# DeMoriarty/TorchPQ

Hardware: AMD Instinct MI355X
Metric: queries/sec + recall@100, SIFT1M IVFPQ d=128 m=64 nprobe=32 (higher is better)
Workload: dtype f32; 1 GPU; SIFT1M-like d=128 n=1000000 IVFPQ n_cells=1024 m=64 nprobe=32 k=100 on 1xMI355X per rank; n_query_per_rank=10000, code_layout=packed, codes=u8 (8-bit PQ), arithmetic=f32 LUT entries, f32 sums, exact ids, use_smart_probing=False, parallelism=query-sharded x1, replicated index, world_size_seen=1, index_broadcast_bytes=0

## Files before the change

__graft_entry__.py:

```python
import os
import subprocess
import sys

ROOT = os.path.dirname(os.path.abspath(__file__))
if ROOT not in sys.path:
    sys.path.insert(0, ROOT)


def build_cabi_demo() -> None:
    src = os.path.join(ROOT, "tests", "cabi", "scan_demo.cpp")
    subprocess.check_call([
        os.environ.get("HIPCC", "/opt/rocm/bin/hipcc"), "--offload-arch=gfx950", "-O2",
        "-I", os.path.join(ROOT, "include"), src, "-L", os.path.join(ROOT, "torchpq_amd"),
        "-ltorchpq_amd", "-Wl,-rpath,$ORIGIN/../../torchpq_amd",
        "-o", os.path.join(ROOT, "tests", "cabi", "scan_demo")])


def check_store_hazard() -> None:
    if os.environ.get("TPQ_SKIP_HAZARD_CHECK", "0") == "1":
        return
    tool = os.path.join(ROOT, "tools", "check_store_hazard.py")
    procs = [(u, subprocess.Popen([sys.executable, tool, "--window", "2", u], stdout=subprocess.PIPE,
                                  stderr=subprocess.STDOUT, text=True))
             for u in ("cascade_core.hip", "assign_cascade.hip", "probe_sims.hip", "lloyd.hip", "select.hip",
                       "coarse_probe.hip", "assign_fast.hip", "flat_topk.hip")]
    bad = []
    for u, p in procs:
        out = p.communicate()[0]
        print(out.strip().splitlines()[-1] if out.strip() else f"{u}: no output")
        if p.returncode != 0:
            bad.append((u, out[-1500:]))
    assert not bad, f"store-data hazard pattern within two instructions: {bad}"


def check_flat_tile_registers() -> None:
    if os.environ.get("TPQ_SKIP_HAZARD_CHECK", "0") == "1":
        return
    out = subprocess.run([sys.executable, os.path.join(ROOT, "tools", "kernel_regs.py"), "flat_topk.hip", "--grep",
                          "flat_tile_kernel"], capture_output=True, text=True, check=True).stdout
    rows = [line for line in out.splitlines() if "flat_tile_kernel" in line]
    assert len(rows) == 5, out
    bad = [line for line in rows if " spill   0 " not in line]
    assert not bad, f"flat_tile_kernel spills registers: {bad}"
    print(f"flat_topk.hip: {len(rows)} flat_tile_kernel instantiations, no register spills")


def check_flat_range_registers() -> None:
    if os.environ.get("TPQ_SKIP_HAZARD_CHECK", "0") == "1":
        return
    out = subprocess.run([sys.executable, os.path.join(ROOT, "tools", "kernel_regs.py"), "flat_range.hip", "--grep",
                          "flat_range_"], capture_output=True, text=True, check=True).stdout
    rows = [line for line in out.splitlines() if "flat_range_" in line]
    assert len(rows) == 2, out
    bad = [line for line in rows if " spill   0 scratch    0 " not in line]
    assert not bad, f"flat_range kernels spill registers or use scratch: {bad}"
    print(f"flat_range.hip: {len(rows)} kernels, no register spills, no scratch")


def check_scan_range_registers() -> None:
    if os.environ.get("TPQ_SKIP_HAZARD_CHECK", "0") == "1":
        return
    out = subprocess.run([sys.executable, os.path.join(ROOT, "tools", "kernel_regs.py"), "scan_range.hip", "--grep",
                          "ivfpq_range_"], capture_output=True, text=True, check=True).stdout
    rows = [line for line in out.splitlines() if "ivfpq_range_" in line]
    assert len(rows) == 4, out
    bad = [line for line in rows if " spill   0 scratch    0 " not in line]
    assert not bad, f"scan_range kernels spill registers or use scratch: {bad}"
    print(f"scan_range.hip: {len(rows)} kernels, no register spills, no scratch")


def check_scan_filtered_registers() -> None:
    if os.environ.get("TPQ_SKIP_HAZARD_CHECK", "0") == "1":
        return
    out = subprocess.run([sys.executable, os.path.join(ROOT, "tools", "kernel_regs.py"), "scan_filtered.hip", "--grep",
                          "filter"], capture_output=True, text=True, check=True).stdout
    rows = [line for line in out.splitlines() if "scan_filtered_" in line or "slot_filter_build" in line]
    assert len(rows) == 11, out
    bad = [line for line in rows if " spill   0 " not in line]
    bad += [line for line in rows if ("<1>" in line or "<2>" in line or "slot_filter" in line)
            and " scratch    0 " not in line]
    assert not bad, f"scan_filtered kernels spill registers or use scratch: {bad}"
    print(f"scan_filtered.hip: {len(rows)} kernels, no register spills, no scratch up to k = 128")


def check_scan_pq4_filtered_registers() -> None:
    if os.environ.get("TPQ_SKIP_HAZARD_CHECK", "0") == "1":
        return
    out = subprocess.run([sys.executable, os.path.join(ROOT, "tools", "kernel_regs.py"), "scan_pq4_filtered.hip",
                          "--grep", "scan_pq4_filtered_"], capture_output=True, text=True, check=True).stdout
    rows = [line for line in out.splitlines() if "scan_pq4_filtered_" in line]
    assert len(rows) == 20, out
    bad = [line for line in rows if " spill   0 " not in line]
    bad += [line for line in rows if ("kernel<1," in line or "kernel<2," in line) and " scratch    0 " not in line]
    assert not bad, f"scan_pq4_filtered kernels spill registers or use scratch: {bad}"
    print(f"scan_pq4_filtered.hip: {len(rows)} kernels, no register spills, no scratch up to k = 128")


def check_scan_pq4_range_registers() -> None:
    if os.environ.get("TPQ_SKIP_HAZARD_CHECK", "0") == "1":
        return
    out = subprocess.run([sys.executable, os.path.join(ROOT, "tools", "kernel_regs.py"), "scan_pq4_range.hip", "--grep",
                          "ivfpq4_range_"], capture_output=True, text=True, check=True).stdout
    rows = [line for line in out.splitlines() if "ivfpq4_range_" in line]
    assert len(rows) == 16, out
    bad = [line for line in rows if " spill   0 scratch    0 " not in line]
    assert not bad, f"scan_pq4_range kernels spill registers or use scratch: {bad}"
    print(f"scan_pq4_range.hip: {len(rows)} kernels, no register spills, no scratch")


def check_scan_flat_registers() -> None:
    if os.environ.get("TPQ_SKIP_HAZARD_CHECK", "0") == "1":
        return
    out = subprocess.run([sys.executable, os.path.join(ROOT, "tools", "kernel_regs.py"), "scan_flat.hip", "--grep",
                          "scan_flat_kernel"], capture_output=True, text=True, check=True).stdout
    rows = [line for line in out.splitlines() if "scan_flat_kernel" in line]
    assert len(rows) == 20, out
    bad = [line for line in rows if " spill   0 " not in line or int(line.split(" vgpr ")[1].split()[0]) > 72]
    assert not bad, f"scan_flat_kernel spills registers or drops below seven waves per SIMD: {bad}"
    print(f"scan_flat.hip: {len(rows)} scan_flat_kernel instantiations, no register spills, at most 72 VGPRs")


def build() -> None:
    subprocess.check_call(["bash", os.path.join(ROOT, "torchpq_amd", "csrc", "build.sh")])
    subprocess.check_call(["make", "-C", os.path.join(ROOT, "oracle"), "libivfpq_oracle.so"])
    build_cabi_demo()
    check_store_hazard()
    check_flat_tile_registers()
    check_flat_range_registers()
    check_scan_range_registers()
    check_scan_filtered_registers()
    check_scan_pq4_filtered_registers()
    check_scan_pq4_range_registers()
    check_scan_flat_registers()
    import torchpq_amd
    from torchpq_amd import _lib
    lib = _lib.load()
    assert lib.tpq_version() >= 100
    for name in _lib.SIGNATURES:
        getattr(lib, name)
    print("build ok:", _lib.LIB_PATH, "version", lib.tpq_version(), "torchpq_amd", torchpq_amd.__version__)


def smoke() -> None:
    import numpy as np
    import torch
    from oracle import c_oracle
    from oracle import ivfpq_oracle as orc
    from torchpq_amd.index import IVFPQIndex

    assert torch.cuda.is_available(), "smoke() needs the MI355X"
    rng = np.random.default_rng(0)
    d, n, nq, k = 64, 8192, 64, 10
    centers = rng.standard_normal((d, 32)) * 4
    base = (centers[:, rng.integers(0, 32, n)] + rng.standard_normal((d, n))).astype(np.float32)
    queries = (base[:, :nq] + 0.1 * rng.standard_normal((d, nq))).astype(np.float32)
    np.random.seed(0)
    idx = IVFPQIndex(d_vector=d, n_subvectors=16, n_cells=32, initial_size=512, device="cuda:0")
    idx.train(torch.from_numpy(base).cuda())
    idx.add(torch.from_numpy(base).cuda())
    idx.n_probe = 8
    xq = torch.from_numpy(queries).cuda()
    vals, ids = idx.search(xq, k=k)
    torch.cuda.synchronize()

    _, cells, npl = idx.probe(xq)
    cells, npl = cells.cpu().numpy(), npl.cpu().numpy()
    lut = c_oracle.adc_lut(queries, idx.pq_codec.codebook.cpu().numpy())
    cs = idx._cell_start.cpu().numpy()[cells]
    sz = idx._cell_size.cpu().numpy()[cells]
    ev, ea = c_oracle.scan_topk(idx._storage.cpu().numpy(), lut, idx._is_empty.cpu().numpy(), cs, sz,
                                npl, k)
    ei = orc.get_id_by_address(idx._address2id.cpu().numpy(), ea)
    assert np.array_equal(vals.cpu().numpy(), ev), "values differ from the oracle"
    assert np.array_equal(ids.cpu().numpy(), ei), "ids differ from the oracle"
    hit = float((ids[:, 0].cpu().numpy() == np.arange(nq)).mean())
    assert hit > 0.8, hit
    print(f"smoke ok: top-1 self hit {hit:.2f}, values/ids bit-exact vs oracle")


if __name__ == "__main__":
    build()
    if len(sys.argv) > 1 and sys.argv[1] == "smoke":
        smoke()
```

include/torchpq_amd.h:

```cpp
#ifndef TORCHPQ_AMD_H_
#define TORCHPQ_AMD_H_

#include <stddef.h>
#include <stdint.h>

#ifdef __cplusplus
extern "C" {
#endif

#define TPQ_VERSION 500

#define TPQ_OK 0
#define TPQ_ERR_INVALID_ARGUMENT (-1)
#define TPQ_ERR_HIP (-2)
#define TPQ_ERR_WORKSPACE (-3)
#define TPQ_ERR_UNSUPPORTED (-4)

#define TPQ_METRIC_NEG_SQ_L2 0
#define TPQ_METRIC_INNER 1

typedef void* tpq_stream_t;

int tpq_version(void);
const char* tpq_last_error(void);

size_t tpq_ivfpq_scan_workspace_bytes(int nq, int k, int n_split, int m);

int tpq_ivfpq_scan_topk(const uint8_t* codes, const float* lut, const uint8_t* is_empty,
                        const int64_t* cell_start, const int64_t* cell_size,
                        const int64_t* n_probe_list, float* out_vals, int64_t* out_addr,
                        const int64_t* address2id, int64_t* out_ids, int64_t n_slots, int nq,
                        int max_nprobe, int m, int k, int n_split, void* workspace,
                        size_t workspace_bytes, tpq_stream_t stream);

int tpq_ivfpq_pack_codes(const uint8_t* codes, uint8_t* packed, int64_t n_slots, int m,
                         int64_t slot_begin, int64_t slot_end, tpq_stream_t stream);

int tpq_ivfpq_scan_topk_packed(const uint8_t* packed, const uint8_t* codes, const float* lut,
                               const uint8_t* is_empty, const int64_t* cell_start,
                               const int64_t* cell_size, const int64_t* n_probe_list,
                               float* out_vals, int64_t* out_addr, const int64_t* address2id,
                               int64_t* out_ids, int64_t n_slots, int nq, int max_nprobe, int m,
                               int k, int n_split, void* workspace, size_t workspace_bytes,
                               tpq_stream_t stream);
size_t tpq_ivfpq_scan_tickets_bytes(int nq);

#define TPQ_SCAN_ROUTE_REF 0
#define TPQ_SCAN_ROUTE_ONE_LAUNCH 1
#define TPQ_SCAN_ROUTE_LISTS 2
#define TPQ_SCAN_ROUTE_POOLS 3
#define TPQ_SCAN_ROUTE_DUMP_F32 8
#define TPQ_SCAN_ROUTE_DUMP_SEL16 16
#define TPQ_SCAN_ROUTE_DUMP_SEL16_W8 17
int tpq_ivfpq_scan_route(int nq, int k, int n_split, int m, int ds, int max_nprobe, int64_t slots_hint, int has_lut,
                         int has_packed, int has_tickets, int residual);
int tpq_ivfpq_scan_order(const int64_t* cell_start, const int64_t* cell_size, const int64_t* n_probe_list, int nq,
                         int max_nprobe, int tile_shift, int32_t* order, int32_t* rank, int32_t* work,
                         tpq_stream_t stream);
int tpq_ivfpq_scan_ordered(int nq, int k, int n_split, int m, int ds, int max_nprobe, int64_t slots_hint, int has_lut,
                           int has_packed, int has_tickets, int residual, int slots, size_t workspace_bytes);
int tpq_ivfpq_scan_topk_packed_tickets(const uint8_t* packed, const uint8_t* codes, const float* lut,
                                       const uint8_t* is_empty, const int64_t* cell_start,
                                       const int64_t* cell_size, const int64_t* n_probe_list,
                                       float* out_vals, int64_t* out_addr, const int64_t* address2id,
                                       int64_t* out_ids, int64_t n_slots, int nq, int max_nprobe,
                                       int m, int k, int n_split, void* workspace,
                                       size_t workspace_bytes, int32_t* tickets, int64_t slots_hint,
                                       tpq_stream_t stream);

int tpq_ivfpq_search_fused(const uint8_t* packed, const uint8_t* codes, const float* query,
                           const float* codebook, int ds, int metric, const uint8_t* is_empty,
                           const int64_t* cell_start, const int64_t* cell_size,
                           const int64_t* n_probe_list, float* out_vals, int64_t* out_addr,
                           const int64_t* address2id, int64_t* out_ids, int64_t n_slots, int nq,
                           int max_nprobe, int m, int k, int n_split, void* workspace,
                           size_t workspace_bytes, tpq_stream_t stream);
int tpq_ivfpq_search_fused_tickets(const uint8_t* packed, const uint8_t* codes, const float* query,
                                   const float* codebook, int ds, int metric, const uint8_t* is_empty,
                                   const int64_t* cell_start, const int64_t* cell_size,
                                   const int64_t* n_probe_list, float* out_vals, int64_t* out_addr,
                                   const int64_t* address2id, int64_t* out_ids, int64_t n_slots,
                                   int nq, int max_nprobe, int m, int k, int n_split, void* workspace,
                                   size_t workspace_bytes, int32_t* tickets, int64_t slots_hint,
                                   tpq_stream_t stream);
int tpq_ivfpq_search_fused_cells(const uint8_t* packed, const uint8_t* codes, const float* query,
                                 const float* codebook, int ds, int metric, const uint8_t* is_empty,
                                 const int64_t* cell_start, const int64_t* cell_size,
                                 const int64_t* n_probe_list, float* out_vals, int64_t* out_addr,
                                 const int64_t* address2id, int64_t* out_ids, int64_t n_slots,
                                 int nq, int max_nprobe, int m, int k, int n_split, void* workspace,
                                 size_t workspace_bytes, int32_t* tickets, int64_t slots_hint,
                                 const int64_t* cells, int n_cells, tpq_stream_t stream);
int tpq_ivfpq_scan_cell_major(int nq, int k, int n_split, int m, int ds, int max_nprobe, int64_t slots_hint, int has_lut,
                              int has_packed, int has_tickets, int residual, int n_cells, int64_t n_slots,
                              size_t workspace_bytes);
int tpq_ivfpq_scan_cell_norms(int nq, int k, int n_split, int m, int ds, int max_nprobe, int64_t slots_hint, int has_lut,
                              int has_packed, int has_tickets, int residual, int n_cells, int64_t n_slots,
                              size_t workspace_bytes);
size_t tpq_ivfpq_cell_candidates_workspace_bytes(int nq, int max_nprobe, int n_cells, int first_probe);
size_t tpq_ivfpq_cell_candidates_norms_workspace_bytes(int nq, int max_nprobe, int n_cells, int first_probe,
                                                       int64_t n_slots);
int tpq_ivfpq_cell_candidates(const uint8_t* codes, const float* query, const float* codebook, int ds, int metric,
                              const uint8_t* is_empty, const int64_t* cell_start, const int64_t* cell_size,
                              const int64_t* n_probe_list, const int64_t* cells, int n_cells, int first_probe,
                              const float* threshold, int64_t n_slots, int nq, int max_nprobe, int m, int capacity,
                              int32_t* out_count, uint32_t* out_keys, uint32_t* out_addr, float* out_delta,
                              int32_t* out_flags, void* workspace, size_t workspace_bytes, tpq_stream_t stream);
float tpq_ivfpq_cell_fold_threshold(float threshold, float q2);
int tpq_ivfpq_scan_cell_threshold(int nq, int k, int n_split, int m, int ds, int max_nprobe, int64_t slots_hint,
                                  int has_lut, int has_packed, int has_tickets, int residual, int n_cells,
                                  int64_t n_slots, size_t workspace_bytes);
int tpq_ivfpq_scan_use_cell_threshold(int on);
int tpq_ivfpq_scan_cell_threshold_probes(void);
#define TPQ_HAS_IVFPQ_CELL_KEPT 1
size_t tpq_ivfpq_cell_kept_bytes(int64_t n_slots, int ds);
long long tpq_ivfpq_scan_cell_inversions(void);
int tpq_ivfpq_search_fused_cells_kept(const uint8_t* packed, const uint8_t* codes, const float* query,
                                      const float* codebook, int ds, int metric, const uint8_t* is_empty,
                                      const int64_t* cell_start, const int64_t* cell_size,
                                      const int64_t* n_probe_list, float* out_vals, int64_t* out_addr,
                                      const int64_t* address2id, int64_t* out_ids, int64_t n_slots,
                                      int nq, int max_nprobe, int m, int k, int n_split, void* workspace,
                                      size_t workspace_bytes, int32_t* tickets, int64_t slots_hint,
                                      const int64_t* cells, int n_cells, void* kept, size_t kept_bytes,
                                      int kept_valid, tpq_stream_t stream);

int tpq_ivfpq_scan_topk_residual(const uint8_t* codes, const float* part1, const float* part2,
                                 const float* full_lut, const int64_t* cells,
                                 const float* base_sims, const uint8_t* is_empty,
                                 const int64_t* cell_start, const int64_t* cell_size,
                                 const int64_t* n_probe_list, float* out_vals, int64_t* out_addr,
                                 const int64_t* address2id, int64_t* out_ids, int64_t n_slots,
                                 int nq, int max_nprobe, int m, int k, tpq_stream_t stream);
int tpq_residual_part1(const float* query, const float* codebook, float* part1, int m, int ds,
                       int nq, tpq_stream_t stream);

int tpq_ivfpq_residual_slot_terms(const uint8_t* codes, const float* part2,
                                  const int64_t* cell_start, const int64_t* cell_size,
                                  float* slot_term, float* cell_bound, int64_t n_slots,
                                  int n_cells, int m, tpq_stream_t stream);
int tpq_ivfpq_scan_topk_residual_packed(
    const uint8_t* packed, const uint8_t* codes, const float* part1, const float* query,
    const float* codebook, int ds, const float* part2, const float* slot_term,
    const float* cell_bound, const int64_t* cells, const float* base_sims, const uint8_t* is_empty,
    const int64_t* cell_start, const int64_t* cell_size, const int64_t* n_probe_list,
    float* out_vals, int64_t* out_addr, const int64_t* address2id, int64_t* out_ids,
    int64_t n_slots, int nq, int max_nprobe, int m, int k, int n_split, void* workspace,
    size_t workspace_bytes, tpq_stream_t stream);

int tpq_adc_lut(const float* query, const float* codebook, float* lut, int m, int ds, int nq,
                int metric, tpq_stream_t stream);

int tpq_topk_select(const float* x, float* vals, int64_t* idx, int rows, int cols, int k,
                    tpq_stream_t stream);

int tpq_coarse_select(const float* dots, const float* a2, const float* b2, float* vals, int64_t* idx,
                      int rows, int cols, int k, tpq_stream_t stream);

size_t tpq_ivfpq_coarse_probe_workspace_bytes(int nq, int n_cells);
int tpq_ivfpq_coarse_probe(const float* query, const float* centroids,
                           const int64_t* cell_start_tbl, const int64_t* cell_size_tbl,
                           float* topk_sims, int64_t* cells, int64_t* cell_start,
                           int64_t* cell_size, int64_t* n_probe_list, int d, int nq, int n_cells,
                           int n_probe, float smart_temperature, void* workspace,
                           size_t workspace_bytes, tpq_stream_t stream);
#define TPQ_PROBE_ROUTE_AUTO 0
#define TPQ_PROBE_ROUTE_FP32 1
#define TPQ_PROBE_ROUTE_FP16 2
size_t tpq_ivfpq_coarse_probe_route_workspace_bytes(int d, int nq, int n_cells, int route);
int tpq_ivfpq_coarse_probe_route(const float* query, const float* centroids,
                                 const int64_t* cell_start_tbl, const int64_t* cell_size_tbl,
                                 float* topk_sims, int64_t* cells, int64_t* cell_start,
                                 int64_t* cell_size, int64_t* n_probe_list, int d, int nq, int n_cells,
                                 int n_probe, float smart_temperature, int route, const void* prepared,
                                 void* workspace, size_t workspace_bytes, tpq_stream_t stream);
size_t tpq_ivfpq_coarse_probe_prepared_bytes(int d, int n_cells);
int tpq_ivfpq_coarse_probe_prepare(const float* centroids, int d, int n_cells, void* prepared,
                                   size_t prepared_bytes, tpq_stream_t stream);

int tpq_smart_probing(const float* topk_sims, int64_t* n_probe_list, int rows, int n_probe,
                      float temperature, tpq_stream_t stream);

int tpq_get_address_by_id(const int64_t* address2id, int64_t capacity, const int64_t* ids,
                          int64_t* address, int64_t n_ids, tpq_stream_t stream);

int tpq_get_id_by_address(const int64_t* address2id, int64_t capacity, const int64_t* address,
                          int64_t* ids, int64_t n, tpq_stream_t stream);

int tpq_max_sim(const float* A, const float* B, float* vals, int64_t* inds, int l, int d, int m,
                int n, int metric, tpq_stream_t stream);

int tpq_max_sim_split_supported(int d, int64_t m, int n);
int tpq_max_sim_split(const float* A, const float* B, float* vals, int64_t* inds, int l, int d, int m,
                      int n, int metric, tpq_stream_t stream);

#define TPQ_ASSIGN_ROUTE_AUTO 0
#define TPQ_ASSIGN_ROUTE_CASCADE 1
int tpq_coarse_assign_supported(int d, int64_t m, int n);
size_t tpq_coarse_assign_workspace_bytes(int d, int64_t m, int n);
size_t tpq_coarse_assign_count_offset(int d, int64_t m, int n);
int tpq_coarse_assign(const float* A, const float* B, float* vals, int64_t* inds, int d, int64_t m, int n,
                      int metric, void* workspace, size_t workspace_bytes, tpq_stream_t stream);
size_t tpq_coarse_assign_route_workspace_bytes(int d, int64_t m, int n, int route);
int tpq_coarse_assign_route(const float* A, const float* B, float* vals, int64_t* inds, int d, int64_t m, int n,
                            int metric, int route, void* workspace, size_t workspace_bytes, tpq_stream_t stream);

int tpq_max_sim_select_supported(int l, int d, int64_t m, int n);
size_t tpq_max_sim_select_workspace_bytes(int l, int d, int64_t m, int n);
int tpq_max_sim_select(const float* A, const float* B, float* vals, int64_t* inds, int l, int d, int64_t m,
                       int n, int metric, void* workspace, size_t workspace_bytes, tpq_stream_t stream);

int tpq_lloyd_supported(int l, int d, int64_t m, int n);
size_t tpq_lloyd_prepared_bytes(int l, int d, int64_t m);
int tpq_lloyd_prepare(const float* data, const float* centroids0, void* prepared, size_t prepared_bytes,
                      int l, int d, int64_t m, int n, tpq_stream_t stream);
size_t tpq_lloyd_step_workspace_bytes(int l, int d, int64_t m, int n);
size_t tpq_lloyd_step_count_offset(int l, int d, int64_t m, int n, int level);
int tpq_lloyd_step(const float* data, const void* prepared, const float* centroids, float* new_centroids,
                   float* vals, int64_t* inds, int l, int d, int64_t m, int n, void* workspace,
                   size_t workspace_bytes, tpq_stream_t stream);

size_t tpq_compute_centroids_workspace_bytes(int l, int d, int k);
int tpq_compute_centroids(const float* data, const int64_t* labels, float* centroids, int l, int d,
                          int64_t n, int k, void* workspace, size_t workspace_bytes,
                          tpq_stream_t stream);

size_t tpq_get_ioa_workspace_bytes(int64_t n);
int tpq_get_ioa(const int64_t* labels, int64_t* ioa, int64_t n, int64_t n_cells, void* workspace,
                size_t workspace_bytes, tpq_stream_t stream);
int tpq_get_write_address(const uint8_t* is_empty, const int64_t* cell_start,
                          const int64_t* cell_capacity, const int64_t* labels, const int64_t* ioa,
                          int64_t* write_address, int64_t n_slots, int64_t n_labels,
                          tpq_stream_t stream);
int tpq_get_cell_by_address(const int64_t* address, const int64_t* cell_start,
                            const int64_t* cell_capacity, int64_t* cells, int64_t n_address,
                            int64_t n_cells, tpq_stream_t stream);

int tpq_grow_cells(const uint8_t* storage, const int64_t* address2id, const uint8_t* is_empty,
                   const int64_t* old_start, const int64_t* old_capacity, const int64_t* new_start,
                   const int64_t* new_capacity, uint8_t* new_storage, int64_t* new_address2id,
                   uint8_t* new_is_empty, int64_t old_slots, int64_t new_slots, int n_cells, int m,
                   tpq_stream_t stream);

int tpq_pq_decode(const float* codebook, const uint8_t* codes, float* out, int m, int ds, int64_t n,
                  tpq_stream_t stream);

int tpq_scatter_codes(const uint8_t* codes, const int64_t* address, uint8_t* storage,
                      uint8_t* packed, int m, int64_t n, int64_t n_slots, tpq_stream_t stream);

int tpq_ivfpqr_rerank(const uint8_t* storage, int64_t capacity, int m, int m_r, const float* codebook,
                      const float* codebook_r, const float* query, int d, int nq, const int64_t* cand_address,
                      int k1, int k, int use_residual, int distance, const int64_t* address2id, float* out_vals,
                      int64_t* out_address, int64_t* out_ids, tpq_stream_t stream);

size_t tpq_ivfflat_scan_workspace_bytes(int nq, int k, int n_split);
int tpq_ivfflat_scan_topk(const float* vectors, const float* query, const uint8_t* is_empty,
                          const int64_t* cell_start, const int64_t* cell_size, const int64_t* n_probe_list,
                          float* out_vals, int64_t* out_addr, int64_t n_slots, int d, int nq, int max_nprobe, int k,
                          int metric, int n_split, void* workspace, size_t workspace_bytes, tpq_stream_t stream);

size_t tpq_ivfpq4_scan_workspace_bytes(int nq, int k, int n_split);
int tpq_ivfpq4_scan_topk(const uint8_t* codes, const float* query, const float* codebook, const uint8_t* is_empty,
                         const int64_t* cell_start, const int64_t* cell_size, const int64_t* n_probe_list,
                         float* out_vals, int64_t* out_addr, int64_t n_slots, int m, int ds, int nq, int max_nprobe,
                         int k, int metric, int n_split, void* workspace, size_t workspace_bytes,
                         tpq_stream_t stream);
// ... 133 lines not shown
```

torchpq_amd/_lib.py:

```python
from __future__ import annotations

import ctypes as C
import os

import torch

_HERE = os.path.dirname(os.path.abspath(__file__))
LIB_PATH = os.environ.get("TPQ_AMD_LIB") or os.path.join(_HERE, "libtorchpq_amd.so")

METRIC_NEG_SQ_L2 = 0
METRIC_INNER = 1
ERR_UNSUPPORTED = -4
ERR_WORKSPACE = -3
ASSIGN_ROUTE_AUTO = 0
ASSIGN_ROUTE_CASCADE = 1
PROBE_ROUTE_AUTO, PROBE_ROUTE_FP32, PROBE_ROUTE_FP16 = 0, 1, 2

_vp, _i, _i64, _sz, _f = C.c_void_p, C.c_int, C.c_int64, C.c_size_t, C.c_float

SIGNATURES = {
    "tpq_version": (_i, []),
    "tpq_last_error": (C.c_char_p, []),
    "tpq_ivfpq_scan_workspace_bytes": (_sz, [_i, _i, _i, _i]),
    "tpq_ivfpq_scan_topk": (_i, [_vp, _vp, _vp, _vp, _vp, _vp, _vp, _vp, _vp, _vp, _i64, _i, _i, _i,
                                 _i, _i, _vp, _sz, _vp]),
    "tpq_ivfpq_pack_codes": (_i, [_vp, _vp, _i64, _i, _i64, _i64, _vp]),
    "tpq_ivfpq_scan_topk_packed": (_i, [_vp, _vp, _vp, _vp, _vp, _vp, _vp, _vp, _vp, _vp, _vp, _i64,
                                        _i, _i, _i, _i, _i, _vp, _sz, _vp]),
    "tpq_ivfpq_search_fused": (_i, [_vp, _vp, _vp, _vp, _i, _i, _vp, _vp, _vp, _vp, _vp, _vp, _vp, _vp,
                                    _i64, _i, _i, _i, _i, _i, _vp, _sz, _vp]),
    "tpq_ivfpq_scan_tickets_bytes": (_sz, [_i]),
    "tpq_ivfpq_scan_route": (_i, [_i, _i, _i, _i, _i, _i, _i64, _i, _i, _i, _i]),
    "tpq_ivfpq_scan_order": (_i, [_vp, _vp, _vp, _i, _i, _i, _vp, _vp, _vp, _vp]),
    "tpq_ivfpq_scan_ordered": (_i, [_i, _i, _i, _i, _i, _i, _i64, _i, _i, _i, _i, _i, _sz]),
    "tpq_ivfpq_scan_topk_packed_tickets": (_i, [_vp, _vp, _vp, _vp, _vp, _vp, _vp, _vp, _vp, _vp, _vp, _i64,
                                                _i, _i, _i, _i, _i, _vp, _sz, _vp, _i64, _vp]),
    "tpq_ivfpq_search_fused_tickets": (_i, [_vp, _vp, _vp, _vp, _i, _i, _vp, _vp, _vp, _vp, _vp, _vp, _vp, _vp,
                                            _i64, _i, _i, _i, _i, _i, _vp, _sz, _vp, _i64, _vp]),
    "tpq_ivfpq_search_fused_cells": (_i, [_vp, _vp, _vp, _vp, _i, _i, _vp, _vp, _vp, _vp, _vp, _vp, _vp, _vp,
                                          _i64, _i, _i, _i, _i, _i, _vp, _sz, _vp, _i64, _vp, _i, _vp]),
    "tpq_ivfpq_search_fused_cells_kept": (_i, [_vp, _vp, _vp, _vp, _i, _i, _vp, _vp, _vp, _vp, _vp, _vp, _vp, _vp,
                                               _i64, _i, _i, _i, _i, _i, _vp, _sz, _vp, _i64, _vp, _i, _vp, _sz, _i,
                                               _vp]),
    "tpq_ivfpq_cell_kept_bytes": (_sz, [_i64, _i]),
    "tpq_ivfpq_scan_cell_inversions": (_i64, []),
    "tpq_ivfpq_scan_cell_major": (_i, [_i, _i, _i, _i, _i, _i, _i64, _i, _i, _i, _i, _i, _i64, _sz]),
    "tpq_ivfpq_scan_cell_norms": (_i, [_i, _i, _i, _i, _i, _i, _i64, _i, _i, _i, _i, _i, _i64, _sz]),
    "tpq_ivfpq_cell_candidates_workspace_bytes": (_sz, [_i, _i, _i, _i]),
    "tpq_ivfpq_cell_candidates_norms_workspace_bytes": (_sz, [_i, _i, _i, _i, _i64]),
    "tpq_ivfpq_cell_candidates": (_i, [_vp, _vp, _vp, _i, _i, _vp, _vp, _vp, _vp, _vp, _i, _i, _vp, _i64, _i, _i, _i,
                                       _i, _vp, _vp, _vp, _vp, _vp, _vp, _sz, _vp]),
    "tpq_ivfpq_cell_fold_threshold": (_f, [_f, _f]),
    "tpq_ivfpq_scan_cell_threshold": (_i, [_i, _i, _i, _i, _i, _i, _i64, _i, _i, _i, _i, _i, _i64, _sz]),
    "tpq_ivfpq_scan_use_cell_threshold": (_i, [_i]),
    "tpq_ivfpq_scan_cell_threshold_probes": (_i, []),
    "tpq_ivfpq_scan_topk_residual": (_i, [_vp, _vp, _vp, _vp, _vp, _vp, _vp, _vp, _vp, _vp, _vp, _vp,
                                          _vp, _vp, _i64, _i, _i, _i, _i, _vp]),
    "tpq_residual_part1": (_i, [_vp, _vp, _vp, _i, _i, _i, _vp]),
    "tpq_ivfpq_residual_slot_terms": (_i, [_vp, _vp, _vp, _vp, _vp, _vp, _i64, _i, _i, _vp]),
    "tpq_ivfpq_scan_topk_residual_packed": (_i, [_vp, _vp, _vp, _vp, _vp, _i, _vp, _vp, _vp, _vp, _vp,
                                                 _vp, _vp, _vp, _vp, _vp, _vp, _vp, _vp, _i64, _i, _i,
                                                 _i, _i, _i, _vp, _sz, _vp]),
    "tpq_adc_lut": (_i, [_vp, _vp, _vp, _i, _i, _i, _i, _vp]),
    "tpq_topk_select": (_i, [_vp, _vp, _vp, _i, _i, _i, _vp]),
    "tpq_coarse_select": (_i, [_vp, _vp, _vp, _vp, _vp, _i, _i, _i, _vp]),
    "tpq_smart_probing": (_i, [_vp, _vp, _i, _i, _f, _vp]),
    "tpq_ivfpq_coarse_probe_workspace_bytes": (_sz, [_i, _i]),
    "tpq_ivfpq_coarse_probe": (_i, [_vp, _vp, _vp, _vp, _vp, _vp, _vp, _vp, _vp, _i, _i, _i, _i, _f,
                                    _vp, _sz, _vp]),
    "tpq_ivfpq_coarse_probe_route_workspace_bytes": (_sz, [_i, _i, _i, _i]),
    "tpq_ivfpq_coarse_probe_route": (_i, [_vp, _vp, _vp, _vp, _vp, _vp, _vp, _vp, _vp, _i, _i, _i, _i, _f, _i,
                                          _vp, _vp, _sz, _vp]),
    "tpq_ivfpq_coarse_probe_prepared_bytes": (_sz, [_i, _i]),
    "tpq_ivfpq_coarse_probe_prepare": (_i, [_vp, _i, _i, _vp, _sz, _vp]),
    "tpq_get_id_by_address": (_i, [_vp, _i64, _vp, _vp, _i64, _vp]),
    "tpq_get_address_by_id": (_i, [_vp, _i64, _vp, _vp, _i64, _vp]),
    "tpq_max_sim": (_i, [_vp, _vp, _vp, _vp, _i, _i, _i, _i, _i, _vp]),
    "tpq_max_sim_split_supported": (_i, [_i, _i64, _i]),
    "tpq_max_sim_split": (_i, [_vp, _vp, _vp, _vp, _i, _i, _i, _i, _i, _vp]),
    "tpq_max_sim_select_supported": (_i, [_i, _i, _i64, _i]),
    "tpq_max_sim_select_workspace_bytes": (_sz, [_i, _i, _i64, _i]),
    "tpq_max_sim_select": (_i, [_vp, _vp, _vp, _vp, _i, _i, _i64, _i, _i, _vp, _sz, _vp]),
    "tpq_lloyd_supported": (_i, [_i, _i, _i64, _i]),
    "tpq_lloyd_prepared_bytes": (_sz, [_i, _i, _i64]),
    "tpq_lloyd_prepare": (_i, [_vp, _vp, _vp, _sz, _i, _i, _i64, _i, _vp]),
    "tpq_lloyd_step_workspace_bytes": (_sz, [_i, _i, _i64, _i]),
    "tpq_lloyd_step_count_offset": (_sz, [_i, _i, _i64, _i, _i]),
    "tpq_lloyd_step": (_i, [_vp, _vp, _vp, _vp, _vp, _vp, _i, _i, _i64, _i, _vp, _sz, _vp]),
    "tpq_coarse_assign_supported": (_i, [_i, _i64, _i]),
    "tpq_coarse_assign_workspace_bytes": (_sz, [_i, _i64, _i]),
    "tpq_coarse_assign_count_offset": (_sz, [_i, _i64, _i]),
    "tpq_coarse_assign": (_i, [_vp, _vp, _vp, _vp, _i, _i64, _i, _i, _vp, _sz, _vp]),
    "tpq_coarse_assign_route_workspace_bytes": (_sz, [_i, _i64, _i, _i]),
    "tpq_coarse_assign_route": (_i, [_vp, _vp, _vp, _vp, _i, _i64, _i, _i, _i, _vp, _sz, _vp]),
    "tpq_compute_centroids_workspace_bytes": (_sz, [_i, _i, _i]),
    "tpq_compute_centroids": (_i, [_vp, _vp, _vp, _i, _i, _i64, _i, _vp, _sz, _vp]),
    "tpq_get_ioa_workspace_bytes": (_sz, [_i64]),
    "tpq_get_ioa": (_i, [_vp, _vp, _i64, _i64, _vp, _sz, _vp]),
    "tpq_get_write_address": (_i, [_vp, _vp, _vp, _vp, _vp, _vp, _i64, _i64, _vp]),
    "tpq_get_cell_by_address": (_i, [_vp, _vp, _vp, _vp, _i64, _i64, _vp]),
    "tpq_grow_cells": (_i, [_vp, _vp, _vp, _vp, _vp, _vp, _vp, _vp, _vp, _vp, _i64, _i64, _i, _i, _vp]),
    "tpq_pq_decode": (_i, [_vp, _vp, _vp, _i, _i, _i64, _vp]),
    "tpq_scatter_codes": (_i, [_vp, _vp, _vp, _vp, _i, _i64, _i64, _vp]),
    "tpq_ivfpqr_rerank": (_i, [_vp, _i64, _i, _i, _vp, _vp, _vp, _i, _i, _vp, _i, _i, _i, _i, _vp, _vp, _vp, _vp,
                               _vp]),
    "tpq_ivfflat_scan_workspace_bytes": (_sz, [_i, _i, _i]),
    "tpq_ivfflat_scan_topk": (_i, [_vp, _vp, _vp, _vp, _vp, _vp, _vp, _vp, _i64, _i, _i, _i, _i, _i, _i, _vp, _sz,
                                   _vp]),
    "tpq_ivfpq4_scan_workspace_bytes": (_sz, [_i, _i, _i]),
    "tpq_ivfpq4_scan_topk": (_i, [_vp] * 9 + [_i64, _i, _i, _i, _i, _i, _i, _i, _vp, _sz, _vp]),
    "tpq_ivfpq4_scan_residual_topk": (_i, [_vp] * 5 + [_i] + [_vp] * 6 + [_i64, _i, _i, _i, _i, _i, _i, _i, _vp, _sz,
                                           _vp]),
    "tpq_ivfpq4_scan_filtered_topk": (_i, [_vp] * 9 + [_i, _i64, _vp, _vp, _i64, _i, _i, _i, _i, _i, _i, _i, _vp, _sz,
                                           _vp]),
    "tpq_ivfpq4_scan_filtered_residual_topk": (_i, [_vp] * 5 + [_i] + [_vp] * 6 + [_i, _i64, _vp, _vp, _i64, _i, _i,
                                                    _i, _i, _i, _i, _i, _vp, _sz, _vp]),
    "tpq_ivfpq4_range_segments": (_sz, [_i, _i]),
    "tpq_ivfpq4_range_count": (_i, [_vp] * 9 + [_i, _i64, _vp, _vp, _i64, _i, _i, _i, _i, _i, _i, _vp]),
    "tpq_ivfpq4_range_fill": (_i, [_vp] * 9 + [_i, _i64] + [_vp] * 4 + [_i64, _i, _i, _i, _i, _i, _i, _vp]),
    "tpq_ivfpq4_range_residual_segments": (_sz, [_i, _i]),
    "tpq_ivfpq4_range_residual_count": (_i, [_vp] * 5 + [_i] + [_vp] * 6 + [_i, _i64, _vp, _vp, _i64, _i, _i, _i, _i,
                                             _i, _vp]),
    "tpq_ivfpq4_range_residual_fill": (_i, [_vp] * 5 + [_i] + [_vp] * 6 + [_i, _i64] + [_vp] * 4 + [_i64, _i, _i, _i,
                                            _i, _i, _vp]),
    "tpq_ivfflat_range_segments": (_sz, [_i, _i]),
    "tpq_ivfflat_range_count": (_i, [_vp, _vp, _vp, _vp, _vp, _vp, _vp, _vp, _i64, _i, _i, _i, _i, _i, _vp]),
    "tpq_ivfflat_range_fill": (_i, [_vp, _vp, _vp, _vp, _vp, _vp, _vp, _vp, _vp, _vp, _i64, _i, _i, _i, _i, _i,
                                    _vp]),
    "tpq_ivfpq_range_segments": (_sz, [_i, _i]),
    "tpq_ivfpq_range_count": (_i, [_vp] * 4 + [_i, _i] + [_vp] * 6 + [_i64, _i, _i, _i, _i, _vp]),
    "tpq_ivfpq_range_fill": (_i, [_vp] * 4 + [_i, _i] + [_vp] * 8 + [_i64, _i, _i, _i, _i, _vp]),
    "tpq_ivfpq_range_residual_segments": (_sz, [_i, _i]),
    "tpq_ivfpq_range_residual_count": (_i, [_vp] * 4 + [_i] + [_vp] * 10 + [_i64, _i, _i, _i, _vp]),
    "tpq_ivfpq_range_residual_fill": (_i, [_vp] * 4 + [_i] + [_vp] * 12 + [_i64, _i, _i, _i, _vp]),
    "tpq_ivfpq_scan_filtered_workspace_bytes": (_sz, [_i, _i, _i]),
    "tpq_ivfpq_scan_filtered_topk": (_i, [_vp] * 4 + [_i, _i] + [_vp] * 6 + [_i, _i64] + [_vp] * 4
                                     + [_i64, _i, _i, _i, _i, _i, _vp, _sz, _vp]),
    "tpq_ivfpq_scan_filtered_residual_topk": (_i, [_vp] * 4 + [_i] + [_vp] * 10 + [_i, _i64] + [_vp] * 4
                                              + [_i64, _i, _i, _i, _i, _vp]),
    "tpq_slot_filter_build": (_i, [_vp, _i64, _vp, _i64, _vp]),
    "tpq_flat_topk_workspace_bytes": (_sz, [_i, _i, _i]),
    "tpq_flat_topk": (_i, [_vp, _vp, _vp, _vp, _vp, _vp, _i64, _i, _i, _i, _i, _i, _vp, _sz, _vp]),
    "tpq_flat_range_segments": (_sz, [_i, _i]),
    "tpq_flat_range_count": (_i, [_vp, _vp, _vp, _vp, _vp, _i64, _i, _i, _i, _i, _vp]),
    "tpq_flat_range_fill": (_i, [_vp, _vp, _vp, _vp, _vp, _vp, _vp, _vp, _i64, _i, _i, _i, _i, _vp]),
    "tpq_ubench_stream_read": (_i, [_vp, _sz, _vp, _i, _vp]),
    "tpq_ubench_stream_read_ex": (_i, [_vp, _sz, _vp, _i, _i, _i, _sz, _i, _vp]),
    "tpq_ubench_rows_read": (_i, [_vp, _i, _i, _i64, _i, _vp, _vp]),
}

_lib = None


class TorchPQAmdError(RuntimeError):
    pass


def load():
    global _lib
    if _lib is None:
        if not os.path.exists(LIB_PATH):
            raise TorchPQAmdError(
                f"{LIB_PATH} not found: build it with `python -c 'import __graft_entry__ as g; "
                "g.build()'` (or torchpq_amd/csrc/build.sh). torchpq_amd has no CPU fallback.")
        lib = C.CDLL(LIB_PATH)
        for name, (res, args) in SIGNATURES.items():
            fn = getattr(lib, name)
            fn.restype = res
            fn.argtypes = args
        _lib = lib
    return _lib


def last_error() -> str:
    msg = load().tpq_last_error()
    return msg.decode("utf-8", "replace") if msg else ""


def check(rc: int, what: str):
    if rc != 0:
        raise TorchPQAmdError(f"{what} failed (code {rc}): {last_error()}")


def ptr(t):
    return None if t is None else C.c_void_p(t.data_ptr())


def stream_ptr(device=None):
    return C.c_void_p(torch.cuda.current_stream(device).cuda_stream)


def require_gpu(*tensors):
    for t in tensors:
        if t is None:
            continue
        if t.device.type != "cuda":
            raise TorchPQAmdError(
                "torchpq_amd runs on an AMD GPU (torch device 'cuda'); got a tensor on "
                f"'{t.device}'. There is no CPU fallback.")
        if not t.is_contiguous():
            raise TorchPQAmdError("torchpq_amd kernels need contiguous tensors")
```

torchpq_amd/csrc/scan.hip:

```cpp
#include <atomic>
#include <chrono>

#include "scan_cells.h"
#include "scan_device.h"
#include "scan_order.h"
#include "scan_ref.h"

namespace tpq {

__global__ __launch_bounds__(256) void residual_part1_kernel(const float* __restrict__ query,
                                                            const float* __restrict__ codebook,
                                                            float* __restrict__ part1, int m,
                                                            int ds, int nq) {
  const int j = blockIdx.y, q = blockIdx.x, c = threadIdx.x;
  float dot = 0.f;
  for (int e = 0; e < ds; ++e)
    dot = fmaf(query[(int64_t)(j * ds + e) * nq + q], codebook[((int64_t)j * ds + e) * 256 + c], dot);
  part1[((int64_t)q * m + j) * 256 + c] = 2.f * dot;
}


static size_t ref_lds_bytes(int m, int R, int max_nprobe, int fused_floats) {
  return list_scan_lds_bytes(list_region0((size_t)m * 1024, R), max_nprobe, (size_t)fused_floats * 4);
}
// ... 110 lines not shown
    if (a.k > kmax || rl4 > 4) return 0;
    if (!a.lut && a.m * a.ds > 128) return 0;
    if (a.lut && a.slots_hint < kDumpLutMinSlots) return 0;
    return kDumpF32;
  }
  if (a.lut || !dump_built(a.m, kDumpSel16) || a.ds > 2) return 0;
  const int rl8 = list_regs_scan(a.k, a.m, a.max_nprobe, a.slots_hint);
  if (rl4 <= 2 || (rl4 <= 4 && rl4 <= rl8)) return kDumpSel16;
  if (e && atoi(e) == 1) return 0;
  if (a.k > 248 && rl8 <= 2) return kDumpSel16W8;
  return 0;
}

template <int N, class Query>
static int device_cached(std::atomic<int> (&cache)[64][N], int i, int fallback, Query query) {
  int dev = 0;
  if (hipGetDevice(&dev) != hipSuccess || dev < 0 || dev >= 64) return fallback;
  int n = cache[dev][i].load(std::memory_order_relaxed);
  if (n <= 0) {
    n = query(dev);
    if (n <= 0) n = fallback;
    cache[dev][i].store(n, std::memory_order_relaxed);
  }
  return n;
}
static int device_cus() {
  static std::atomic<int> cus[64][1] = {};
  return device_cached(cus, 0, 256, [](int dev) {
    int n = 0;
    return hipDeviceGetAttribute(&n, hipDeviceAttributeMultiprocessorCount, dev) == hipSuccess ? n : 0;
  });
}
static int dump_slots(const PackedUnit& u, int mode) {
  static std::atomic<int> per_cu[64][3 * 4] = {};
  const int mi = mode == kDumpSel16 ? 0 : (mode == kDumpF32 ? 1 : 2), ci = u.m == 64 ? 0 : (u.m == 32 ? 1 : (u.m == 16 ? 2 : 3));
  return device_cached(per_cu, mi * 4 + ci, 4, [&](int) { return u.dump_occupancy(mode); }) * device_cus();
}
static void dump_tail(int nq, int nw, int RL, int slots, int* unsplit, int* parts) {
  *unsplit = nq;
  *parts = 1;
  if (slots <= 0) return;
  const int whole = (nq / slots) * slots, rest = nq - whole;
  if (rest == 0) return;
  for (int c = 4; c >= 2; c >>= 1) {
    if ((int64_t)rest * c <= slots && c * nw * RL <= 16) {
      *unsplit = whole;
      *parts = c;
      return;
    }
  }
}

struct ScanPlan {
  int route = -1;
  int R = 0;
  int RL = 0;
  int Rf = 0;
  int mode = 0;
  int waves = 0;
  int n_split = 1;
  bool fuse = false;
  bool small_lists = false;
  int unsplit = 0;
  int parts = 1;
  bool ordered = false;
};

static ScanPlan plan_scan(const ScanArgs& a, bool residual) {
  const int m = a.m, k = a.k;
  ScanPlan p;
  p.n_split = a.n_split;
  if (!packed_unit(m)) {
    if (!residual && !a.lut) p.route = TPQ_SCAN_ROUTE_REF;
    return p;
  }
  p.R = list_regs_packed(k);
  p.waves = packed_waves(m);
  const bool lds_fits =
      scan_lds_bytes_packed(m, p.R > 16 ? 16 : p.R, a.max_nprobe, fused_floats_of(a), residual) <= 160 * 1024;
  if (p.R > 16 || !lds_fits) {
    p.route = TPQ_SCAN_ROUTE_REF;
    if (residual) p.n_split = 1;
    return p;
  }
  const bool pools = !residual && p.R >= pool_min_list_regs(m) && (p.waves < 16 || k > 768) && fuse_enabled();
  const int Rf = dump_finish_regs(k, a.slots_hint), mode = dump_route(a, residual, Rf);
  if (mode && !(is_sel16(mode) && pools)) {
    const int nw = scan_waves(m, mode), RL = list_regs_scan(k, m, a.max_nprobe, a.slots_hint, nw);
    if (dump_pair_built(mode, RL, Rf)) {
      p.route = mode == kDumpF32 ? TPQ_SCAN_ROUTE_DUMP_F32
                                 : (mode == kDumpSel16 ? TPQ_SCAN_ROUTE_DUMP_SEL16 : TPQ_SCAN_ROUTE_DUMP_SEL16_W8);
      p.mode = mode, p.waves = nw, p.RL = RL, p.Rf = Rf, p.n_split = 1;
      return p;
    }
  }
  if (pools) {
    p.route = TPQ_SCAN_ROUTE_POOLS;
    p.RL = pool_list_regs(k, m);
    if (p.n_split > pool_max_split(m, k)) p.n_split = pool_max_split(m, k);
    return p;
  }
  p.RL = list_regs_scan(k, m, a.max_nprobe, a.slots_hint);
  p.small_lists = p.RL < p.R;
  p.fuse = !residual && fuse_enabled() && fuse_fits(m, p.R) && p.waves * p.RL >= p.R && (a.n_split == 1 || a.tickets);
  p.route = p.fuse ? TPQ_SCAN_ROUTE_ONE_LAUNCH : TPQ_SCAN_ROUTE_LISTS;
  return p;
}

static void plan_dump_dispatch(ScanPlan& p, int nq, int slots, size_t workspace_bytes) {
  int unsplit = nq, parts = 1;
  if (p.mode != kDumpSel16W8) dump_tail(nq, p.waves, p.RL, slots, &unsplit, &parts);
  if (parts > 1 && workspace_bytes < ws_bytes_for(nq, p.RL, parts * p.waves)) unsplit = nq, parts = 1;
  p.parts = parts;
  p.unsplit = parts > 1 ? unsplit : 0;
  p.ordered = slots > 0 && nq > slots && nq <= kOrderMaxQueries &&
              workspace_bytes >= ws_bytes_for(nq, p.RL, parts * p.waves) + order_ws_bytes(nq);
}
static bool is_dump_route(int route) {
  return route == TPQ_SCAN_ROUTE_DUMP_F32 || route == TPQ_SCAN_ROUTE_DUMP_SEL16 || route == TPQ_SCAN_ROUTE_DUMP_SEL16_W8;
}

static ScanArgs route_query_args(int nq, int k, int n_split, int m, int ds, int max_nprobe, int64_t slots_hint,
                                 int has_lut, int has_tickets) {
  ScanArgs a{};
  static const float dummy_lut = 0.f;
  static int32_t dummy_tickets = 0;
  a.lut = has_lut ? &dummy_lut : nullptr;
  a.ds = has_lut ? 0 : ds;
  a.nq = nq; a.k = k; a.n_split = n_split; a.m = m; a.max_nprobe = max_nprobe;
  a.slots_hint = slots_hint;
  a.tickets = has_tickets ? &dummy_tickets : nullptr;
  return a;
}

extern "C" int tpq_ivfpq_scan_route(int nq, int k, int n_split, int m, int ds, int max_nprobe, int64_t slots_hint,
                                    int has_lut, int has_packed, int has_tickets, int residual) {
  if (nq <= 0 || k < 1 || k > 1024 || m < 4 || m % 4 != 0 || n_split < 1 || max_nprobe < 1) return -1;
  if (!has_packed) return TPQ_SCAN_ROUTE_REF;
  return plan_scan(route_query_args(nq, k, n_split, m, ds, max_nprobe, slots_hint, has_lut, has_tickets), residual != 0)
      .route;
}

extern "C" int tpq_ivfpq_scan_ordered(int nq, int k, int n_split, int m, int ds, int max_nprobe, int64_t slots_hint,
                                      int has_lut, int has_packed, int has_tickets, int residual, int slots,
                                      size_t workspace_bytes) {
  if (nq <= 0 || k < 1 || k > 1024 || m < 4 || m % 4 != 0 || n_split < 1 || max_nprobe < 1) return -1;
  if (!has_packed) return 0;
  ScanPlan p =
      plan_scan(route_query_args(nq, k, n_split, m, ds, max_nprobe, slots_hint, has_lut, has_tickets), residual != 0);
  if (!is_dump_route(p.route)) return 0;
  plan_dump_dispatch(p, nq, slots > 0 ? slots : dump_slots(*packed_unit(m), p.mode), workspace_bytes);
  return p.ordered ? 1 : 0;
}

struct CellMajor {
  const int64_t* cells;
  int n_cells;
  void* kept = nullptr;
  size_t kept_bytes = 0;
  int kept_valid = 0;
};
static void cell_major_use_kept(CellArgs& c, const CellMajor& cm) {
  if (cm.kept && c.norm && cm.kept_bytes >= cell_kept_bytes(c.n_slots, c.ds)) cell_use_kept(c, cm.kept, cm.kept_valid);
}
static int cell_major_chunks(const ScanArgs& a, const ScanPlan& p, bool residual, int n_cells, size_t workspace_bytes) {
  if (residual || p.route != TPQ_SCAN_ROUTE_DUMP_SEL16 || a.lut || a.m != 64 || a.ds < 1 || a.ds > 2) return 0;
  if (a.k > 128 || a.max_nprobe <= kCellP0 || n_cells < 1 || a.n_slots <= 0 || a.slots_hint <= 0) return 0;
  if ((int64_t)a.nq * a.slots_hint < (int64_t)kCellMinRereads * a.n_slots) return 0;
  if ((int64_t)a.nq * a.max_nprobe >= 0x7fffffffLL) return 0;
  const size_t extra = cell_extra_bytes(a.nq, a.max_nprobe, n_cells, kCellP0);
  for (int chunks = 16; chunks >= 8; chunks >>= 1)
    if ((a.k + 63) / 64 < chunks && workspace_bytes >= ws_bytes_for(a.nq, 1, chunks) + extra) return chunks;
  return 0;
}
static bool cell_major_norms(const ScanArgs& a, int chunks, int n_cells, size_t workspace_bytes) {
  return chunks > 0 && workspace_bytes >= ws_bytes_for(a.nq, 1, chunks) +
                                              cell_extra_bytes(a.nq, a.max_nprobe, n_cells, kCellP0) +
                                              cell_norm_bytes(a.n_slots);
}

static int run_cell_major(ScanArgs& a, ScanPlan p, const PackedUnit& u, const CellMajor& cm, int chunks, void* workspace,
                          size_t workspace_bytes, hipStream_t st) {
  const int nq = a.nq;
  ScanArgs t = a;
  t.probe_cap = kCellP0;
  plan_dump_dispatch(p, nq, dump_slots(u, p.mode), workspace_bytes);
  t.n_split = p.parts;
  t.unsplit = p.unsplit;
  const size_t lists_bytes = ws_bytes_for(nq, p.RL, p.parts * p.waves);
  int rc = need_ws(workspace, workspace_bytes, lists_bytes, "ivfpq_scan_packed");
  if (rc) return rc;
  fill_ws(t, workspace, p.RL, p.parts * p.waves);
  if (p.ordered) {
    int* o = reinterpret_cast<int*>(reinterpret_cast<char*>(workspace) + lists_bytes);
    const size_t stride = order_ws_bytes(nq) / 3 / sizeof(int);
    rc = launch_scan_order(a.cell_start, a.cell_size, a.n_probe_list, nq, a.max_nprobe, packed_tile_shift(a.m), o,
                           o + stride, o + 2 * stride, st, kCellP0);
    if (rc) return rc;
    t.order = o;
    t.rank = o + stride;
  }
  rc = u.dump(t, p.RL, p.Rf, p.mode, st);
  if (rc) return rc;
  a.n_split = 1;
  a.unsplit = 0;
  fill_ws(a, workspace, 1, chunks);
  CellArgs c{};
  c.codes = a.codes; c.query = a.query; c.codebook = a.codebook; c.is_empty = a.is_empty;
  c.cell_start = a.cell_start; c.cell_size = a.cell_size; c.n_probe_list = a.n_probe_list; c.cells = cm.cells;
  c.n_slots = a.n_slots; c.nq = nq; c.max_nprobe = a.max_nprobe; c.n_cells = cm.n_cells; c.ds = a.ds;
  c.euclid = a.euclid; c.p0 = kCellP0; c.p_hi = a.max_nprobe; c.k = a.k; c.chunks = chunks; c.epoch = a.epoch;
  c.rel = cell_delta_rel(a.ds);
  c.seed_vals = a.out_vals; c.seed_addr = a.out_addr;
  c.keys = reinterpret_cast<unsigned*>(a.ws_vals); c.idx = reinterpret_cast<unsigned*>(a.ws_idx);
  c.list_evict = a.list_evict; c.flags = a.flags; c.ws_delta = a.ws_delta;
  const size_t cm_lists = ws_bytes_for(nq, 1, chunks);
  cell_fill_extras(c, reinterpret_cast<char*>(workspace) + cm_lists, workspace_bytes - cm_lists);
  cell_major_use_kept(c, cm);
  rc = launch_cell_candidates(c, st);
  if (rc) return rc;
  return u.finish(a, chunks, p.Rf, (a.k + 63) / 64, c.cnt, st);
}

static bool cell_threshold_form(const ScanArgs& a, int chunks, int n_cells, size_t workspace_bytes) {
  if (!cell_major_norms(a, chunks, n_cells, workspace_bytes) || a.max_nprobe <= kCellThrProbes) return false;
  const size_t need = ws_bytes_for(a.nq, 1, chunks) + cell_extra_bytes(a.nq, a.max_nprobe, n_cells, kCellP0) +
                      cell_norm_bytes(a.n_slots) + cell_thr_bytes(a.nq, a.max_nprobe, n_cells);
  const int64_t mean_cell = a.slots_hint / a.max_nprobe;
  return workspace_bytes >= need && mean_cell >= kCellThrMinCell &&
         (int64_t)kCellThrProbes * mean_cell / kCellThrGroup >= 2 * (int64_t)a.k;
}

static int run_cell_threshold(ScanArgs& a, const ScanPlan& p, const PackedUnit& u, const CellMajor& cm, int chunks,
                              void* workspace, hipStream_t st) {
  const int nq = a.nq;
  a.n_split = 1;
  a.unsplit = 0;
  fill_ws(a, workspace, 1, chunks);
  CellArgs c{};
  c.codes = a.codes; c.query = a.query; c.codebook = a.codebook; c.is_empty = a.is_empty;
  c.cell_start = a.cell_start; c.cell_size = a.cell_size; c.n_probe_list = a.n_probe_list; c.cells = cm.cells;
  c.n_slots = a.n_slots; c.nq = nq; c.max_nprobe = a.max_nprobe; c.n_cells = cm.n_cells; c.ds = a.ds;
  c.euclid = a.euclid; c.p0 = 0; c.p_hi = a.max_nprobe; c.k = 0; c.thr_k = a.k; c.chunks = chunks; c.epoch = a.epoch;
  c.rel = cell_delta_rel(a.ds);
  c.keys = reinterpret_cast<unsigned*>(a.ws_vals); c.idx = reinterpret_cast<unsigned*>(a.ws_idx);
  c.list_evict = a.list_evict; c.flags = a.flags; c.ws_delta = a.ws_delta;
  char* at = reinterpret_cast<char*>(workspace) + ws_bytes_for(nq, 1, chunks);
  const size_t head = cell_extra_bytes(nq, a.max_nprobe, cm.n_cells, kCellP0) + cell_norm_bytes(a.n_slots);
  cell_fill_extras(c, at, head, kCellP0);
  cell_major_use_kept(c, cm);
  CellThrArrays t{};
  cell_fill_thr(t, at + head, nq, a.max_nprobe, cm.n_cells);
  int rc = launch_cell_threshold(c, t, st);
  if (rc) return rc;
  return u.finish(a, chunks, p.Rf, 0, c.cnt, st);
}

extern "C" int tpq_ivfpq_scan_cell_major(int nq, int k, int n_split, int m, int ds, int max_nprobe, int64_t slots_hint,
                                         int has_lut, int has_packed, int has_tickets, int residual, int n_cells,
                                         int64_t n_slots, size_t workspace_bytes) {
  if (nq <= 0 || k < 1 || k > 1024 || m < 4 || m % 4 != 0 || n_split < 1 || max_nprobe < 1) return -1;
  if (!has_packed) return 0;
  ScanArgs a = route_query_args(nq, k, n_split, m, ds, max_nprobe, slots_hint, has_lut, has_tickets);
  a.n_slots = n_slots;
  const ScanPlan p = plan_scan(a, residual != 0);
  return cell_major_chunks(a, p, residual != 0, n_cells, workspace_bytes) ? 1 : 0;
}

extern "C" int tpq_ivfpq_scan_cell_norms(int nq, int k, int n_split, int m, int ds, int max_nprobe, int64_t slots_hint,
                                         int has_lut, int has_packed, int has_tickets, int residual, int n_cells,
                                         int64_t n_slots, size_t workspace_bytes) {
  if (nq <= 0 || k < 1 || k > 1024 || m < 4 || m % 4 != 0 || n_split < 1 || max_nprobe < 1) return -1;
  if (!has_packed) return 0;
  ScanArgs a = route_query_args(nq, k, n_split, m, ds, max_nprobe, slots_hint, has_lut, has_tickets);
  a.n_slots = n_slots;
  const ScanPlan p = plan_scan(a, residual != 0);
  const int chunks = cell_major_chunks(a, p, residual != 0, n_cells, workspace_bytes);
  return cell_major_norms(a, chunks, n_cells, workspace_bytes) ? 1 : 0;
}

extern "C" int tpq_ivfpq_scan_cell_threshold(int nq, int k, int n_split, int m, int ds, int max_nprobe,
                                             int64_t slots_hint, int has_lut, int has_packed, int has_tickets,
                                             int residual, int n_cells, int64_t n_slots, size_t workspace_bytes) {
  if (nq <= 0 || k < 1 || k > 1024 || m < 4 || m % 4 != 0 || n_split < 1 || max_nprobe < 1) return -1;
  if (!has_packed) return 0;
  ScanArgs a = route_query_args(nq, k, n_split, m, ds, max_nprobe, slots_hint, has_lut, has_tickets);
  a.n_slots = n_slots;
  const ScanPlan p = plan_scan(a, residual != 0);
  const int chunks = cell_major_chunks(a, p, residual != 0, n_cells, workspace_bytes);
  return cell_threshold_form(a, chunks, n_cells, workspace_bytes) ? 1 : 0;
}

static std::atomic<int> g_cell_threshold{1};
extern "C" int tpq_ivfpq_scan_use_cell_threshold(int on) { return g_cell_threshold.exchange(on ? 1 : 0); }
extern "C" int tpq_ivfpq_scan_cell_threshold_probes(void) { return kCellThrProbes; }

static int run_packed(ScanArgs a, const ResidualArgs* ra, void* workspace, size_t workspace_bytes,
                      tpq_stream_t stream, const CellMajor* cm = nullptr) {
  int rc = validate(a);
  if (rc) return rc;
  TPQ_REQUIRE(a.packed != nullptr, "ivfpq_scan_packed: null packed pointer");
  if (a.nq == 0) return TPQ_OK;
  hipStream_t st = reinterpret_cast<hipStream_t>(stream);
  ScanPlan p = plan_scan(a, ra != nullptr);
  if (p.route == TPQ_SCAN_ROUTE_REF) {
    a.n_split = p.n_split;
    return ra ? run_residual_ref(a, *ra, st) : run_ref(a, workspace, workspace_bytes, st);
  }
  if (p.route < 0) {
    set_error("ivfpq_scan_packed: no scan-layout kernel instantiated for n_subvectors=%d; use "
              "tpq_ivfpq_scan_topk", a.m);
    return TPQ_ERR_UNSUPPORTED;
  }
  const PackedUnit& u = *packed_unit(a.m);
  const int nq = a.nq;
  a.n_split = p.n_split;
  a.small_lists = p.small_lists;
  a.fuse = p.fuse;
  if (!p.fuse) a.tickets = nullptr;
  a.epoch = fresh_epoch();
#ifdef TPQ_SCAN_PROFILE
  a.prof = g_scan_prof;
#endif
  switch (p.route) {
    case TPQ_SCAN_ROUTE_POOLS: {
      const int n_lists = p.n_split * p.waves;
      rc = need_ws(workspace, workspace_bytes, pool_ws_bytes(nq, a.k, a.m, n_lists), "ivfpq_scan_packed");
      if (rc) return rc;
      fill_ws_pool(a, workspace, n_lists);
      rc = u.pool(a, p.RL, st);
      break;
    }
    case TPQ_SCAN_ROUTE_DUMP_F32:
    case TPQ_SCAN_ROUTE_DUMP_SEL16:
    case TPQ_SCAN_ROUTE_DUMP_SEL16_W8: {
      if (const int chunks = cm ? cell_major_chunks(a, p, ra != nullptr, cm->n_cells, workspace ? workspace_bytes : 0) : 0) {
        rc = g_cell_threshold.load() && cell_threshold_form(a, chunks, cm->n_cells, workspace_bytes)
                 ? run_cell_threshold(a, p, u, *cm, chunks, workspace, st)
                 : run_cell_major(a, p, u, *cm, chunks, workspace, workspace_bytes, st);
        break;
      }
      plan_dump_dispatch(p, nq, dump_slots(u, p.mode), workspace ? workspace_bytes : 0);
      a.n_split = p.parts;
      a.unsplit = p.unsplit;
      const size_t lists_bytes = ws_bytes_for(nq, p.RL, p.parts * p.waves);
      rc = need_ws(workspace, workspace_bytes, lists_bytes, "ivfpq_scan_packed");
      if (rc) return rc;
      fill_ws(a, workspace, p.RL, p.parts * p.waves);
      if (p.ordered) {
        int* o = reinterpret_cast<int*>(reinterpret_cast<char*>(workspace) + lists_bytes);
        const size_t stride = order_ws_bytes(nq) / 3 / sizeof(int);
        rc = launch_scan_order(a.cell_start, a.cell_size, a.n_probe_list, nq, a.max_nprobe, packed_tile_shift(a.m), o,
                               o + stride, o + 2 * stride, st, 0);
        if (rc) return rc;
        a.order = o;
        a.rank = o + stride;
      }
      rc = u.dump(a, p.RL, p.Rf, p.mode, st);
      break;
    }
    default: {
      const int n_lists = p.n_split * p.waves;
      rc = need_ws(workspace, workspace_bytes, ws_bytes_for(nq, p.RL, n_lists), "ivfpq_scan_packed");
      if (rc) return rc;
      fill_ws(a, workspace, p.RL, n_lists);
      rc = u.packed(a, ra, p.RL, p.R, st);
      if (p.fuse) return rc;
    }
  }
  if (rc) return rc;
  return redo_flagged(a, ra, st);
}

extern "C" size_t tpq_ivfpq_scan_tickets_bytes(int nq) { return nq > 0 ? (size_t)nq * sizeof(int32_t) : 0; }

extern "C" size_t tpq_ivfpq_cell_kept_bytes(int64_t n_slots, int ds) {
  return n_slots > 0 && (ds == 1 || ds == 2) ? cell_kept_bytes(n_slots, ds) : 0;
}

extern "C" int tpq_ivfpq_search_fused_cells_kept(const uint8_t* packed, const uint8_t* codes,
                                                 const float* query, const float* codebook, int ds,
                                                 int metric, const uint8_t* is_empty,
                                                 const int64_t* cell_start, const int64_t* cell_size,
                                                 const int64_t* n_probe_list, float* out_vals,
                                                 int64_t* out_addr, const int64_t* address2id,
                                                 int64_t* out_ids, int64_t n_slots, int nq, int max_nprobe,
                                                 int m, int k, int n_split, void* workspace,
                                                 size_t workspace_bytes, int32_t* tickets,
                                                 int64_t slots_hint, const int64_t* cells, int n_cells,
                                                 void* kept, size_t kept_bytes, int kept_valid,
                                                 tpq_stream_t stream) {
  TPQ_REQUIRE(metric == TPQ_METRIC_NEG_SQ_L2 || metric == TPQ_METRIC_INNER,
              "ivfpq_search_fused: bad metric %d", metric);
  TPQ_REQUIRE(ds >= 1 && ds <= 1024, "ivfpq_search_fused: bad sub-vector length %d", ds);
  ScanArgs a = scan_args(codes, packed, nullptr, is_empty, cell_start, cell_size, n_probe_list, out_vals, out_addr,
                         address2id, out_ids, n_slots, nq, max_nprobe, m, k, n_split);
  a.query = query; a.codebook = codebook; a.ds = ds; a.euclid = metric == TPQ_METRIC_NEG_SQ_L2 ? 1 : 0;
  a.tickets = tickets; a.slots_hint = slots_hint;
  TPQ_REQUIRE((reinterpret_cast<uintptr_t>(kept) & 15) == 0, "ivfpq_search_fused: the kept state must be 16-byte aligned");
  const CellMajor cm{cells, n_cells, kept, kept_bytes, kept_valid};
  return packed ? run_packed(a, nullptr, workspace, workspace_bytes, stream, cells ? &cm : nullptr)
                : run_ref(a, workspace, workspace_bytes, reinterpret_cast<hipStream_t>(stream));
}

extern "C" int tpq_ivfpq_search_fused_cells(const uint8_t* packed, const uint8_t* codes,
                                            const float* query, const float* codebook, int ds,
                                            int metric, const uint8_t* is_empty,
                                            const int64_t* cell_start, const int64_t* cell_size,
                                            const int64_t* n_probe_list, float* out_vals,
                                            int64_t* out_addr, const int64_t* address2id,
                                            int64_t* out_ids, int64_t n_slots, int nq, int max_nprobe,
                                            int m, int k, int n_split, void* workspace,
                                            size_t workspace_bytes, int32_t* tickets,
                                            int64_t slots_hint, const int64_t* cells, int n_cells,
                                            tpq_stream_t stream) {
  return tpq_ivfpq_search_fused_cells_kept(packed, codes, query, codebook, ds, metric, is_empty, cell_start, cell_size,
                                           n_probe_list, out_vals, out_addr, address2id, out_ids, n_slots, nq,
                                           max_nprobe, m, k, n_split, workspace, workspace_bytes, tickets, slots_hint,
                                           cells, n_cells, nullptr, 0, 0, stream);
}

extern "C" int tpq_ivfpq_search_fused_tickets(const uint8_t* packed, const uint8_t* codes,
                                              const float* query, const float* codebook, int ds,
                                              int metric, const uint8_t* is_empty,
                                              const int64_t* cell_start, const int64_t* cell_size,
                                              const int64_t* n_probe_list, float* out_vals,
                                              int64_t* out_addr, const int64_t* address2id,
                                              int64_t* out_ids, int64_t n_slots, int nq, int max_nprobe,
                                              int m, int k, int n_split, void* workspace,
                                              size_t workspace_bytes, int32_t* tickets,
                                              int64_t slots_hint, tpq_stream_t stream) {
  return tpq_ivfpq_search_fused_cells(packed, codes, query, codebook, ds, metric, is_empty, cell_start, cell_size,
                                      n_probe_list, out_vals, out_addr, address2id, out_ids, n_slots, nq, max_nprobe, m,
                                      k, n_split, workspace, workspace_bytes, tickets, slots_hint, nullptr, 0, stream);
}

extern "C" int tpq_ivfpq_search_fused(const uint8_t* packed, const uint8_t* codes,
                                      const float* query, const float* codebook, int ds,
                                      int metric, const uint8_t* is_empty,
                                      const int64_t* cell_start, const int64_t* cell_size,
                                      const int64_t* n_probe_list, float* out_vals,
                                      int64_t* out_addr, const int64_t* address2id,
                                      int64_t* out_ids, int64_t n_slots, int nq, int max_nprobe,
                                      int m, int k, int n_split, void* workspace,
                                      size_t workspace_bytes, tpq_stream_t stream) {
  return tpq_ivfpq_search_fused_tickets(packed, codes, query, codebook, ds, metric, is_empty, cell_start,
                                        cell_size, n_probe_list, out_vals, out_addr, address2id, out_ids,
                                        n_slots, nq, max_nprobe, m, k, n_split, workspace, workspace_bytes,
                                        nullptr, 0, stream);
}

extern "C" int tpq_ivfpq_scan_topk(const uint8_t* codes, const float* lut, const uint8_t* is_empty,
                                   const int64_t* cell_start, const int64_t* cell_size,
                                   const int64_t* n_probe_list, float* out_vals, int64_t* out_addr,
// ... 149 lines not shown
```

torchpq_amd/csrc/scan_cells.h:

```cpp
#pragma once
#include "common.h"

namespace tpq {

#ifndef TPQ_CELL_P0
#define TPQ_CELL_P0 4
#endif
constexpr int kCellP0 = TPQ_CELL_P0;
#ifndef TPQ_CELL_THR_PROBES
#define TPQ_CELL_THR_PROBES 6
#endif
#ifndef TPQ_CELL_THR_GROUP
#define TPQ_CELL_THR_GROUP 16
#endif
constexpr int kCellThrProbes = TPQ_CELL_THR_PROBES;
constexpr int kCellThrGroup = TPQ_CELL_THR_GROUP;
static_assert(kCellThrGroup == 8 || kCellThrGroup == 16, "a group is half or all of a lane's 16 rows of a tile");
constexpr int kCellThrMinCell = 512;
constexpr int kCellMinRereads = 96;
constexpr int kCellQSplit = 256;
constexpr int kCellGroup = 32;
#ifndef TPQ_CELL_PIECES_A
#define TPQ_CELL_PIECES_A 2
#endif
#ifndef TPQ_CELL_PIECES_B
#define TPQ_CELL_PIECES_B 1
#endif
constexpr int kCellPiecesA = TPQ_CELL_PIECES_A, kCellPiecesB = TPQ_CELL_PIECES_B;
static_assert(kCellPiecesA >= 1 && kCellPiecesA <= 8 && kCellPiecesB >= 1 && kCellPiecesB <= 8, "pieces per block");
constexpr int cell_pieces(bool maxima) { return maxima ? kCellPiecesA : kCellPiecesB; }
#ifndef TPQ_CELL_SLICE
#define TPQ_CELL_SLICE 128
#endif
constexpr int kCellSlice = TPQ_CELL_SLICE;
constexpr int kCellLdsCells = 16384;

struct CellView {
  int *hist, *cell_off, *blk_off, *cell_st, *cell_sz, *pairs;
};

struct CellArgs {
  const uint8_t* codes;
  const float* query;
  const float* codebook;
  const uint8_t* is_empty;
  const int64_t* cell_start;
  const int64_t* cell_size;
  const int64_t* n_probe_list;
  const int64_t* cells;
  int64_t n_slots;
  int nq, max_nprobe, n_cells, ds, euclid;
  int p0;
  int p_hi;
  int k;
  int thr_k;
  int work;
  int chunks;
  int epoch;
  float rel;
  const float* seed_vals;
  const int64_t* seed_addr;
  const float* thr_in;
  unsigned* keys;
  unsigned* idx;
  int* list_evict;
  int* flags;
  float* ws_delta;
  float* params;
  float* thr;
  float* qscale;
  float* qnorm;
  int* cnt;
  int* hist;
  int* cell_off;
  int* blk_off;
  int* cell_st;
  int* cell_sz;
  int* pairs;
  _Float16* qsplit;
  float* norm;
  int* hist2;
  int* n_max;
  int p_a;
  CellView va;
  float* kparams;
  unsigned* book;
  int kept_build;
};
inline size_t cell_book_bytes(int ds) { return (size_t)64 * 256 * 4 * ds; }
inline size_t cell_kept_bytes(int64_t n_slots, int ds) {
  return 256 + cell_book_bytes(ds) + ((((size_t)(n_slots > 0 ? n_slots : 0) * 4) + 255) & ~(size_t)255);
}
inline void cell_use_kept(CellArgs& a, void* kept, int valid) {
  char* p = reinterpret_cast<char*>(kept);
  a.kparams = reinterpret_cast<float*>(p);
  a.book = reinterpret_cast<unsigned*>(p + 256);
  a.norm = reinterpret_cast<float*>(p + 256 + cell_book_bytes(a.ds));
  a.kept_build = valid ? 0 : 1;
}
struct CellThrArrays {
  int* pairs_b;
  int *hist, *cell_off, *blk_off, *cell_st, *cell_sz, *pairs, *n_max;
};

__host__ __device__ inline CellView cell_view(const CellArgs& a) {
  return CellView{a.hist, a.cell_off, a.blk_off, a.cell_st, a.cell_sz, a.pairs};
}
inline size_t cell_align(size_t x) { return (x + 255) & ~(size_t)255; }
inline size_t cell_extra_bytes(int nq, int max_nprobe, int n_cells, int p0) {
  const int np = max_nprobe > p0 ? max_nprobe - p0 : 0;
  return 256 + 4 * cell_align((size_t)nq * 4) + cell_align((size_t)n_cells * 4) +
         2 * cell_align(((size_t)n_cells + 1) * 4) + 2 * cell_align((size_t)n_cells * 4) +
         cell_align((size_t)nq * np * 4) + cell_align((size_t)nq * kCellQSplit * 2);
}
inline size_t cell_norm_bytes(int64_t n_slots) { return cell_align((size_t)(n_slots > 0 ? n_slots : 0) * 4); }
inline size_t cell_thr_bytes(int nq, int max_nprobe, int n_cells) {
  const int t = max_nprobe < kCellThrProbes ? max_nprobe : kCellThrProbes;
  return cell_align((size_t)nq * max_nprobe * 4) + 3 * cell_align((size_t)n_cells * 4) +
         2 * cell_align(((size_t)n_cells + 1) * 4) + cell_align((size_t)nq * t * 4) + cell_align((size_t)nq * 4);
}
__host__ __device__ inline int cell_float_ord(float f) {
  const unsigned b = __builtin_bit_cast(unsigned, f);
  return (b & 0x80000000u) ? (int)(0x80000000u - b) : (int)b;
}
__host__ __device__ inline float cell_ord_float(int o) {
  return __builtin_bit_cast(float, o >= 0 ? (unsigned)o : 0x80000000u - (unsigned)o);
}
__host__ __device__ inline float cell_fold_threshold(float thr, float q2) {
  constexpr long long kTop = 0x7f800000;
  if (!(thr == thr) || thr == __builtin_inff() || thr == -__builtin_inff()) return thr;
  auto pass = [&](long long o) { return (cell_ord_float((int)o) - q2) >= thr; };
  const float t0 = thr + q2;
  if (!(t0 == t0)) return t0;
  long long lo, hi, step = 1;
  if (pass(cell_float_ord(t0))) {
    hi = cell_float_ord(t0);
    for (;; step *= 2) {
      lo = hi - step > -kTop ? hi - step : -kTop;
      if (lo == -kTop || !pass(lo)) break;
      hi = lo;
    }
  } else {
    lo = cell_float_ord(t0);
    for (;; step *= 2) {
      hi = lo + step < kTop ? lo + step : kTop;
      if (hi == kTop || pass(hi)) break;
      lo = hi;
    }
  }
  while (hi - lo > 1) {
    const long long mid = lo + (hi - lo) / 2;
    if (pass(mid)) hi = mid; else lo = mid;
  }
  return cell_ord_float((int)hi);
}

void cell_fill_extras(CellArgs& a, void* at, size_t room, int layout_p0 = -1);
float cell_delta_rel(int ds);
int launch_cell_candidates(const CellArgs& a, hipStream_t st);
void cell_fill_thr(CellThrArrays& t, void* at, int nq, int max_nprobe, int n_cells);
int launch_cell_threshold(const CellArgs& a, const CellThrArrays& t, hipStream_t st);

}
```

torchpq_amd/csrc/scan_cells.hip:

```cpp
#include <atomic>
#include <cmath>

#include "mfma_util.h"
#include "scan_cells.h"
#include "scan_fk.h"
#include "wave_topk.h"

namespace tpq {

float cell_delta_rel(int ds) {
  const double D = 64.0 * ds, N = 3.0 * D, u = 1.0 / 16777216.0;
  const double sum = 0.5 * (3.03 * 4 * u + 1.003 * N * 2 * u) + 1.01 * std::sqrt(D) * u / 4 + (D + 1) * u + 14 * u + 4 * u +
                     1.001 * (64 + ds + 2) * u;
  return (float)(1.25 * sum * (1.0 + 1.0 / 1024));
}

void cell_fill_extras(CellArgs& a, void* at, size_t room, int layout_p0) {
  char* p = reinterpret_cast<char*>(at);
  const int p0 = layout_p0 >= 0 ? layout_p0 : a.p0;
  const size_t extras = cell_extra_bytes(a.nq, a.max_nprobe, a.n_cells, p0);
  a.norm = room >= extras && room - extras >= cell_norm_bytes(a.n_slots) ? reinterpret_cast<float*>(p + extras) : nullptr;
  auto take = [&](size_t bytes) {
    char* r = p;
    p += cell_align(bytes);
    return r;
  };
  const int np = a.max_nprobe > p0 ? a.max_nprobe - p0 : 0;
  a.params = reinterpret_cast<float*>(take(256));
  a.thr = reinterpret_cast<float*>(take((size_t)a.nq * 4));
  a.qscale = reinterpret_cast<float*>(take((size_t)a.nq * 4));
  a.qnorm = reinterpret_cast<float*>(take((size_t)a.nq * 4));
  a.cnt = reinterpret_cast<int*>(take((size_t)a.nq * 4));
  a.hist = reinterpret_cast<int*>(take((size_t)a.n_cells * 4));
  a.cell_off = reinterpret_cast<int*>(take(((size_t)a.n_cells + 1) * 4));
  a.blk_off = reinterpret_cast<int*>(take(((size_t)a.n_cells + 1) * 4));
  a.cell_st = reinterpret_cast<int*>(take((size_t)a.n_cells * 4));
  a.cell_sz = reinterpret_cast<int*>(take((size_t)a.n_cells * 4));
  a.pairs = reinterpret_cast<int*>(take((size_t)a.nq * np * 4));
  a.qsplit = reinterpret_cast<_Float16*>(take((size_t)a.nq * kCellQSplit * 2));
  a.kparams = a.params;
  a.book = nullptr;
  a.kept_build = 0;
}

constexpr int kCellScaleExp = 12;
constexpr int kCellMaxExp = 40;
constexpr unsigned kMaxFiniteBits = 0x7f7fffffu;

__device__ __forceinline__ float pow2i(int e) { return __uint_as_float((unsigned)(e + 127) << 23); }
__device__ __forceinline__ int exp_of_bits(unsigned bits) { return (int)((bits >> 23) & 255u) - 127; }

template <int DS>
__device__ __forceinline__ unsigned prep_maxima(const float* __restrict__ codebook, int lane, int wave, float* c2max_s) {
  float y[4][4][DS];
#pragma unroll
  for (int jj = 0; jj < 4; ++jj)
#pragma unroll
    for (int cc = 0; cc < 4; ++cc)
#pragma unroll
      for (int e = 0; e < DS; ++e) y[jj][cc][e] = codebook[((wave + 16 * jj) * DS + e) * 256 + lane + 64 * cc];
  unsigned mb = 0u;
#pragma unroll
  for (int jj = 0; jj < 4; ++jj) {
    float c2m = 0.f;
#pragma unroll
    for (int cc = 0; cc < 4; ++cc) {
      float c2 = 0.f;
#pragma unroll
      for (int e = 0; e < DS; ++e) {
        const unsigned b = __float_as_uint(y[jj][cc][e]) & 0x7fffffffu;
        mb = b > mb ? b : mb;
        c2 = fmaf(y[jj][cc][e], y[jj][cc][e], c2);
      }
      c2m = fmaxf(c2m, c2);
    }
#pragma unroll
    for (int d = 32; d > 0; d >>= 1) c2m = fmaxf(c2m, __shfl_xor(c2m, d, 64));
    if (lane == 0) c2max_s[wave + 16 * jj] = c2m;
  }
  return mb;
}

__global__ __launch_bounds__(1024) void cell_prep_kernel(CellArgs a) {
  __shared__ unsigned maxbits_s;
  __shared__ float c2max_s[64];
  const int tid = (int)threadIdx.x, lane = tid & 63, wave = tid >> 6;
  if (tid == 0) maxbits_s = 0u;
  __syncthreads();
  const unsigned mb = a.ds == 1 ? prep_maxima<1>(a.codebook, lane, wave, c2max_s)
                                : prep_maxima<2>(a.codebook, lane, wave, c2max_s);
  atomicMax(&maxbits_s, mb);
  __syncthreads();
  if (tid == 0) {
    float x2 = 0.f;
    for (int j = 0; j < 64; ++j) x2 += c2max_s[j];
    x2 *= 1.0001f;
    const unsigned bits = maxbits_s;
    const int e = exp_of_bits(bits);
    const bool ok = bits != 0u && bits <= kMaxFiniteBits && e >= -kCellMaxExp && e <= kCellMaxExp && x2 <= 3e38f;
    a.kparams[0] = __uint_as_float(bits);
    a.kparams[1] = x2;
    a.kparams[2] = ok ? 1.f : 0.f;
    a.kparams[3] = ok ? pow2i(kCellScaleExp - e) : 0.f;
  }
}

struct ListedProbe {
  bool listed;
  int cell;
};
__device__ __forceinline__ int cell_n_probe(const CellArgs& a, int q) {
  const int n = (int)a.n_probe_list[q];
  return n < 0 ? 0 : (n > a.p_hi ? a.p_hi : n);
}
__device__ __forceinline__ ListedProbe listed_probe(const CellArgs& a, int q, int p) {
  const int64_t o = (int64_t)q * a.max_nprobe + p;
  const int64_t st = a.cell_start[o], sz = a.cell_size[o];
  const bool again = p > 0 && a.cell_start[o - 1] == st;
  return ListedProbe{sz > 0 && !again, (int)a.cells[o]};
}

__global__ __launch_bounds__(256) void cell_seed_kernel(CellArgs a) {
  const int lane = (int)(threadIdx.x & 63);
  const int q = (int)blockIdx.x * 4 + (int)(threadIdx.x >> 6);
  for (int i = (int)(blockIdx.x * 256 + threadIdx.x); i < a.n_cells; i += (int)gridDim.x * 256) {
    a.hist[i] = 0;
    if (a.hist2) a.hist2[i] = 0;
  }
  if (blockIdx.x == 0 && threadIdx.x < 2) reinterpret_cast<int*>(a.params)[8 + threadIdx.x] = 0;
  if (q >= a.nq) return;
  const int D = 64 * a.ds;
  const float x0 = lane < D ? a.query[(int64_t)lane * a.nq + q] : 0.f;
  const float x1 = 64 + lane < D ? a.query[(int64_t)(64 + lane) * a.nq + q] : 0.f;
  unsigned mb = __float_as_uint(x0) & 0x7fffffffu;
  const unsigned mb1 = __float_as_uint(x1) & 0x7fffffffu;
  mb = mb1 > mb ? mb1 : mb;
  float q2 = fmaf(x1, x1, x0 * x0);
#pragma unroll
  for (int d = 32; d > 0; d >>= 1) {
    const unsigned o = (unsigned)__shfl_xor((int)mb, d, 64);
    mb = o > mb ? o : mb;
    q2 += __shfl_xor(q2, d, 64);
  }
  const int n_probe = cell_n_probe(a, q);
  bool bad_cell = false;
  for (int p = a.p0 + lane; p < n_probe; p += 64) {
    const int64_t c = a.cells[(int64_t)q * a.max_nprobe + p];
    bad_cell = bad_cell || c < 0 || c >= (int64_t)a.n_cells;
  }
  bad_cell = __ballot(bad_cell) != 0ull;
  const float tau = a.k > 0 ? a.seed_vals[(int64_t)q * a.k + a.k - 1] : (a.thr_k > 0 ? 0.f : a.thr_in[q]);
  const int eq = exp_of_bits(mb);
  const bool flagged = a.k > 0 && a.flags[q] == a.epoch;
  const bool scalable = a.kparams[2] != 0.f && mb != 0u && mb <= kMaxFiniteBits && eq >= -kCellMaxExp &&
                        eq <= kCellMaxExp && q2 <= 3e38f;
  const bool tau_ok = tau == tau && tau != INFINITY;
  const bool active = !flagged && scalable && tau_ok && !bad_cell;
  if (!active) {
    if (lane == 0) {
      a.flags[q] = a.epoch;
      a.cnt[q] = 0;
      a.thr[q] = INFINITY;
    }
    return;
  }
  const float B = sqrtf(q2) * 1.000001f + sqrtf(a.kparams[1]) * 1.000001f;
  const float delta = a.rel * (B * B);
  if (lane == 0) {
    if (a.thr_k == 0) a.thr[q] = a.euclid ? cell_fold_threshold(tau - delta, q2) : tau - delta;
    a.ws_delta[q] = 2.f * delta;
    a.qscale[q] = pow2i(kCellScaleExp - eq);
    a.qnorm[q] = q2;
    a.cnt[q] = 0;
    if (a.k == 0) a.flags[q] = 0;
  }
  if (a.list_evict && lane < a.chunks) a.list_evict[(int64_t)q * a.chunks + lane] = 0;
  {
    const float sq = pow2i(kCellScaleExp - eq);
    _Float16* qs = a.qsplit + (int64_t)q * kCellQSplit;
    const float y0 = x0 * sq, y1 = x1 * sq;
    const _Float16 h0 = (_Float16)y0, h1 = (_Float16)y1;
    if (lane < D) {
      qs[lane] = h0;
      qs[128 + lane] = (_Float16)(y0 - (float)h0);
    }
    if (64 + lane < D) {
      qs[64 + lane] = h1;
      qs[192 + lane] = (_Float16)(y1 - (float)h1);
    }
  }
  const int64_t base = (int64_t)q * a.chunks * 64;
  const int seed_chunks = (a.k + 63) / 64;
  for (int t = 0; t < a.chunks; ++t) {
    const int e = t * 64 + lane;
    Key key = pad_key();
    if (e < a.k) {
      const int64_t ad = a.seed_addr[(int64_t)q * a.k + e];
      if (ad >= 0) key = make_key(a.seed_vals[(int64_t)q * a.k + e], (int)ad);
    }
    if (t < seed_chunks) a.keys[base + e] = key.hi;
    a.idx[base + e] = key.lo;
  }
}

constexpr int kCellSliceThreads = 1024;
template <class F>
__device__ __forceinline__ void for_slice_pairs(const CellArgs& a, int q0, F&& f) {
  const int np = a.p_hi - a.p0;
  const int nqs = a.nq - q0 < kCellSlice ? a.nq - q0 : kCellSlice;
  for (int i = (int)threadIdx.x; i < nqs * np; i += kCellSliceThreads) {
    const int dq = i / np;
    const int q = q0 + dq, p = a.p0 + (i - dq * np);
    if (p >= cell_n_probe(a, q) || a.flags[q] == a.epoch) continue;
    const ListedProbe lp = listed_probe(a, q, p);
    if (lp.listed) f(q, p, lp.cell);
  }
}
template <bool TWO>
__device__ __forceinline__ void count_slice(const CellArgs& a, int q0, int* cell_h) {
  for (int c = (int)threadIdx.x; c < (TWO ? 2 : 1) * a.n_cells; c += kCellSliceThreads) cell_h[c] = 0;
  __syncthreads();
  for_slice_pairs(a, q0, [&](int, int p, int c) {
    atomicAdd(&cell_h[c], 1);
    if (TWO && p < a.p_a) atomicAdd(&cell_h[a.n_cells + c], 1);
  });
  __syncthreads();
}

template <bool TWO>
__global__ __launch_bounds__(kCellSliceThreads) void cell_count_kernel(CellArgs a) {
  extern __shared__ int cell_h[];
  count_slice<TWO>(a, (int)blockIdx.x * kCellSlice, cell_h);
  for (int c = (int)threadIdx.x; c < a.n_cells; c += kCellSliceThreads) {
    const int h = cell_h[c];
    if (h) atomicAdd(&a.hist[c], h);
    if constexpr (TWO) {
      const int ha = cell_h[a.n_cells + c];
      if (ha) atomicAdd(&a.hist2[c], ha);
    }
  }
}

__global__ __launch_bounds__(256) void cell_count_wide_kernel(CellArgs a) {
  const int lane = (int)(threadIdx.x & 63);
  const int q = (int)blockIdx.x * 4 + (int)(threadIdx.x >> 6);
  if (q >= a.nq) return;
  if (a.flags[q] == a.epoch) return;
  const int n_probe = cell_n_probe(a, q);
  for (int p = a.p0 + lane; p < n_probe; p += 64) {
    const ListedProbe lp = listed_probe(a, q, p);
    if (lp.listed) atomicAdd(&a.hist[lp.cell], 1);
  }
}

__global__ __launch_bounds__(1024) void cell_scan_kernel(CellArgs a) {
  __shared__ int sp[2][1024], sb[2][1024];
  const int tid = (int)threadIdx.x;
  if (blockIdx.x == 1) {
    a.hist = a.va.hist;
    a.cell_off = a.va.cell_off;
    a.blk_off = a.va.blk_off;
  }
  const int per = (a.n_cells + 1023) / 1024;
  const int lo = tid * per < a.n_cells ? tid * per : a.n_cells;
  const int hi = lo + per < a.n_cells ? lo + per : a.n_cells;
  int np = 0, nb = 0;
  for (int c = lo; c < hi; ++c) {
    const int h = a.hist[c];
    np += h;
    nb += (h + kCellGroup - 1) / kCellGroup;
  }
  sp[0][tid] = np;
  sb[0][tid] = nb;
  __syncthreads();
  int cur = 0;
  for (int d = 1; d < 1024; d <<= 1) {
    const int vp = sp[cur][tid] + (tid >= d ? sp[cur][tid - d] : 0);
    const int vb = sb[cur][tid] + (tid >= d ? sb[cur][tid - d] : 0);
    sp[cur ^ 1][tid] = vp;
    sb[cur ^ 1][tid] = vb;
    cur ^= 1;
    __syncthreads();
  }
  int op = sp[cur][tid] - np, ob = sb[cur][tid] - nb;
  for (int c = lo; c < hi; ++c) {
    const int h = a.hist[c];
    a.cell_off[c] = op;
    a.blk_off[c] = ob;
    a.hist[c] = op;
    op += h;
    ob += (h + kCellGroup - 1) / kCellGroup;
  }
  if (tid == 1023) {
    a.cell_off[a.n_cells] = sp[cur][1023];
    a.blk_off[a.n_cells] = sb[cur][1023];
  }
}

__device__ __forceinline__ void place_pair(const CellArgs& a, const CellView& v, int q, int p, int c, int pos) {
  v.pairs[pos] = q;
  if (pos == v.cell_off[c]) {
    const int64_t o = (int64_t)q * a.max_nprobe + p;
    v.cell_st[c] = (int)a.cell_start[o];
    v.cell_sz[c] = (int)a.cell_size[o];
  }
}

template <bool TWO>
__global__ __launch_bounds__(kCellSliceThreads) void cell_scatter_kernel(CellArgs a) {
  extern __shared__ int cell_h[];
  const int q0 = (int)blockIdx.x * kCellSlice;
  count_slice<TWO>(a, q0, cell_h);
  for (int c = (int)threadIdx.x; c < a.n_cells; c += kCellSliceThreads) {
    const int h = cell_h[c];
    if (h) cell_h[c] = atomicAdd(&a.hist[c], h);
    if constexpr (TWO) {
      const int ha = cell_h[a.n_cells + c];
      if (ha) cell_h[a.n_cells + c] = atomicAdd(&a.hist2[c], ha);
    }
  }
  __syncthreads();
  for_slice_pairs(a, q0, [&](int q, int p, int c) {
    place_pair(a, cell_view(a), q, p, c, atomicAdd(&cell_h[c], 1));
    if (TWO && p < a.p_a) place_pair(a, a.va, q, p, c, atomicAdd(&cell_h[a.n_cells + c], 1));
  });
}

__global__ __launch_bounds__(256) void cell_scatter_wide_kernel(CellArgs a) {
  const int lane = (int)(threadIdx.x & 63);
  const int q = (int)blockIdx.x * 4 + (int)(threadIdx.x >> 6);
  if (q >= a.nq) return;
  if (a.flags[q] == a.epoch) return;
  const int n_probe = cell_n_probe(a, q);
  for (int p = a.p0 + lane; p < n_probe; p += 64) {
    const ListedProbe lp = listed_probe(a, q, p);
    if (lp.listed) place_pair(a, cell_view(a), q, p, lp.cell, atomicAdd(&a.hist[lp.cell], 1));
  }
}

#ifndef TPQ_CELL_WAVES
#define TPQ_CELL_WAVES 8
#endif
constexpr int kCellWaves = TPQ_CELL_WAVES;
constexpr size_t kCellLdsBytes = 160 * 1024;
template <int DS>
struct CellBook {
  static constexpr int KS = 4 * DS;
  static constexpr size_t kBook = (size_t)64 * 256 * 4 * DS;
  static constexpr int kWaves = kCellWaves;
  static constexpr int kThreads = 64 * kWaves;
  static constexpr size_t kNorms = (size_t)kWaves * 32 * 4;
  static constexpr int kDepth = (int)((kCellLdsBytes - (size_t)64 * 256 * 8 - kNorms) / ((size_t)kWaves * 64 * 8));
  static constexpr size_t kBytes = kBook + kNorms + (size_t)kWaves * 64 * kDepth * 8;
  static_assert(kDepth >= 1 && kBytes <= kCellLdsBytes, "the staging area does not fit the CU's LDS");
};

__device__ __forceinline__ unsigned pack_f16x2(_Float16 lo, _Float16 hi) {
  return (unsigned)__builtin_bit_cast(unsigned short, lo) | ((unsigned)__builtin_bit_cast(unsigned short, hi) << 16);
}
__device__ __forceinline__ float f16_lo(unsigned w) { return (float)__builtin_bit_cast(_Float16, (unsigned short)(w & 0xffffu)); }
__device__ __forceinline__ float f16_hi(unsigned w) { return (float)__builtin_bit_cast(_Float16, (unsigned short)(w >> 16)); }

template <int DS>
__device__ __forceinline__ void book_entry(const float* __restrict__ codebook, float sx, int i, unsigned* book) {
  const int j = i >> 8, c = i & 255;
  _Float16 h[DS], l[DS];
#pragma unroll
  for (int e = 0; e < DS; ++e) {
    const float ys = codebook[(j * DS + e) * 256 + c] * sx;
    h[e] = (_Float16)ys;
    l[e] = (_Float16)(ys - (float)h[e]);
  }
  if constexpr (DS == 2) {
    book[2 * i] = pack_f16x2(h[0], h[1]);
    book[2 * i + 1] = pack_f16x2(l[0], l[1]);
  } else {
    book[i] = pack_f16x2(h[0], l[0]);
  }
}
template <int DS>
__global__ __launch_bounds__(256) void cell_book_kernel(CellArgs a) {
  const int i = (int)(blockIdx.x * 256 + threadIdx.x);
  book_entry<DS>(a.codebook, a.kparams[3], i, a.book);
}

template <int DS, bool ALL = false>
__global__ __launch_bounds__(512) void cell_norm_kernel(CellArgs a) {
  constexpr int KS = 4 * DS;
  extern __shared__ __attribute__((aligned(16))) char smem[];
  float* sums = reinterpret_cast<float*>(smem);
  const int tid = (int)threadIdx.x;
  const float sx = a.kparams[3];
  const float inv_sx = 1.f / sx;
  const float inv_sx2 = inv_sx * inv_sx;
  for (int i = tid; i < 64 * 256; i += 512) {
    const int j = i >> 8, c = i & 255;
#pragma unroll
    for (int e = 0; e < DS; ++e) {
      const float ys = a.codebook[(j * DS + e) * 256 + c] * sx;
      const _Float16 h = (_Float16)ys;
      const _Float16 l = (_Float16)(ys - (float)h);
      sums[i * DS + e] = (float)h + (float)l;
    }
  }
  __syncthreads();
  const int n_units = ALL ? (int)((a.n_slots + 511) / 512) : a.n_cells;
  for (int c = (int)blockIdx.x; c < n_units; c += (int)gridDim.x) {
    int64_t st;
    int sz;
    if constexpr (ALL) {
      st = (int64_t)c * 512;
      sz = a.n_slots - st < 512 ? (int)(a.n_slots - st) : 512;
    } else {
      if (a.cell_off[c + 1] == a.cell_off[c]) continue;
      st = a.cell_st[c];
      sz = a.cell_sz[c];
      if (st < 0 || sz < 0 || st + sz > a.n_slots) sz = 0;
    }
    for (int r = tid; r < sz; r += 512) {
      const int64_t slot = st + r;
      const uint32_t* __restrict__ cw = reinterpret_cast<const uint32_t*>(a.codes) + slot;
      uint32_t w[16];
#pragma unroll
      for (int g = 0; g < 16; ++g) w[g] = cw[(int64_t)g * a.n_slots];
      const bool empty = a.is_empty && a.is_empty[slot];
      float x2h[2];
#pragma unroll
      for (int half = 0; half < 2; ++half) {
        float x2 = 0.f;
#pragma unroll
        for (int s = 0; s < KS; ++s) {
#pragma unroll
          for (int bb = 0; bb < 8 / DS; ++bb) {
            const int j = (16 * s + 8 * half) / DS + bb;
            const int code = (int)((w[j >> 2] >> (8 * (j & 3))) & 255u);
            if constexpr (DS == 2) {
              const float2 v = reinterpret_cast<const float2*>(sums)[j * 256 + code];
              x2 = fmaf(v.x, v.x, x2);
              x2 = fmaf(v.y, v.y, x2);
            } else {
              const float v = sums[j * 256 + code];
              x2 = fmaf(v, v, x2);
            }
          }
        }
        x2h[half] = x2;
      }
      a.norm[slot] = empty ? __builtin_nanf("") : (x2h[0] + x2h[1]) * inv_sx2;
    }
  }
}

template <int DS, bool NORMS, bool EUCLID, bool MAXIMA = false>
__global__ __launch_bounds__(CellBook<DS>::kThreads) void cell_cand_kernel(CellArgs a) {
  static_assert(!MAXIMA || NORMS, "pass A reads the slot norms");
  using T = CellBook<DS>;
  constexpr int S = cell_pieces(MAXIMA);
  constexpr int KS = T::KS;
  constexpr int kDepth = T::kDepth;
  extern __shared__ __attribute__((aligned(16))) char smem[];
  unsigned* book = reinterpret_cast<unsigned*>(smem);
  const int tid = (int)threadIdx.x, lane = tid & 63, wave = tid >> 6;
  float* x2w = reinterpret_cast<float*>(smem + T::kBook) + wave * 32;
  uint2* stage = reinterpret_cast<uint2*>(smem + T::kBook + T::kNorms) + wave * (64 * kDepth) + lane;
  int* work = reinterpret_cast<int*>(a.params) + 8 + a.work;
  const int n_blocks = a.blk_off[a.n_cells];
  const int col = lane & 31, half = lane >> 5;
  const float sx = a.kparams[3];
  const float inv_sx = 1.f / sx;
  const float inv_sx2 = inv_sx * inv_sx;
  const uint8_t* __restrict__ emp = a.is_empty ? a.is_empty : a.codes;
  if (a.book) {
    const u32x4* __restrict__ img = reinterpret_cast<const u32x4*>(a.book);
    for (int i = tid; i < (int)(T::kBook / 16); i += T::kThreads) reinterpret_cast<u32x4*>(book)[i] = img[i];
  } else {
    for (int i = tid; i < 64 * 256; i += T::kThreads) book_entry<DS>(a.codebook, sx, i, book);
  }
  __syncthreads();
  const int64_t cap = (int64_t)a.chunks * 64;
  const int seed_entries = ((a.k + 63) / 64) * 64;
  for (;;) {
    int b = 0;
    if (lane == 0) b = atomicAdd(work, 1);
    b = __builtin_amdgcn_readfirstlane(b);
    const int piece = S > 1 ? b % S : 0;
    if constexpr (S > 1) b /= S;
    if (b >= n_blocks) break;
    int lo = 0, hi = a.n_cells;
    while (hi - lo > 1) {
      const int mid = (lo + hi) >> 1;
      if (a.blk_off[mid] <= b) lo = mid; else hi = mid;
    }
    const int c = lo, g = b - a.blk_off[c];
    const int first = a.cell_off[c] + g * kCellGroup;
    const int n_listed = a.cell_off[c + 1] - first;
    const int nqs = n_listed < kCellGroup ? n_listed : kCellGroup;
    const int64_t st = a.cell_st[c];
    int sz = a.cell_sz[c];
    if (st < 0 || sz < 0 || st + sz > a.n_slots) sz = 0;
    if (sz == 0) continue;
    int r_lo = 0, r_hi = sz;
    if constexpr (S > 1) {
      const int nt = (sz + 31) >> 5;
      r_lo = (piece * nt / S) << 5;
      r_hi = ((piece + 1) * nt / S) << 5;
      if (r_lo == r_hi) continue;
      if (r_hi > sz) r_hi = sz;
    }
    const bool qvalid = col < nqs;
    const int q = qvalid ? a.pairs[first + col] : 0;
    const float sq = qvalid ? a.qscale[q] : 0.f;
    const float thr2 = qvalid ? a.thr[q] : INFINITY;
    const float q2 = qvalid ? a.qnorm[q] : 0.f;
    const float unscale = qvalid ? (1.f / sq) * inv_sx : 0.f;
    const float um = EUCLID ? 2.f * unscale : unscale;
    f16x8 qh[KS], ql[KS];
    const _Float16* __restrict__ qs = a.qsplit + (int64_t)q * kCellQSplit + 8 * half;
#pragma unroll
    for (int s = 0; s < KS; ++s) {
      const u32x4 z = {0u, 0u, 0u, 0u};
      qh[s] = __builtin_bit_cast(f16x8, qvalid ? *reinterpret_cast<const u32x4*>(qs + 16 * s) : z);
      ql[s] = __builtin_bit_cast(f16x8, qvalid ? *reinterpret_cast<const u32x4*>(qs + 128 + 16 * s) : z);
    }
    auto load_tile = [&](int r0, uint32_t (&w)[8], unsigned& aux) {
      const int row = r0 + col < sz ? r0 + col : sz - 1;
      const int64_t slot = st + row;
      const uint32_t* __restrict__ cw = reinterpret_cast<const uint32_t*>(a.codes) + slot;
#pragma unroll
      for (int i = 0; i < 8; ++i) {
        const int gq = DS == 2 ? 2 * i + half : 4 * (i >> 1) + 2 * half + (i & 1);
        w[i] = cw[(int64_t)gq * a.n_slots];
      }
      if constexpr (NORMS)
        aux = __float_as_uint(a.norm[slot]);
      else
        aux = emp[slot];
    };
    int fill = 0;
    auto flush = [&]() {
      if (fill > 0) {
        const int64_t e0 = (int64_t)seed_entries + atomicAdd(&a.cnt[q], fill);
        if (e0 + fill > cap) a.flags[q] = a.epoch;
        unsigned* __restrict__ qkeys = a.keys + (int64_t)q * cap + e0;
        unsigned* __restrict__ qidx = a.idx + (int64_t)q * cap + e0;
        const int fits = e0 + fill <= cap ? fill : (e0 < cap ? (int)(cap - e0) : 0);
#pragma unroll 1
        for (int i = 0; i < fits; ++i) {
          const uint2 v = stage[i * 64];
          qkeys[i] = v.x;
          qidx[i] = v.y;
        }
      }
      fill = 0;
    };
    int me = (int)cap;
    unsigned* __restrict__ mkeys = a.keys + (int64_t)q * cap;
    if constexpr (MAXIMA) {
      if (qvalid) me = atomicAdd(&a.cnt[q], ((r_hi - r_lo + 31) >> 5) * (16 / kCellThrGroup));
    }
    uint32_t w[8], wn[8];
    unsigned aux = 0u, aux_n = 0u;
    load_tile(r_lo, w, aux);
    for (int r0 = r_lo; r0 < r_hi; r0 += 32) {
      load_tile(r0 + 32, wn, aux_n);
      const bool rv = r0 + col < sz;
      asm volatile("" : "+v"(aux));
      float nrm = 0.f;
      bool live = false;
      if constexpr (NORMS)
        nrm = rv ? __uint_as_float(aux) : __builtin_nanf("");
      else
        live = rv & ((a.is_empty == nullptr) | (aux == 0u));
      f32x16 acc = zero_f32x16();
      float x2 = 0.f;
#pragma unroll
      for (int s = 0; s < KS; ++s) {
        u32x4 vh, vl;
        if constexpr (DS == 2) {
          const int j0 = 8 * s + 4 * half;
          uint2 en[4];
#pragma unroll
          for (int bb = 0; bb < 4; ++bb)
            en[bb] = reinterpret_cast<const uint2*>(book)[(j0 + bb) * 256 + (int)((w[s] >> (8 * bb)) & 255u)];
#pragma unroll
          for (int bb = 0; bb < 4 && !NORMS; ++bb) {
            const float v0 = f16_lo(en[bb].x) + f16_lo(en[bb].y), v1 = f16_hi(en[bb].x) + f16_hi(en[bb].y);
            x2 = fmaf(v0, v0, x2);
            x2 = fmaf(v1, v1, x2);
          }
          vh = u32x4{en[0].x, en[1].x, en[2].x, en[3].x};
          vl = u32x4{en[0].y, en[1].y, en[2].y, en[3].y};
        } else {
          const int j0 = 16 * s + 8 * half;
          unsigned en[8];
#pragma unroll
          for (int bb = 0; bb < 8; ++bb)
            en[bb] = book[(j0 + bb) * 256 + (int)((w[2 * s + (bb >> 2)] >> (8 * (bb & 3))) & 255u)];
#pragma unroll
          for (int bb = 0; bb < 8 && !NORMS; ++bb) {
            const float v0 = f16_lo(en[bb]) + f16_hi(en[bb]);
            x2 = fmaf(v0, v0, x2);
          }
          vh = u32x4{(en[0] & 0xffffu) | (en[1] << 16), (en[2] & 0xffffu) | (en[3] << 16),
                        (en[4] & 0xffffu) | (en[5] << 16), (en[6] & 0xffffu) | (en[7] << 16)};
          vl = u32x4{(en[0] >> 16) | (en[1] & 0xffff0000u), (en[2] >> 16) | (en[3] & 0xffff0000u),
                     (en[4] >> 16) | (en[5] & 0xffff0000u), (en[6] >> 16) | (en[7] & 0xffff0000u)};
        }
        acc = __builtin_amdgcn_mfma_f32_32x32x16_f16(__builtin_bit_cast(f16x8, vl), qh[s], acc, 0, 0, 0);
        acc = __builtin_amdgcn_mfma_f32_32x32x16_f16(__builtin_bit_cast(f16x8, vh), ql[s], acc, 0, 0, 0);
        acc = __builtin_amdgcn_mfma_f32_32x32x16_f16(__builtin_bit_cast(f16x8, vh), qh[s], acc, 0, 0, 0);
      }
      if constexpr (NORMS) {
        if (half == 0) x2w[col] = EUCLID ? nrm : nrm * 0.f;
      } else {
        x2 += __shfl_xor(x2, 32, 64);
        const float v = live ? x2 * inv_sx2 : __builtin_nanf("");
        if (half == 0) x2w[col] = EUCLID ? v : v * 0.f;
      }
      __builtin_amdgcn_fence(__ATOMIC_ACQ_REL, "wavefront");
      if constexpr (MAXIMA) {
        float gm[16 / kCellThrGroup];
#pragma unroll
        for (int g = 0; g < 16 / kCellThrGroup; ++g) gm[g] = -INFINITY;
#pragma unroll
        for (int gq = 0; gq < 4; ++gq) {
          const f32x4 x4 = *reinterpret_cast<const f32x4*>(x2w + 8 * gq + 4 * half);
#pragma unroll
          for (int i = 0; i < 4; ++i) {
            const int r = 4 * gq + i;
            gm[r / kCellThrGroup] = fmaxf(gm[r / kCellThrGroup], fmaf(acc[r], um, -x4[i]));
          }
        }
#pragma unroll
        for (int g = 0; g < 16 / kCellThrGroup; ++g) {
          const unsigned key = gm[g] == -INFINITY ? 0u : f2key(EUCLID ? gm[g] - q2 : gm[g]);
          if (me < (int)cap) mkeys[(int)cap - 1 - me] = key;
          ++me;
        }
        __builtin_amdgcn_fence(__ATOMIC_ACQ_REL, "wavefront");
#pragma unroll
        for (int i = 0; i < 8; ++i) w[i] = wn[i];
        aux = aux_n;
        continue;
      }
      float xr[16];
      bool adm[16];
      unsigned long long any[16];
#pragma unroll
      for (int gq = 0; gq < 4; ++gq) {
        const f32x4 x4 = *reinterpret_cast<const f32x4*>(x2w + 8 * gq + 4 * half);
#pragma unroll
        for (int i = 0; i < 4; ++i) {
          const int r = 4 * gq + i;
          xr[r] = x4[i];
          adm[r] = fmaf(acc[r], um, -xr[r]) >= thr2;
          any[r] = __ballot(adm[r]);
        }
      }
#pragma unroll
      for (int r = 0; r < 16; ++r) asm volatile("" ::"s"(any[r]));
#pragma unroll
      for (int r = 0; r < 16; ++r) {
        if (__builtin_expect(any[r] != 0ull, 0)) {
          if ((any[r] & __ballot(fill >= kDepth)) != 0ull) flush();
          if (adm[r]) {
            const int row = (r & 3) + 8 * (r >> 2) + 4 * half;
            float s = acc[r];
            asm volatile("" : "+v"(s));
            const float dot = s * unscale;
            const float fast = EUCLID ? (2.f * dot - xr[r]) - q2 : dot;
            stage[fill * 64] = make_uint2(f2key(fast), ~(unsigned)(st + r0 + row));
            ++fill;
          }
        }
      }
      __builtin_amdgcn_fence(__ATOMIC_ACQ_REL, "wavefront");
#pragma unroll
      for (int i = 0; i < 8; ++i) w[i] = wn[i];
      aux = aux_n;
    }
    flush();
  }
}

template <int NCH>
__global__ __launch_bounds__(256) void cell_kth_kernel(CellArgs a) {
  const int lane = (int)(threadIdx.x & 63);
  const int q = (int)blockIdx.x * 4 + (int)(threadIdx.x >> 6);
  if (q >= a.nq) return;
  const int n_all = __builtin_amdgcn_readfirstlane(a.cnt[q]);
  if (lane == 0) {
    a.cnt[q] = 0;
    if (a.n_max) a.n_max[q] = n_all;
  }
  if (a.flags[q] == a.epoch) return;
  const int cap = a.chunks * 64;
  const int n = n_all < cap ? n_all : cap;
  const unsigned* __restrict__ keys = a.keys + (int64_t)q * cap;
  unsigned hi[NCH];
#pragma unroll
  for (int t = 0; t < NCH; ++t) hi[t] = t * 64 + lane < n ? keys[cap - 1 - (t * 64 + lane)] : 0u;
  const unsigned fk = finish_fk_upto<2, NCH>(hi, (n + 63) / 64, a.thr_k);
  if (lane == 0) {
    const float t = (fk ? key2f(fk) : -INFINITY) - a.ws_delta[q];
    a.thr[q] = a.euclid ? cell_fold_threshold(t, a.qnorm[q]) : t;
  }
}

template <int DS, bool NORMS, bool MAXIMA = false>
static int launch_cand(const CellArgs& a, dim3 grid, dim3 wg, hipStream_t st) {
  return a.euclid ? launch_with_lds(cell_cand_kernel<DS, NORMS, true, MAXIMA>, "cell_cand_kernel", grid, wg, CellBook<DS>::kBytes, st, a)
                  : launch_with_lds(cell_cand_kernel<DS, NORMS, false, MAXIMA>, "cell_cand_kernel", grid, wg, CellBook<DS>::kBytes, st, a);
}

static int cell_cus() {
  int dev = 0, n_cus = 0;
  if (hipGetDevice(&dev) != hipSuccess ||
      hipDeviceGetAttribute(&n_cus, hipDeviceAttributeMultiprocessorCount, dev) != hipSuccess || n_cus <= 0)
    n_cus = 256;
  return n_cus;
}

static int launch_cell_kept_build(const CellArgs& a, hipStream_t st) {
  hipLaunchKernelGGL(cell_prep_kernel, dim3(1), dim3(1024), 0, st, a);
  TPQ_LAUNCH_CHECK("cell_prep_kernel");
  if (a.ds == 1)
    hipLaunchKernelGGL(cell_book_kernel<1>, dim3(64), dim3(256), 0, st, a);
  else
    hipLaunchKernelGGL(cell_book_kernel<2>, dim3(64), dim3(256), 0, st, a);
  TPQ_LAUNCH_CHECK("cell_book_kernel");
  const int64_t units = (a.n_slots + 511) / 512;
  if (units < 1) return TPQ_OK;
  const int n_cus = cell_cus();
  const dim3 grid((unsigned)(units < n_cus ? units : n_cus)), wg(512);
  return a.ds == 1 ? launch_with_lds(cell_norm_kernel<1, true>, "cell_norm_kernel", grid, wg, 64 * 256 * 4, st, a)
                   : launch_with_lds(cell_norm_kernel<2, true>, "cell_norm_kernel", grid, wg, 64 * 256 * 8, st, a);
}

static int launch_cell_head(const CellArgs& a, hipStream_t st) {
  if (!a.book) {
    hipLaunchKernelGGL(cell_prep_kernel, dim3(1), dim3(1024), 0, st, a);
    TPQ_LAUNCH_CHECK("cell_prep_kernel");
  } else if (a.kept_build) {
    if (int rc = launch_cell_kept_build(a, st)) return rc;
  }
  hipLaunchKernelGGL(cell_seed_kernel, dim3((unsigned)((a.nq + 3) / 4)), dim3(256), 0, st, a);
  TPQ_LAUNCH_CHECK("cell_seed_kernel");
  return TPQ_OK;
}

static std::atomic<long long> g_cell_inversions{0};
static int launch_cell_inversion(const CellArgs& a, hipStream_t st) {
  g_cell_inversions.fetch_add(1);
  const dim3 per_query((unsigned)((a.nq + 3) / 4));
  const bool lds_hist = a.n_cells <= kCellLdsCells;
  const dim3 per_slice((unsigned)((a.nq + kCellSlice - 1) / kCellSlice)), slice_wg(kCellSliceThreads);
  const size_t hist_lds = (size_t)a.n_cells * sizeof(int);
  if (a.p_a > 0) {
    hipLaunchKernelGGL(cell_count_kernel<true>, per_slice, slice_wg, 2 * hist_lds, st, a);
    TPQ_LAUNCH_CHECK("cell_count_kernel");
    hipLaunchKernelGGL(cell_scan_kernel, dim3(2), dim3(1024), 0, st, a);
    TPQ_LAUNCH_CHECK("cell_scan_kernel");
    hipLaunchKernelGGL(cell_scatter_kernel<true>, per_slice, slice_wg, 2 * hist_lds, st, a);
    TPQ_LAUNCH_CHECK("cell_scatter_kernel");
    return TPQ_OK;
  }
  if (lds_hist) {
    hipLaunchKernelGGL(cell_count_kernel<false>, per_slice, slice_wg, hist_lds, st, a);
    TPQ_LAUNCH_CHECK("cell_count_kernel");
  } else {
    hipLaunchKernelGGL(cell_count_wide_kernel, per_query, dim3(256), 0, st, a);
    TPQ_LAUNCH_CHECK("cell_count_wide_kernel");
  }
  hipLaunchKernelGGL(cell_scan_kernel, dim3(1), dim3(1024), 0, st, a);
  TPQ_LAUNCH_CHECK("cell_scan_kernel");
  if (lds_hist) {
    hipLaunchKernelGGL(cell_scatter_kernel<false>, per_slice, slice_wg, hist_lds, st, a);
    TPQ_LAUNCH_CHECK("cell_scatter_kernel");
  } else {
    hipLaunchKernelGGL(cell_scatter_wide_kernel, per_query, dim3(256), 0, st, a);
    TPQ_LAUNCH_CHECK("cell_scatter_wide_kernel");
  }
  return TPQ_OK;
}

static int launch_cell_norms(const CellArgs& a, int n_cus, hipStream_t st) {
  const dim3 norm_grid((unsigned)(a.n_cells < n_cus ? a.n_cells : n_cus)), wg(512);
  return a.ds == 1 ? launch_with_lds(cell_norm_kernel<1>, "cell_norm_kernel", norm_grid, wg, 64 * 256 * 4, st, a)
                   : launch_with_lds(cell_norm_kernel<2>, "cell_norm_kernel", norm_grid, wg, 64 * 256 * 8, st, a);
}

static unsigned cell_cand_grid(const CellArgs& a, int n_cus, bool maxima = false) {
  const int64_t np = (int64_t)a.nq * (a.p_hi > a.p0 ? a.p_hi - a.p0 : 0);
  int64_t blocks = (int64_t)a.n_cells + np / kCellGroup;
  if (blocks > np) blocks = np;
  if (blocks < 1) return 0;
  blocks = (blocks * cell_pieces(maxima) + kCellWaves - 1) / kCellWaves;
  return (unsigned)(blocks > n_cus ? n_cus : blocks);
}

static bool cell_draws_fit(const CellArgs& a) {
  const int64_t blocks = (int64_t)a.n_cells + (int64_t)a.nq * a.max_nprobe / kCellGroup;
  const int s = kCellPiecesA > kCellPiecesB ? kCellPiecesA : kCellPiecesB;
  return blocks * s + 65536 < 0x7fffffffLL;
}

int launch_cell_candidates(const CellArgs& a, hipStream_t st) {
  if (a.nq <= 0) return TPQ_OK;
  TPQ_REQUIRE(cell_draws_fit(a), "ivfpq_scan (cell-major): more pieces of blocks than the draw counter holds");
  if (int rc = launch_cell_head(a, st)) return rc;
  if (a.p_hi <= a.p0) return TPQ_OK;
  if (int rc = launch_cell_inversion(a, st)) return rc;
  const int n_cus = cell_cus();
  const dim3 grid(cell_cand_grid(a, n_cus)), cand_wg(64 * kCellWaves);
  if (a.norm) {
    if (!a.book)
      if (int rc = launch_cell_norms(a, n_cus, st)) return rc;
    return a.ds == 1 ? launch_cand<1, true>(a, grid, cand_wg, st) : launch_cand<2, true>(a, grid, cand_wg, st);
  }
  return a.ds == 1 ? launch_cand<1, false>(a, grid, cand_wg, st) : launch_cand<2, false>(a, grid, cand_wg, st);
}

void cell_fill_thr(CellThrArrays& t, void* at, int nq, int max_nprobe, int n_cells) {
  char* p = reinterpret_cast<char*>(at);
  auto take = [&](size_t bytes) {
    int* r = reinterpret_cast<int*>(p);
    p += cell_align(bytes);
    return r;
  };
  const int tp = max_nprobe < kCellThrProbes ? max_nprobe : kCellThrProbes;
  t.pairs_b = take((size_t)nq * max_nprobe * 4);
  t.hist = take((size_t)n_cells * 4);
  t.cell_off = take(((size_t)n_cells + 1) * 4);
  t.blk_off = take(((size_t)n_cells + 1) * 4);
  t.cell_st = take((size_t)n_cells * 4);
  t.cell_sz = take((size_t)n_cells * 4);
  t.pairs = take((size_t)nq * tp * 4);
  t.n_max = take((size_t)nq * 4);
}

int launch_cell_threshold(const CellArgs& a, const CellThrArrays& t, hipStream_t st) {
  if (a.nq <= 0) return TPQ_OK;
  TPQ_REQUIRE(a.norm && a.k == 0 && a.thr_k >= 1 && a.p0 == 0 && a.p_hi == a.max_nprobe && a.chunks <= 16,
              "ivfpq_scan (cell threshold): arguments outside the form");
  TPQ_REQUIRE(cell_draws_fit(a), "ivfpq_scan (cell threshold): more pieces of blocks than the draw counter holds");
  CellArgs b = a;
  b.n_max = t.n_max;
  b.pairs = t.pairs_b;
  b.hist2 = t.hist;
  b.work = 0;
  CellArgs pa = b;
  pa.p_hi = a.max_nprobe < kCellThrProbes ? a.max_nprobe : kCellThrProbes;
  pa.hist = t.hist; pa.cell_off = t.cell_off; pa.blk_off = t.blk_off; pa.cell_st = t.cell_st; pa.cell_sz = t.cell_sz;
  pa.pairs = t.pairs;
  pa.hist2 = nullptr;
  pa.work = 1;
  if (int rc = launch_cell_head(b, st)) return rc;
  const bool one_walk = a.n_cells <= kCellLdsCells / 2;
  if (one_walk) {
    b.p_a = pa.p_hi;
    b.va = CellView{t.hist, t.cell_off, t.blk_off, t.cell_st, t.cell_sz, t.pairs};
  }
  if (int rc = launch_cell_inversion(b, st)) return rc;
  b.p_a = 0;
  const int n_cus = cell_cus();
  if (!b.book)
    if (int rc = launch_cell_norms(b, n_cus, st)) return rc;
  if (!one_walk)
    if (int rc = launch_cell_inversion(pa, st)) return rc;
  const dim3 cand_wg(64 * kCellWaves);
  if (int rc = a.ds == 1 ? launch_cand<1, true, true>(pa, dim3(cell_cand_grid(pa, n_cus, true)), cand_wg, st)
                         : launch_cand<2, true, true>(pa, dim3(cell_cand_grid(pa, n_cus, true)), cand_wg, st))
    return rc;
  const dim3 per_query((unsigned)((a.nq + 3) / 4));
  if (a.chunks <= 8)
    hipLaunchKernelGGL(cell_kth_kernel<8>, per_query, dim3(256), 0, st, b);
  else
    hipLaunchKernelGGL(cell_kth_kernel<16>, per_query, dim3(256), 0, st, b);
  TPQ_LAUNCH_CHECK("cell_kth_kernel");
  const dim3 grid(cell_cand_grid(b, n_cus));
  return a.ds == 1 ? launch_cand<1, true>(b, grid, cand_wg, st) : launch_cand<2, true>(b, grid, cand_wg, st);
}

}

using namespace tpq;

extern "C" int tpq_ivfpq_cell_candidates(const uint8_t* codes, const float* query, const float* codebook, int ds,
                                         int metric, const uint8_t* is_empty, const int64_t* cell_start,
                                         const int64_t* cell_size, const int64_t* n_probe_list, const int64_t* cells,
                                         int n_cells, int first_probe, const float* threshold, int64_t n_slots, int nq,
                                         int max_nprobe, int m, int capacity, int32_t* out_count, uint32_t* out_keys,
                                         uint32_t* out_addr, float* out_delta, int32_t* out_flags, void* workspace,
                                         size_t workspace_bytes, tpq_stream_t stream) {
  TPQ_REQUIRE(codes && query && codebook && cell_start && cell_size && n_probe_list && cells && threshold &&
                  out_count && out_keys && out_addr && out_delta && out_flags,
              "ivfpq_cell_candidates: null pointer argument");
  TPQ_REQUIRE(m == 64 && (ds == 1 || ds == 2), "ivfpq_cell_candidates: m = 64 and ds <= 2 only (m=%d, ds=%d)", m, ds);
  TPQ_REQUIRE(metric == TPQ_METRIC_NEG_SQ_L2 || metric == TPQ_METRIC_INNER, "ivfpq_cell_candidates: bad metric %d",
              metric);
  TPQ_REQUIRE(nq >= 0 && max_nprobe >= 1 && n_cells >= 1 && first_probe >= 0 && n_slots >= 0 &&
                  n_slots < 0x7fffffffLL && (int64_t)nq * max_nprobe < 0x7fffffffLL,
              "ivfpq_cell_candidates: bad shape (nq=%d, max_nprobe=%d, n_cells=%d, first_probe=%d)", nq, max_nprobe,
              n_cells, first_probe);
  TPQ_REQUIRE(capacity >= 64 && capacity % 64 == 0 && capacity <= 65536,
              "ivfpq_cell_candidates: capacity=%d must be a multiple of 64 in [64, 65536]", capacity);
  const size_t need = cell_extra_bytes(nq, max_nprobe, n_cells, first_probe);
  if (!workspace || workspace_bytes < need) {
    set_error("ivfpq_cell_candidates: workspace too small (%zu < %zu)", workspace_bytes, need);
    return TPQ_ERR_WORKSPACE;
  }
  CellArgs a{};
  a.codes = codes; a.query = query; a.codebook = codebook; a.is_empty = is_empty;
  a.cell_start = cell_start; a.cell_size = cell_size; a.n_probe_list = n_probe_list; a.cells = cells;
  a.n_slots = n_slots; a.nq = nq; a.max_nprobe = max_nprobe; a.n_cells = n_cells; a.ds = ds;
  a.euclid = metric == TPQ_METRIC_NEG_SQ_L2 ? 1 : 0;
  a.p0 = first_probe; a.p_hi = max_nprobe; a.k = 0; a.chunks = capacity / 64; a.epoch = 1; a.rel = cell_delta_rel(ds);
  a.thr_in = threshold;
  a.keys = out_keys; a.idx = out_addr; a.flags = out_flags; a.ws_delta = out_delta;
  cell_fill_extras(a, workspace, workspace_bytes);
  a.cnt = out_count;
  return launch_cell_candidates(a, reinterpret_cast<hipStream_t>(stream));
}

extern "C" long long tpq_ivfpq_scan_cell_inversions(void) { return g_cell_inversions.load(); }

extern "C" float tpq_ivfpq_cell_fold_threshold(float threshold, float q2) { return cell_fold_threshold(threshold, q2); }

extern "C" size_t tpq_ivfpq_cell_candidates_workspace_bytes(int nq, int max_nprobe, int n_cells, int first_probe) {
  if (nq <= 0 || max_nprobe < 1 || n_cells < 1 || first_probe < 0) return 0;
  return cell_extra_bytes(nq, max_nprobe, n_cells, first_probe);
}

extern "C" size_t tpq_ivfpq_cell_candidates_norms_workspace_bytes(int nq, int max_nprobe, int n_cells, int first_probe,
                                                                  int64_t n_slots) {
  if (nq <= 0 || max_nprobe < 1 || n_cells < 1 || first_probe < 0 || n_slots < 0) return 0;
  return cell_extra_bytes(nq, max_nprobe, n_cells, first_probe) + cell_norm_bytes(n_slots);
}
```

torchpq_amd/csrc/scan_host.h:

```cpp
#pragma once
#include "scan_args.h"
#include "scan_packed_kernel.h"
#include "scan_finish.h"

namespace tpq {

static int pool_max_split(int m, int k) {
  const int nw = packed_waves(m), len = 64 * (nw == 4 ? 8 : 4);
  const int kcap = (k + 63) / 64 * 64;
  int s = (int)((65536 - (size_t)kcap * 8) / ((size_t)nw * len * 8));
  return s < 1 ? 1 : s;
}

constexpr int kBandSlack = 8;
static int list_regs_packed(int k) { return pow2_ceil((k + kBandSlack + 63) / 64); }
static int dump_finish_regs(int k, int64_t slots_hint) {
  const int slack = (slots_hint > 0 && slots_hint <= 16384) ? kBandSlack : 16 + k / 8;
  return pow2_ceil((k + slack + 63) / 64);
}
#ifndef TPQ_SCAN_MIN_RL_K
#define TPQ_SCAN_MIN_RL_K 1
#endif
static int list_regs_scan(int k, int m, int max_nprobe, int64_t slots_hint, int waves = 0) {
  const int nw = waves ? waves : packed_waves(m);
  const int rp = list_regs_packed(k);
  if (k < TPQ_SCAN_MIN_RL_K) return rp;
  const int64_t round_slots = (int64_t)nw * 64 * packed_slots(m);
  const bool spread = slots_hint > 0 && 4 * slots_hint >= 3 * round_slots * (max_nprobe > 0 ? max_nprobe : 1);
  const int budget = (spread ? 2 : 4) * k;
  int rl = 1;
  while (rl < rp && nw * 64 * rl < budget) rl <<= 1;
  return rl;
}

static int pool_list_regs(int k, int m) {
  const int nw = packed_waves(m);
  return pow2_ceil(((k + nw - 1) / nw + 63) / 64);
}
static int pool_capacity(int k, int m) {
  return (k <= 512 && m > 32) ? 1024 : 2048;
}

static size_t scan_lds_bytes_packed(int m, int R, int max_nprobe, int fused_floats, bool res) {
  const int nw = packed_waves(m);
  size_t b = (size_t)m * 1024 + packed_aux_bytes(R, m) + nw * 512 +
             (size_t)(3 * max_nprobe + 1) * 4 + 8 + 3 * nw * 4 + (res ? 8 * (size_t)max_nprobe : 0) +
             (size_t)fused_floats * 4;
  return (b + 15) & ~(size_t)15;
}
static size_t scan_lds_bytes_dump(int m, bool sel16, int nw, int max_nprobe, int fused_floats) {
  size_t b = (size_t)m * (sel16 ? 512 : 1024) + nw * 512 + (size_t)(3 * max_nprobe + 1) * 4 + 8 + 3 * nw * 4 +
             (size_t)fused_floats * 4;
  return (b + 15) & ~(size_t)15;
}
static int fused_floats_of(const ScanArgs& a) { return a.lut ? 0 : a.m * a.ds + a.m; }
constexpr int kFuseMaxR = 4;
static bool fuse_fits(int m, int RM) {
  const int nw = packed_waves(m);
  return RM <= kFuseMaxR &&
         (size_t)(nw + 1) * RM * 64 * 8 <= (size_t)m * 1024 + packed_aux_bytes(RM, m) + (size_t)nw * 512;
}

#ifndef TPQ_PACKED_M_LIST
#error "scan_host.h is included through scan_device.h, which defines TPQ_PACKED_M_LIST"
#endif
#define TPQ_DECLARE_PACKED(M) \
  int dispatch_packed_##M(const ScanArgs& a, const ResidualArgs* ra, int RL, int R, hipStream_t st); \
  int dispatch_pool_##M(const ScanArgs& a, int RL, hipStream_t st);                                  \
  int dispatch_dump_##M(const ScanArgs& a, int RL, int R, int mode, hipStream_t st);                 \
  int dump_occupancy_##M(int mode);                                                                  \
  int dispatch_finish_##M(const ScanArgs& a, int chunks, int R, int seed_chunks, const int* cnt, hipStream_t st);
TPQ_PACKED_M_LIST(TPQ_DECLARE_PACKED)
#undef TPQ_DECLARE_PACKED

template <class K>
static int set_lds(K kernel, size_t bytes, const char* name) {
  if (int rc = check_lds(name, bytes)) return rc;
  return check_hip(hipFuncSetAttribute(reinterpret_cast<const void*>(kernel),
                                       hipFuncAttributeMaxDynamicSharedMemorySize, (int)bytes),
                   name);
}

static size_t align256(size_t x) { return (x + 255) & ~(size_t)255; }

static size_t ws_bytes_for(int nq, int R, int n_lists) {
  return 2 * align256((size_t)nq * 4) + (size_t)nq * n_lists * R * 64 * 8 + align256((size_t)nq * n_lists * 4);
}

static size_t pool_ws_bytes(int nq, int k, int m, int n_lists) {
  return 2 * align256((size_t)nq * 4) + (size_t)nq * n_lists * pool_capacity(k, m) * 8 +
         align256((size_t)nq * n_lists * 4);
}
static void fill_ws_pool(ScanArgs& a, void* workspace, int n_lists) {
  char* p = reinterpret_cast<char*>(workspace);
  a.flags = reinterpret_cast<int*>(p);
  a.ws_delta = reinterpret_cast<float*>(p + align256((size_t)a.nq * 4));
  char* pools = p + 2 * align256((size_t)a.nq * 4);
  a.pool_cap = pool_capacity(a.k, a.m);
  const size_t n = (size_t)a.nq * n_lists * a.pool_cap;
  a.pool_hi = reinterpret_cast<unsigned*>(pools);
  a.pool_lo = reinterpret_cast<unsigned*>(pools + n * 4);
  a.pool_cnt = reinterpret_cast<int*>(pools + n * 8);
}

static void fill_ws(ScanArgs& a, void* workspace, int R, int n_lists) {
  char* p = reinterpret_cast<char*>(workspace);
  a.flags = reinterpret_cast<int*>(p);
  a.ws_delta = reinterpret_cast<float*>(p + align256((size_t)a.nq * 4));
  char* lists = p + 2 * align256((size_t)a.nq * 4);
  a.ws_vals = reinterpret_cast<float*>(lists);
  a.ws_idx = reinterpret_cast<int*>(lists + (size_t)a.nq * n_lists * R * 64 * 4);
  a.list_evict = reinterpret_cast<int*>(lists + (size_t)a.nq * n_lists * R * 64 * 8);
}

static int validate(const ScanArgs& a) {
  TPQ_REQUIRE(a.codes && (a.lut || (a.query && a.codebook)) && a.cell_start && a.cell_size &&
                  a.n_probe_list && a.out_vals && a.out_addr,
              "ivfpq_scan: null pointer argument");
  TPQ_REQUIRE(a.lut || a.ds >= 1, "ivfpq_scan: bad sub-vector length %d", a.ds);
  TPQ_REQUIRE(a.nq >= 0 && a.max_nprobe >= 1, "ivfpq_scan: bad nq/max_nprobe (%d, %d)", a.nq,
              a.max_nprobe);
  TPQ_REQUIRE(a.m >= 4 && a.m % 4 == 0, "ivfpq_scan: n_subvectors=%d must be a positive multiple of 4", a.m);
  TPQ_REQUIRE(a.k >= 1 && a.k <= 1024, "ivfpq_scan: k=%d out of range (0, 1024]", a.k);
  TPQ_REQUIRE(a.n_slots >= 0 && a.n_slots < 0x7fffffffLL, "ivfpq_scan: n_slots=%lld out of range",
              (long long)a.n_slots);
  TPQ_REQUIRE(a.n_split >= 1 && a.n_split <= 1024, "ivfpq_scan: n_split=%d out of range", a.n_split);
  TPQ_REQUIRE((a.out_ids == nullptr) || (a.address2id != nullptr),
              "ivfpq_scan: out_ids given without address2id");
  return TPQ_OK;
}

}
```

torchpq_amd/fn/IVFPQTopk.py:

```python
from ..kernels import IVFPQTopkHip


class IVFPQTopk:
    def __init__(self, n_subvectors, contiguous_size=4, sm_size=None):
        self.n_subvectors = n_subvectors
        self.contiguous_size = contiguous_size
        self._scan = IVFPQTopkHip(m=n_subvectors, n_cs=contiguous_size)

    def topk(self, data, precomputed, cell_start, cell_size, is_empty, n_probe_list, k=256,
             packed=None, address2id=None, slots_hint=None):
        assert 0 < k <= 1024
        return self._scan.topk(data=data, precomputed=precomputed, is_empty=is_empty,
                               cell_start=cell_start, cell_size=cell_size,
                               n_probe_list=n_probe_list, n_candidates=k, packed=packed,
                               address2id=address2id, slots_hint=slots_hint)

    def topk_fused(self, data, query, codebook, cell_start, cell_size, is_empty, n_probe_list, k=256,
                   distance="euclidean", packed=None, address2id=None, slots_hint=None, cells=None, n_cells=0,
                   cell_threshold=True, kept=None):
        assert 0 < k <= 1024
        return self._scan.topk_fused(data=data, query=query, codebook=codebook, is_empty=is_empty,
                                     cell_start=cell_start, cell_size=cell_size,
                                     n_probe_list=n_probe_list, n_candidates=k, distance=distance,
                                     packed=packed, address2id=address2id, slots_hint=slots_hint,
                                     cells=cells, n_cells=n_cells, cell_threshold=cell_threshold, kept=kept)

    def topk_residual(self, data, precomputed, cell_start, cell_size, base_sims, is_empty,
                      n_probe_list, k=256, address2id=None):
        assert 0 < k <= 1024
        return self._scan.topk_residual(data=data, precomputed=precomputed, base_sims=base_sims,
                                        is_empty=is_empty, cell_start=cell_start,
                                        cell_size=cell_size, n_probe_list=n_probe_list,
                                        n_candidates=k, address2id=address2id)

    def topk_residual_precomputed(self, data, part1, part2, cell_start, cell_size, cells, base_sims,
                                  is_empty, n_probe_list=None, k=256, address2id=None):
        assert 0 < k <= 1024
        return self._scan.topk_residual_precomputed(
            data=data, part1=part1, part2=part2, cells=cells, base_sims=base_sims,
            is_empty=is_empty, cell_start=cell_start, cell_size=cell_size,
            n_probe_list=n_probe_list, n_candidates=k, address2id=address2id)
```

torchpq_amd/index/IVFPQIndex.py:

```python
import torch

from .. import util
from ..codec import PQCodec
from ..container import CellContainer
from ..fn import IVFPQTopk
from ..kernels import PACKED_M, CellKeptState, IVFPQFilteredTopkHip, IVFPQRangeHip, ResidualPart1Hip, ResidualSlotTermsHip
from ._coarse import CoarseProbeMixin
from ._filter import IdFilter, filtered_search_batches
from ._range import range_search_batches


class IVFPQIndex(CoarseProbeMixin, CellContainer):
    packed_min_subvectors = 0
    packed_max_short_subvectors = 24
    fused_lut_max_subvector = 4
    use_cell_major = True
    use_cell_threshold = True
    use_cell_kept = True

    def __init__(self, d_vector, n_subvectors=8, n_cells=128, initial_size=None,
                 expand_step_size=128, expand_mode="double", distance="euclidean",
                 device="cuda:0", pq_use_residual=False, verbose=0):
        if torch.device(device).type == "cuda":
            assert torch.cuda.is_available(), "cuda is not available"
            assert n_subvectors <= util.max_subvectors()
        assert d_vector % n_subvectors == 0
        assert n_subvectors % 4 == 0, "codes are stored 4 sub-quantizers per word (contiguous_size=4)"
        assert distance in ("euclidean", "cosine"), \
            "euclidean and cosine work end to end (MultiKMeans.py:82-113)"
        super().__init__(code_size=n_subvectors, n_cells=n_cells, dtype="uint8", device=device,
                         initial_size=initial_size, expand_step_size=expand_step_size,
                         expand_mode=expand_mode, use_inverse_id_mapping=True, contiguous_size=4,
                         verbose=verbose)
        self.d_vector = d_vector
        self.n_subvectors = n_subvectors
        self.d_subvector = d_vector // n_subvectors
        self.distance = distance
        self.verbose = verbose
        self.pq_use_residual = pq_use_residual
        self._use_precomputed = bool(pq_use_residual and
                                     (n_cells * 256 * n_subvectors * 4) <= 4 * 1024 ** 3)
        self._precomputed_part2 = None
        self._part2_by_cell = None
        self._slot_terms = None
        self._use_cublas = True
        self._use_tensor_core = False
        self._fp16_scale_mode = "a"
        self.use_packed_layout = True
        self.use_fused_lut = True
        self.use_cell_major = True
        self.use_cell_threshold = True
        self.use_cell_kept = True
        self._cell_kept = None
        self._cell_kept_built = 0

        self._init_coarse(n_cells, verbose)
        self.pq_codec = PQCodec(d_vector=d_vector, n_subvectors=n_subvectors, n_clusters=256,
                                distance=distance, verbose=verbose)
        self._ivfpq_topk = IVFPQTopk(n_subvectors=n_subvectors, contiguous_size=self.contiguous_size)
        self._ivfpq_range = IVFPQRangeHip(m=n_subvectors)
        self._ivfpq_filtered = IVFPQFilteredTopkHip(m=n_subvectors)
        self.to(device)

    @property
    def use_cublas(self):
        return self._use_cublas

    @use_cublas.setter
    def use_cublas(self, value):
        assert type(value) is bool
        self._use_cublas = value

    @property
    def use_tensor_core(self):
        return self._use_tensor_core

    @use_tensor_core.setter
    def use_tensor_core(self, value):
        assert type(value) is bool
        assert self.use_cublas
        self._use_tensor_core = value
        self._coarse_probe.route = "fp16" if value else "auto"

    @property
    def fp16_scale_mode(self):
        return self._fp16_scale_mode

    @fp16_scale_mode.setter
    def fp16_scale_mode(self, value):
        assert value in ["a", "b", "both", "none"]
        self._fp16_scale_mode = value

    @property
    def use_precomputed(self):
        return self._use_precomputed

    @use_precomputed.setter
    def use_precomputed(self, value):
        assert type(value) is bool
        if value:
            assert self.pq_use_residual, " `use_precomputed=True` is only valid when `pq_use_residual` is True"
            assert (self.pq_codec.is_trained and self.vq_codec.is_trained), "index is not trained"
            self.precompute_part2()
        else:
            self._drop_part2()
        self._use_precomputed = value

    def _drop_part2(self):
        self._precomputed_part2 = None
        self._part2_by_cell = None
        self._slot_terms = None

    def precompute_part2(self):
        pq_codebook = self.pq_codec.codebook
        vq_codebook = self.vq_codec.codebook.reshape(self.n_subvectors, self.d_subvector, self.n_cells)
        part2 = (torch.bmm(vq_codebook.transpose(-1, -2), pq_codebook) * -2
                 - pq_codebook.norm(dim=1).pow(2)[:, None])
        self._part2_by_cell = part2.transpose(0, 1).contiguous()
        del part2
        self._precomputed_part2 = self._part2_by_cell.transpose(0, 1)
        self._slot_terms = None

    def _residual_slot_terms(self):
        if self._slot_terms is None or self._slot_terms[0] != self._codes_version:
            st, cb = ResidualSlotTermsHip()(self._storage, self._part2_by_cell, self._cell_start,
                                            self._cell_size)
            self._slot_terms = (self._codes_version, st, cb)
        return self._slot_terms[1], self._slot_terms[2]

    def _codec_knob(codec, attr, typed):
        def getter(self):
            return getattr(getattr(self, codec).kmeans, attr)

        def setter(self, value):
            if typed:
                assert type(value) is int
                assert value > 0
            assert not getattr(self, codec).is_trained, f"{codec} is already trained"
            setattr(getattr(self, codec).kmeans, attr, value)
        return property(getter, setter)

    vq_codec_max_iter = _codec_knob("vq_codec", "max_iter", True)
    vq_codec_n_redo = _codec_knob("vq_codec", "n_redo", True)
    vq_codec_tolerance = _codec_knob("vq_codec", "tol", False)
    pq_codec_max_iter = _codec_knob("pq_codec", "max_iter", True)
    pq_codec_n_redo = _codec_knob("pq_codec", "n_redo", True)
    pq_codec_tolerance = _codec_knob("pq_codec", "tol", False)
    del _codec_knob

    def _cell_kept_state(self, n_bytes, device):
        def ident(t):
            return None if t is None else (t.data_ptr(), tuple(t.shape), util.tensor_version(t), str(t.device))
        key = (self._codes_version, bool(self._has_holes), ident(self.pq_codec.codebook), ident(self._storage),
               ident(self._is_empty))
        st = self._cell_kept
        if st is not None and st.key == key and st.buf.numel() >= n_bytes and st.buf.device == torch.device(device):
            return st
        if torch.cuda.is_current_stream_capturing():
            return None
        self._drop_cell_kept()
        self._cell_kept = CellKeptState(n_bytes, device, key)
        return self._cell_kept

    def _drop_cell_kept(self):
        if self._cell_kept is not None:
            self._cell_kept_built += self._cell_kept.builds
        self._cell_kept = None

    @property
    def cell_kept_builds(self):
        return self._cell_kept_built + (0 if self._cell_kept is None else self._cell_kept.builds)

    def to(self, *args, **kwargs):
        if getattr(self, "_cell_kept", None) is not None:
            self._drop_cell_kept()
        return super().to(*args, **kwargs)

    def _after_load_state_dict(self):
        self.to(self.device)
        self._drop_part2()
        self._drop_cell_kept()
        super()._after_load_state_dict()

    def train(self, x, force_retrain=False):
        if self.vq_codec.is_trained and self.pq_codec.is_trained and not force_retrain:
            self.print_message("index is already trained", 1)
            return
        x = self._prepare(x)
        self.print_message("start training VQ codec...", 1)
        code = self.vq_codec.train(x)
        self.print_message("start training PQ codec...", 1)
        if self.pq_use_residual:
            self.pq_codec.train((x - self.vq_codec.decode(code)).contiguous())
            self._drop_part2()
        else:
            self.pq_codec.train(x)
        self.print_message("index is trained successfully!", 1)

    def encode(self, x):
        x = self._prepare(x)
        if self.pq_use_residual:
            return self._encode_raw(x)
        return self.pq_codec.encode(x)

    def decode(self, x):
        if self.pq_use_residual:
            assert len(x) == 2
            pq_code, vq_code = x
            assert pq_code.shape[0] == self.n_subvectors
            assert pq_code.shape[1] == vq_code.shape[0]
            return self.vq_codec.decode(vq_code.to(self.device)) + self.pq_codec.decode(pq_code.to(self.device))
        assert len(x.shape) == 2
        assert x.shape[0] == self.n_subvectors
        return self.pq_codec.decode(x.to(self.device))

    def add(self, x, ids=None, return_address=False):
        x = self._prepare(x)
        if self.pq_use_residual:
            codes, assigned_cells = self._encode_raw(x)
        else:
            assigned_cells = self.vq_codec.encode(x)
            codes = self.pq_codec.encode(x)
        return super().add(codes, cells=assigned_cells, ids=ids, return_address=return_address)

    def _encode_raw(self, x):
        vq_code = self.vq_codec.encode(x)
        return self.pq_codec.encode((x - self.vq_codec.decode(vq_code)).contiguous()), vq_code

    def precomputed_adc_residual_precomputed(self, x):
        part1 = ResidualPart1Hip()(x, self.pq_codec.codebook)
        if self._precomputed_part2 is None:
            self.precompute_part2()
        return part1, self._part2_by_cell

    def precomputed_adc_residual(self, x, cells):
        n_query, n_probe = cells.shape
        pq_codebook = self.pq_codec.codebook
        xs = x.reshape(self.n_subvectors, self.d_subvector, n_query).transpose(-1, -2)
        part1 = 2 * (xs @ pq_codebook).permute(1, 0, 2) - pq_codebook.norm(dim=1).pow(2)[None]
        vq = self.vq_codec.codebook.reshape(self.n_subvectors, self.d_subvector, self.n_cells)
        vq = vq[:, :, cells].permute(0, 2, 3, 1)
        part2 = -2 * (vq @ pq_codebook[:, None].expand(-1, n_query, -1, -1))
        return (part1[:, None] + part2.permute(1, 2, 0, 3)).contiguous()

    def _scan_layout(self):
        m = self.n_subvectors
        if self.use_packed_layout and m in PACKED_M and (
                m >= self.packed_min_subvectors or m <= self.packed_max_short_subvectors):
            return self.packed_storage()
        return None

    def search_cells(self, x, cells, base_sims=None, n_probe_list=None, k=1, return_address=False,
                     _extents=None):
        n_probe_list, cell_start, cell_size, slots_hint, is_empty = self._scan_preamble(x, cells, n_probe_list,
                                                                                        _extents)
        lists = dict(data=self._scan_codes(), cell_start=cell_start, cell_size=cell_size, is_empty=is_empty,
                     n_probe_list=n_probe_list, address2id=self._address2id)
        fused = self.use_fused_lut and self.d_subvector <= self.fused_lut_max_subvector
        if self.pq_use_residual:
            assert base_sims is not None, "base_sims is required when pq_use_residual is True"
            if self.use_precomputed and self.use_packed_layout and self.n_subvectors in PACKED_M:
                if self._precomputed_part2 is None:
                    self.precompute_part2()
                slot_term, cell_bound = self._residual_slot_terms()
                part1 = None if fused else self.precomputed_adc_residual_precomputed(x)[0]
                found = self._ivfpq_topk._scan.topk_residual_packed(
                    packed=self.packed_storage(), part2=self._part2_by_cell, slot_term=slot_term,
                    cell_bound=cell_bound, cells=cells, base_sims=base_sims, n_candidates=k, part1=part1,
                    query=x if fused else None, codebook=self.pq_codec.codebook if fused else None,
                    slots_hint=slots_hint, **lists)
            elif self.use_precomputed:
                part1, part2 = self.precomputed_adc_residual_precomputed(x)
                found = self._ivfpq_topk.topk_residual_precomputed(
                    part1=part1, part2=part2, cells=cells, base_sims=base_sims, k=k, **lists)
            else:
                found = self._ivfpq_topk.topk_residual(
                    base_sims=base_sims, precomputed=self.precomputed_adc_residual(x, cells), k=k, **lists)
        elif fused:
            found = self._ivfpq_topk.topk_fused(
                packed=self._scan_layout(), query=x, codebook=self.pq_codec.codebook, k=k, distance=self.distance,
                slots_hint=slots_hint, cells=cells if self.use_cell_major else None, n_cells=self.n_cells,
                cell_threshold=self.use_cell_threshold,
                kept=self._cell_kept_state if self.use_cell_kept and self.use_cell_major else None, **lists)
        else:
            found = self._ivfpq_topk.topk(
                packed=self._scan_layout(), precomputed=self.pq_codec.precompute_adc(x), k=k,
                slots_hint=slots_hint, **lists)
        topk_val, topk_address, topk_ids = found
        return (topk_val, topk_ids, topk_address) if return_address else (topk_val, topk_ids)

    def graphed_search(self, n_query, k=1):
        from .graphed import GraphedSearch
        return GraphedSearch(self, n_query, k)

    def search(self, x, k=1, return_address=False):
        x = self._prepare(x)
        assert 0 < k <= 1024
        assert self.vq_codec.is_trained and self.pq_codec.is_trained, "index is not trained"
        assert 1 <= self.n_probe <= self.n_cells
        return self._search_batches(x, lambda xb, sims, cells, n_probe_list, extents: self.search_cells(
            x=xb, cells=cells, base_sims=sims, n_probe_list=n_probe_list, k=k, return_address=False,
            _extents=extents))

    def range_search_cells(self, x, cells, threshold, base_sims=None, n_probe_list=None, return_address=False,
                           _extents=None):
        n_probe_list, cell_start, cell_size, slots_hint, is_empty = self._scan_preamble(x, cells, n_probe_list,
                                                                                        _extents)
        lists = dict(data=self._scan_codes(), cell_start=cell_start.contiguous(), cell_size=cell_size.contiguous(),
                     n_probe_list=n_probe_list, threshold=threshold, is_empty=is_empty)
        fused = self.use_fused_lut and self.d_subvector <= self.fused_lut_max_subvector
        if self.pq_use_residual:
            assert base_sims is not None, "base_sims is required when pq_use_residual is True"
            if self.use_precomputed:
                if self._precomputed_part2 is None:
                    self.precompute_part2()
                tables = dict(part2=self._part2_by_cell, cells=cells)
                if fused:
                    tables.update(query=x, codebook=self.pq_codec.codebook)
                else:
                    tables.update(part1=ResidualPart1Hip()(x, self.pq_codec.codebook))
            else:
                tables = dict(full=self.precomputed_adc_residual(x, cells))
            lims, vals, address = self._ivfpq_range.residual(base_sims=base_sims, **tables, **lists)
        elif fused:
            lims, vals, address = self._ivfpq_range(query=x, codebook=self.pq_codec.codebook, distance=self.distance,
                                                    slots_hint=slots_hint, **lists)
        else:
            lims, vals, address = self._ivfpq_range(precomputed=self.pq_codec.precompute_adc(x),
                                                    slots_hint=slots_hint, **lists)
        ids = self.get_id_by_address(address) if address.numel() else torch.empty_like(address)
        return (lims, vals, ids, address) if return_address else (lims, vals, ids)

    def range_search(self, x, threshold, return_address=False, sort=False):
        x = self._prepare(x)
        assert self.vq_codec.is_trained and self.pq_codec.is_trained, "index is not trained"
        assert 1 <= self.n_probe <= self.n_cells
        return range_search_batches(
            self, x, threshold, lambda xb, thr, sims, cells, n_probe_list, extents: self.range_search_cells(
                xb, cells, thr, base_sims=sims, n_probe_list=n_probe_list, return_address=True, _extents=extents),
            return_address, sort)

    def id_filter(self, ids):
        return IdFilter(self, ids)

    def search_cells_filtered(self, x, cells, flt, filter_of_query=None, base_sims=None, n_probe_list=None, k=1,
                              return_address=False, _extents=None):
        n_probe_list, cell_start, cell_size, slots_hint, is_empty = self._scan_preamble(x, cells, n_probe_list,
                                                                                        _extents)
        lists = dict(data=self._scan_codes(), cell_start=cell_start, cell_size=cell_size, n_probe_list=n_probe_list,
                     k=k, filter_bits=flt.bits(self), filter_of_query=filter_of_query, is_empty=is_empty,
                     address2id=self._address2id)
        fused = self.use_fused_lut and self.d_subvector <= self.fused_lut_max_subvector
        if self.pq_use_residual:
            assert base_sims is not None, "base_sims is required when pq_use_residual is True"
            if self.use_precomputed:
                if self._precomputed_part2 is None:
                    self.precompute_part2()
                tables = dict(part2=self._part2_by_cell, cells=cells)
                if fused:
                    tables.update(query=x, codebook=self.pq_codec.codebook)
                else:
                    tables.update(part1=ResidualPart1Hip()(x, self.pq_codec.codebook))
            else:
                tables = dict(full=self.precomputed_adc_residual(x, cells))
            vals, address, ids = self._ivfpq_filtered.residual(base_sims=base_sims, **tables, **lists)
        elif fused:
            vals, address, ids = self._ivfpq_filtered(query=x, codebook=self.pq_codec.codebook,
                                                      distance=self.distance, slots_hint=slots_hint, **lists)
        else:
            vals, address, ids = self._ivfpq_filtered(precomputed=self.pq_codec.precompute_adc(x),
                                                      slots_hint=slots_hint, **lists)
        return (vals, ids, address) if return_address else (vals, ids)

    def search_filtered(self, x, k, flt, filter_of_query=None):
        x = self._prepare(x)
        assert 0 < k <= 1024
        assert self.vq_codec.is_trained and self.pq_codec.is_trained, "index is not trained"
        assert 1 <= self.n_probe <= self.n_cells
        return filtered_search_batches(
            self, x, flt, filter_of_query, lambda xb, rows, sims, cells, n_probe_list, extents:
            self.search_cells_filtered(xb, cells, flt, filter_of_query=rows, base_sims=sims,
                                       n_probe_list=n_probe_list, k=k, _extents=extents))
```

torchpq_amd/index/graphed.py:

```python
import torch

from ..util import tensor_version


class GraphedSearch:

    KNOBS = ("n_probe", "use_smart_probing", "_smart_probing_temperature", "use_packed_layout",
             "use_fused_lut", "use_cell_major", "use_cell_threshold", "use_cell_kept", "use_fused_probe", "use_cublas", "_use_precomputed", "pq_use_residual",
             "distance", "max_query_batch", "_has_holes", "_codes_version")

    @staticmethod
    def _buffers(index):
        slot = index._slot_terms
        kept = getattr(index, "_cell_kept", None)
        return {
            "vq_codebook": index.vq_codec.codebook, "pq_codebook": index.pq_codec.codebook,
            "_storage": index._storage, "_packed": index._packed if index._packed_valid else None,
            "_is_empty": index._is_empty, "_address2id": index._address2id,
            "_cell_start": index._cell_start, "_cell_size": index._cell_size,
            "_part2_by_cell": index._part2_by_cell,
            "slot_term": None if slot is None else slot[1],
            "cell_bound": None if slot is None else slot[2],
            "cell_kept": None if kept is None or not kept.valid else kept.buf,
        }

    @classmethod
    def _snapshot(cls, index):
        knobs = tuple(getattr(index, name) for name in cls.KNOBS)
        bufs = cls._buffers(index)
        ident = tuple((name, None if t is None else (t.data_ptr(), tuple(t.shape), tensor_version(t)))
                      for name, t in bufs.items())
        return knobs, ident, bufs

    def __init__(self, index, n_query, k, warmup=2):
        assert n_query >= 1
        self.index = index
        self.n_query = n_query
        self.k = k
        device = torch.device(index.device)
        self.x = torch.zeros(index.d_vector, n_query, device=device, dtype=torch.float32)
        self._tickets = torch.zeros(max(n_query, 1), device=device, dtype=torch.int32)
        scan = index._ivfpq_topk._scan
        side = torch.cuda.Stream(device=device)
        side.wait_stream(torch.cuda.current_stream(device))
        prev = scan.ticket_buffer
        scan.ticket_buffer = self._tickets
        try:
            with torch.cuda.stream(side):
                for _ in range(warmup):
                    index.search(self.x, k=k)
            torch.cuda.current_stream(device).wait_stream(side)
            self.graph = torch.cuda.CUDAGraph()
            with torch.cuda.graph(self.graph):
                self.values, self.ids = index.search(self.x, k=k)
        finally:
            scan.ticket_buffer = prev
        self._knobs, self._ident, self._held = self._snapshot(index)

    def stale_reason(self):
        knobs, ident, _ = self._snapshot(self.index)
        for name, old, new in zip(self.KNOBS, self._knobs, knobs):
            if old != new:
                return f"{name} changed ({old!r} -> {new!r})"
        for (name, old), (_, new) in zip(self._ident, ident):
            if old != new:
                return f"buffer {name} was replaced or written"
        return None

    def __call__(self, x):
        assert x.shape == self.x.shape, f"graph was captured for queries of shape {tuple(self.x.shape)}"
        why = self.stale_reason()
        if why is not None:
            raise RuntimeError(f"the index changed since the graph was captured ({why}): "
                               "call index.graphed_search() again")
        self.x.copy_(x, non_blocking=True)
        self.graph.replay()
        return self.values, self.ids
```

torchpq_amd/kernels/scan.py:

```python
import torch

from .._lib import check, load, ptr, require_gpu, stream_ptr
from ._common import alloc_pair, alloc_topk, call, metric_code, topk_result, workgroups_per_query

PACKED_M = (4, 8, 12, 16, 20, 24, 28, 32, 40, 48, 56, 64, 96, 120, 128)


def packed_chunk_width(m):
    return 16 if m % 16 == 0 else (8 if m % 8 == 0 else 4)


class CellKeptState:

    def __init__(self, n_bytes, device, key=None):
        self.buf = torch.empty(n_bytes, device=device, dtype=torch.uint8)
        self.key = key
        self.valid = False
        self.builds = 0
        self.ready = None

    def before_use(self, device):
        if self.valid and not torch.cuda.is_current_stream_capturing():
            torch.cuda.current_stream(device).wait_event(self.ready)

    def after_build(self, device):
        stream = torch.cuda.current_stream(device)
        self.ready = torch.cuda.Event()
        self.ready.record(stream)
        self.valid = True
        self.builds += 1


class IVFPQTopkHip:

    def __init__(self, m=8, k=256, tpb=256, n_cs=4, stack_capacity=2, sm_size=None):
        assert k == 256
        assert n_cs == 4
        assert m % n_cs == 0
        self.m = m
        self.k = k
        self.tpb = tpb
        self.n_cs = n_cs
        self.n_cus = None
        self.record_events = None
        self.last_n_split = None
        self.ticket_buffer = None
        self._ticket_cache = {}
        self.keep_workspace = False
        self.last_workspace = None
        self.last_call = None
        self.workspace_bytes = None
        self.last_workspace_bytes = None
        self._last_device = None
        self._last_cells = None
        self._last_withheld = False
        self.last_cell_kept = None

    def _tickets(self, n_query, n_split, device):
        if n_split <= 1:
            return None
        if self.ticket_buffer is not None:
            t = self.ticket_buffer
            assert t.dtype == torch.int32 and t.numel() >= n_query and t.device == torch.device(device)
            return t
        if torch.cuda.is_current_stream_capturing():
            return None
        dev = torch.device(device)
        key = (dev.index, torch.cuda.current_stream(dev).cuda_stream)
        t = self._ticket_cache.get(key)
        if t is None or t.numel() < n_query:
            if len(self._ticket_cache) >= 64:
                self._ticket_cache.clear()
            t = torch.zeros(max(n_query, 1024), device=dev, dtype=torch.int32)
            self._ticket_cache[key] = t
        return t

    def _drop_tickets(self, device):
        dev = torch.device(device)
        self._ticket_cache.pop((dev.index, torch.cuda.current_stream(dev).cuda_stream), None)

    def last_redone(self, n_query):
        ws = self.last_workspace
        route = self.last_route()
        if ws is None or route in (None, "reference_layout", "rejected"):
            return None
        off = (n_query * 4 + 255) // 256 * 256
        d = ws[off:off + 4 * n_query].view(torch.float32)
        return int((d == (1.0 if route == "one_launch_finish" else -1.0)).sum().item())

    ROUTES = {0: "reference_layout", 1: "one_launch_finish", 2: "sorted_lists", 3: "pools", 8: "dump_f32",
              16: "dump_sel16", 17: "dump_sel16_w8", -1: "rejected"}

    def route(self, n_query, k, n_split=1, ds=0, n_probe=1, slots_hint=None, has_lut=True, packed=True,
              tickets=None, residual=False):
        if tickets is None:
            tickets = n_split > 1
        code = load().tpq_ivfpq_scan_route(int(n_query), int(k), int(n_split), self.m, int(ds), int(n_probe),
                                            int(slots_hint or 0), int(bool(has_lut)),
                                            int(bool(packed) and self.m in PACKED_M), int(bool(tickets)),
                                            int(bool(residual)))
        return self.ROUTES.get(code, str(code))

    def last_route(self):
        return None if self.last_call is None else self.route(**self.last_call)

    def ordered(self, workspace_bytes, slots=0):
        if self.last_call is None:
            return None
        c = self.last_call
        with torch.cuda.device(self._last_device):
            code = load().tpq_ivfpq_scan_ordered(int(c["n_query"]), int(c["k"]), int(c["n_split"]), self.m, int(c["ds"]),
                                                  int(c["n_probe"]), int(c["slots_hint"] or 0), int(bool(c["has_lut"])),
                                                  int(bool(c["packed"]) and self.m in PACKED_M), int(c["n_split"] > 1),
                                                  int(bool(c.get("residual", False))), int(slots), int(workspace_bytes))
        return code == 1

    def last_ordered(self):
        return None if self.last_call is None else self.ordered(self.last_workspace_bytes)

    def _cell_query(self, name, workspace_bytes, n_cells, n_slots):
        if self.last_call is None:
            return None
        c = self.last_call
        code = getattr(load(), name)(int(c["n_query"]), int(c["k"]), int(c["n_split"]), self.m, int(c["ds"]),
                                     int(c["n_probe"]), int(c["slots_hint"] or 0), int(bool(c["has_lut"])),
                                     int(bool(c["packed"]) and self.m in PACKED_M), int(c["n_split"] > 1),
                                     int(bool(c.get("residual", False))), int(n_cells), int(n_slots),
                                     int(workspace_bytes))
        return code == 1

    def cell_major(self, workspace_bytes, n_cells, n_slots):
        return self._cell_query("tpq_ivfpq_scan_cell_major", workspace_bytes, n_cells, n_slots)

    def cell_norms(self, workspace_bytes, n_cells, n_slots):
        return self._cell_query("tpq_ivfpq_scan_cell_norms", workspace_bytes, n_cells, n_slots)

    def last_cell_major(self):
        if self.last_call is None:
            return None
        if self._last_cells is None:
            return False
        return self.cell_major(self.last_workspace_bytes, *self._last_cells)

    def last_cell_norms(self):
        if self.last_call is None:
            return None
        if self._last_cells is None:
            return False
        return self.cell_norms(self.last_workspace_bytes, *self._last_cells)

    def cell_threshold(self, workspace_bytes, n_cells, n_slots):
        return self._cell_query("tpq_ivfpq_scan_cell_threshold", workspace_bytes, n_cells, n_slots)

    def last_cell_threshold(self):
        if self.last_call is None:
            return None
        if self._last_cells is None or self._last_withheld:
            return False
        return self.cell_threshold(self.last_workspace_bytes, *self._last_cells)

    def last_cell_threshold_state(self):
        assert self.last_workspace is not None and self.last_cell_threshold() is True
        ws, c = self.last_workspace, self.last_call
        nq, k, n_probe = c["n_query"], c["k"], c["n_probe"]
        n_cells, n_slots = self._last_cells
        align = lambda n: (n + 255) // 256 * 256
        lists = lambda ch: 2 * align(nq * 4) + nq * ch * 512 + align(nq * ch * 4)
        extras = load().tpq_ivfpq_cell_candidates_workspace_bytes(nq, n_probe, n_cells, 4)
        chunks = next(ch for ch in (16, 8) if (k + 63) // 64 < ch and self.last_workspace_bytes >= lists(ch) + extras)
        cap = chunks * 64

        def arr(off, n, dtype):
            return ws[off:off + 4 * n].view(dtype)
        band = arr(align(nq * 4), nq, torch.float32).clone()
        keys = arr(2 * align(nq * 4), nq * cap, torch.int32).view(nq, cap)
        ex = lists(chunks) + 256
        thr, qnorm, cand = (arr(ex + i * align(nq * 4), nq, t).clone()
                            for i, t in ((0, torch.float32), (2, torch.float32), (3, torch.int32)))
        t_probes = load().tpq_ivfpq_scan_cell_threshold_probes()
        off = (lists(chunks) + extras + align(n_slots * 4) + align(nq * n_probe * 4) + 3 * align(n_cells * 4)
               + 2 * align((n_cells + 1) * 4) + align(nq * min(t_probes, n_probe) * 4))
        count = arr(off, nq, torch.int32).clone()
        e = torch.arange(cap, device=ws.device)[None, :]
        stored = e < count.clamp(max=cap)[:, None]
        rev = keys.flip(1)
        bits = torch.where(rev < 0, rev & 0x7fffffff, ~rev).view(torch.float32)
        maxima = torch.where(stored, bits, torch.full_like(bits, -float("inf")))
        maxima = torch.where(stored & (rev == 0), torch.full_like(bits, float("nan")), maxima)
        survived = stored & (cap - 1 - e >= cand.clamp(max=cap)[:, None])
        return dict(count=count, maxima=maxima, survived=survived, threshold=thr, band=band, qnorm=qnorm,
                    candidates=cand)

    def _n_split(self, n_query, device, slots_hint=None):
        if self.n_cus is None:
            self.n_cus = torch.cuda.get_device_properties(device).multi_processor_count
        per_cu, waves = (4, 4) if self.m <= 32 else (2, 8) if self.m <= 64 else (1, 16)
        return workgroups_per_query(n_query, self.n_cus, per_cu, waves, slots_hint)

    def _scan(self, name, inputs, data, cell_start, address2id, k, n_split, slots_hint, packed, ticketed,
              cells=None, n_cells=0, cell_threshold=True, kept=None, **route):
        n_data, device = data.shape[1], data.device
        n_query, n_probe = cell_start.shape
        values, address, ids = alloc_topk(n_query, k, device, address2id)
        if n_query == 0:
            return topk_result(values, address, ids)
        lib = load()
        if n_split is None:
            n_split = self._n_split(n_query, device, slots_hint)
        self.last_n_split = n_split
        self.last_call = dict(n_query=n_query, k=k, n_split=n_split, n_probe=n_probe, slots_hint=slots_hint,
                              packed=packed is not None, **route)
        self._last_cells = (int(n_cells), int(n_data)) if cells is not None else None
        self._last_withheld = not cell_threshold
        ws_bytes = lib.tpq_ivfpq_scan_workspace_bytes(n_query, k, n_split, self.m)
        if self.workspace_bytes is not None:
            ws_bytes = int(self.workspace_bytes)
        self.last_workspace_bytes, self._last_device = ws_bytes, device
        ws = torch.empty(max(ws_bytes, 1), device=device, dtype=torch.uint8)
        self.last_cell_kept = None
        if kept is not None and cells is not None and self.cell_norms(ws_bytes, n_cells, n_data):
            kept = kept(lib.tpq_ivfpq_cell_kept_bytes(int(n_data), int(route["ds"])), device)
            if kept is not None and not kept.valid and torch.cuda.is_current_stream_capturing():
                kept = None
        else:
            kept = None
        ev = None
        if self.record_events is not None:
            ev = (torch.cuda.Event(enable_timing=True), torch.cuda.Event(enable_timing=True))
            ev[0].record(torch.cuda.current_stream(device))
        with torch.cuda.device(device):
            tail = ()
            if ticketed:
                tickets = self._tickets(n_query, n_split, device) if packed is not None else None
                tail = (ptr(tickets), int(slots_hint or 0))
                if cells is not None:
                    tail += (ptr(cells), int(n_cells))
                if kept is not None:
                    name = "tpq_ivfpq_search_fused_cells_kept"
                    kept.before_use(device)
                    tail += (ptr(kept.buf), kept.buf.numel(), int(kept.valid))
            before = lib.tpq_ivfpq_scan_use_cell_threshold(1 if cell_threshold else 0)
            try:
                rc = getattr(lib, name)(*inputs, ptr(values), ptr(address), ptr(address2id), ptr(ids), n_data, n_query,
                                        n_probe, self.m, k, n_split, ptr(ws), ws_bytes, *tail, stream_ptr(device))
            finally:
                lib.tpq_ivfpq_scan_use_cell_threshold(before)
            if rc != 0 and ticketed:
                self._drop_tickets(device)
            check(rc, name)
            if kept is not None:
                self.last_cell_kept = "reused" if kept.valid else "built"
                if not kept.valid:
                    kept.after_build(device)
        if self.keep_workspace:
            self.last_workspace = ws
        if ev is not None:
            ev[1].record(torch.cuda.current_stream(device))
            self.record_events.append(ev)
        return topk_result(values, address, ids)

    def topk(self, data, precomputed, is_empty, cell_start, cell_size, n_probe_list,
             n_candidates=None, packed=None, address2id=None, n_split=None, slots_hint=None):
        n_data = data.shape[1]
        n_query, n_probe = cell_start.shape
        assert precomputed.shape == (self.m, n_query, self.k)
        assert data.shape[0] == self.m // self.n_cs
        assert data.shape[2] == self.n_cs
        assert cell_size.shape[1] == n_probe
        assert data.dtype == torch.uint8
        assert precomputed.dtype == torch.float32
        assert cell_start.dtype == cell_size.dtype == torch.int64
        assert n_probe_list.shape == (n_query,)
        assert n_probe_list.dtype == torch.int64
        if is_empty is not None:
            assert is_empty.shape[0] == n_data
            assert is_empty.dtype == torch.uint8
        if n_candidates is None:
            n_candidates = self.tpb
        assert 0 < n_candidates <= 1024
        require_gpu(data, precomputed, is_empty, cell_start, cell_size, n_probe_list, packed,
                    address2id)
        inputs = (ptr(data), ptr(precomputed), ptr(is_empty), ptr(cell_start), ptr(cell_size), ptr(n_probe_list))
        if packed is not None and self.m in PACKED_M:
            return self._scan("tpq_ivfpq_scan_topk_packed_tickets", (ptr(packed), *inputs), data, cell_start,
                              address2id, n_candidates, n_split, slots_hint, packed, True, ds=0, has_lut=True)
        return self._scan("tpq_ivfpq_scan_topk", inputs, data, cell_start, address2id, n_candidates, n_split,
                          slots_hint, packed, False, ds=0, has_lut=True)

    def topk_fused(self, data, query, codebook, is_empty, cell_start, cell_size, n_probe_list,
                   n_candidates, distance="euclidean", packed=None, address2id=None, n_split=None,
                   slots_hint=None, cells=None, n_cells=0, cell_threshold=True, kept=None):
        n_data = data.shape[1]
        n_query, n_probe = cell_start.shape
        m, ds, kk = codebook.shape
        assert m == self.m and kk == self.k
        assert query.shape == (m * ds, n_query)
        assert query.dtype == codebook.dtype == torch.float32
        assert data.shape == (self.m // self.n_cs, n_data, self.n_cs) and data.dtype == torch.uint8
        assert cell_size.shape == (n_query, n_probe)
        assert cell_start.dtype == cell_size.dtype == torch.int64
        assert n_probe_list.shape == (n_query,) and n_probe_list.dtype == torch.int64
        assert 0 < n_candidates <= 1024
        query = query.contiguous()
        codebook = codebook.contiguous()
        require_gpu(data, query, codebook, is_empty, cell_start, cell_size, n_probe_list, packed,
                    address2id)
        inputs = (ptr(packed), ptr(data), ptr(query), ptr(codebook), ds, metric_code(distance), ptr(is_empty),
                  ptr(cell_start), ptr(cell_size), ptr(n_probe_list))
        if cells is not None:
            assert cells.shape == (n_query, n_probe) and cells.dtype == torch.int64 and n_cells >= 1
            cells = cells.contiguous()
            require_gpu(cells)
            return self._scan("tpq_ivfpq_search_fused_cells", inputs, data, cell_start, address2id, n_candidates,
                              n_split, slots_hint, packed, True, cells=cells, n_cells=n_cells, cell_threshold=cell_threshold,
                              kept=kept, ds=ds, has_lut=False)
        return self._scan("tpq_ivfpq_search_fused_tickets", inputs, data, cell_start, address2id, n_candidates,
                          n_split, slots_hint, packed, True, ds=ds, has_lut=False)

    def _residual(self, data, part1, part2, full, cells, base_sims, is_empty, cell_start, cell_size,
                  n_probe_list, n_candidates, address2id):
        n_data = data.shape[1]
        n_query, n_probe = cell_start.shape
        assert data.shape == (self.m // self.n_cs, n_data, self.n_cs)
        assert cell_size.shape == (n_query, n_probe)
        assert base_sims.shape == (n_query, n_probe)
        assert data.dtype == torch.uint8
        assert cell_start.dtype == cell_size.dtype == torch.int64
        assert base_sims.dtype == torch.float32
        assert n_probe_list.shape == (n_query,)
        assert n_probe_list.dtype == torch.int64
        if is_empty is not None:
            assert is_empty.shape == (n_data,) and is_empty.dtype == torch.uint8
        if n_candidates is None:
            n_candidates = self.tpb
        assert 0 < n_candidates <= 1024
        part1 = None if part1 is None else part1.contiguous()
        part2 = None if part2 is None else part2.contiguous()
        full = None if full is None else full.contiguous()
        cells = None if cells is None else cells.contiguous()
        base_sims = base_sims.contiguous()
        require_gpu(data, part1, part2, full, cells, base_sims, is_empty, cell_start, cell_size,
                    n_probe_list, address2id)
        k = n_candidates
        values, address, ids = alloc_topk(n_query, k, data.device, address2id)
        if n_query:
            call("tpq_ivfpq_scan_topk_residual", data.device,
                 ptr(data), ptr(part1), ptr(part2), ptr(full), ptr(cells), ptr(base_sims),
                 ptr(is_empty), ptr(cell_start), ptr(cell_size), ptr(n_probe_list), ptr(values),
                 ptr(address), ptr(address2id), ptr(ids), n_data, n_query, n_probe, self.m, k)
        return topk_result(values, address, ids)

    def topk_residual_packed(self, data, packed, part2, slot_term, cell_bound, cells, base_sims,
                             is_empty, cell_start, cell_size, n_probe_list, n_candidates,
                             part1=None, query=None, codebook=None, address2id=None, n_split=None,
                             slots_hint=None):
        n_data = data.shape[1]
        n_query, n_probe = cell_start.shape
        assert self.m in PACKED_M and packed is not None
        assert data.shape == (self.m // self.n_cs, n_data, self.n_cs) and data.dtype == torch.uint8
        assert part2.shape[1:] == (self.m, self.k) and part2.dtype == torch.float32
        assert part2.is_contiguous()
        assert slot_term.shape == (n_data,) and slot_term.dtype == torch.float32
        assert cell_bound.shape == (part2.shape[0],) and cell_bound.dtype == torch.float32
        assert cells.shape == cell_start.shape == cell_size.shape == base_sims.shape
        assert cells.dtype == cell_start.dtype == cell_size.dtype == torch.int64
        assert base_sims.dtype == torch.float32
        assert n_probe_list.shape == (n_query,) and n_probe_list.dtype == torch.int64
        assert 0 < n_candidates <= 1024
        ds = 0
        if part1 is not None:
            assert part1.shape == (n_query, self.m, self.k) and part1.dtype == torch.float32
            part1 = part1.contiguous()
        else:
            assert query is not None and codebook is not None
            ds = codebook.shape[1]
            assert codebook.shape == (self.m, ds, self.k) and query.shape == (self.m * ds, n_query)
            assert query.dtype == codebook.dtype == torch.float32
            query = query.contiguous()
            codebook = codebook.contiguous()
        cells = cells.contiguous()
        base_sims = base_sims.contiguous()
        require_gpu(data, packed, part1, query, codebook, part2, slot_term, cell_bound, cells,
                    base_sims, is_empty, cell_start, cell_size, n_probe_list, address2id)
        inputs = (ptr(packed), ptr(data), ptr(part1), ptr(query), ptr(codebook), ds, ptr(part2), ptr(slot_term),
                  ptr(cell_bound), ptr(cells), ptr(base_sims), ptr(is_empty), ptr(cell_start), ptr(cell_size),
                  ptr(n_probe_list))
        return self._scan("tpq_ivfpq_scan_topk_residual_packed", inputs, data, cell_start, address2id,
                          n_candidates, n_split, slots_hint, packed, False, ds=ds, has_lut=part1 is not None,
                          residual=True)

    def topk_residual(self, data, precomputed, base_sims, is_empty, cell_start, cell_size,
                      n_probe_list, n_candidates=None, address2id=None):
        n_query, n_probe = cell_start.shape
        assert precomputed.shape == (n_query, n_probe, self.m, self.k)
        assert precomputed.dtype == torch.float32
        return self._residual(data, None, None, precomputed, None, base_sims, is_empty, cell_start,
                              cell_size, n_probe_list, n_candidates, address2id)

    def topk_residual_precomputed(self, data, part1, part2, cells, base_sims, is_empty, cell_start,
                                  cell_size, n_probe_list, n_candidates=None, address2id=None):
        n_query = cell_start.shape[0]
        assert part1.shape == (n_query, self.m, self.k) and part2.shape[1:] == (self.m, self.k)
        assert part1.dtype == part2.dtype == torch.float32
        assert cells.shape == cell_start.shape and cells.dtype == torch.int64
        return self._residual(data, part1, part2, None, cells, base_sims, is_empty, cell_start,
                              cell_size, n_probe_list, n_candidates, address2id)


class CellCandidatesHip:

    def __call__(self, data, query, codebook, cells, n_cells, cell_start, cell_size, n_probe_list, threshold,
                 first_probe=0, capacity=1024, is_empty=None, distance="euclidean", slot_norms=True):
        m, ds, kk = codebook.shape
        n_data = data.shape[1]
        n_query, n_probe = cell_start.shape
        assert m == 64 and kk == 256 and ds in (1, 2) and query.shape == (m * ds, n_query)
        assert data.shape == (16, n_data, 4) and data.dtype == torch.uint8
        assert cells.shape == cell_size.shape == (n_query, n_probe)
        assert cells.dtype == cell_start.dtype == cell_size.dtype == n_probe_list.dtype == torch.int64
        assert threshold.shape == (n_query,) and threshold.dtype == torch.float32
        query, codebook, cells = query.contiguous(), codebook.contiguous(), cells.contiguous()
        require_gpu(data, query, codebook, cells, is_empty, cell_start, cell_size, n_probe_list, threshold)
        dev = data.device
        count = torch.zeros(n_query, device=dev, dtype=torch.int32)
        keys = torch.zeros(n_query, capacity, device=dev, dtype=torch.int32)
        addr = torch.zeros(n_query, capacity, device=dev, dtype=torch.int32)
        band = torch.zeros(n_query, device=dev, dtype=torch.float32)
        flags = torch.zeros(n_query, device=dev, dtype=torch.int32)
        if slot_norms:
            ws_bytes = load().tpq_ivfpq_cell_candidates_norms_workspace_bytes(n_query, n_probe, int(n_cells),
                                                                              int(first_probe), n_data)
        else:
            ws_bytes = load().tpq_ivfpq_cell_candidates_workspace_bytes(n_query, n_probe, int(n_cells), int(first_probe))
        ws = torch.empty(max(ws_bytes, 1), device=dev, dtype=torch.uint8)
        call("tpq_ivfpq_cell_candidates", dev, ptr(data), ptr(query), ptr(codebook), ds, metric_code(distance),
             ptr(is_empty), ptr(cell_start), ptr(cell_size), ptr(n_probe_list), ptr(cells), int(n_cells),
             int(first_probe), ptr(threshold), n_data, n_query, n_probe, m, int(capacity), ptr(count), ptr(keys),
             ptr(addr), ptr(band), ptr(flags), ptr(ws), ws_bytes)
        address = (~addr).to(torch.int64)
        stored = torch.arange(capacity, device=dev)[None, :] < count.clamp(max=capacity)[:, None]
        address = torch.where(stored, address, torch.full_like(address, -1))
        neg = keys < 0
        bits = torch.where(neg, keys & 0x7fffffff, ~keys)
        values = torch.where(stored, bits.view(torch.float32), torch.full_like(band[:, None].expand_as(bits), -float("inf")))
        return count, values, address, band, flags


class ScanOrderHip:

    def __call__(self, cell_start, cell_size, n_probe_list, tile_shift=6):
        n_query, n_probe = cell_start.shape
        assert cell_size.shape == (n_query, n_probe) and n_probe >= 1
        assert cell_start.dtype == cell_size.dtype == torch.int64
        assert n_probe_list.shape == (n_query,) and n_probe_list.dtype == torch.int64
        require_gpu(cell_start, cell_size, n_probe_list)
        order, rank, work = (torch.empty(n_query, device=cell_start.device, dtype=torch.int32) for _ in range(3))
        if n_query:
            call("tpq_ivfpq_scan_order", cell_start.device, ptr(cell_start), ptr(cell_size), ptr(n_probe_list),
                 n_query, n_probe, int(tile_shift), ptr(order), ptr(rank), ptr(work))
        return order, rank, work


class ResidualSlotTermsHip:

    def __call__(self, data, part2, cell_start, cell_size):
        n_cells, m, kk = part2.shape
        n_data = data.shape[1]
        assert kk == 256 and data.shape == (m // 4, n_data, 4) and data.dtype == torch.uint8
# ... 621 lines not shown
```

Baseline: 12.83 million queries/s.

## Use single-product f16 candidate keys in cell-threshold scan for ds=2

Adds a single-product mode to the cell-major candidate kernel for ds=2. It multiplies only the f16 high part of the query against an f16 codebook, instead of three split-precision products, which halves the LDS codebook footprint and allows 12 waves instead of 8. To keep candidate filtering safe, the prep kernel computes per-piece codebook norm maxima and the per-query error bound delta is widened accordingly. The finish stage gets a larger register budget to absorb the extra candidates that pass the looser bound. The risk is more false candidates to re-rank and extra prep work.

```diff
diff --git a/__graft_entry__.py b/__graft_entry__.py
--- a/__graft_entry__.py
+++ b/__graft_entry__.py
@@ -120,6 +120,18 @@
     print(f"scan_flat.hip: {len(rows)} scan_flat_kernel instantiations, no register spills, at most 72 VGPRs")
 
 
+def check_scan_cells_registers() -> None:
+    if os.environ.get("TPQ_SKIP_HAZARD_CHECK", "0") == "1":
+        return
+    out = subprocess.run([sys.executable, os.path.join(ROOT, "tools", "kernel_regs.py"), "scan_cells.hip", "--grep",
+                          "cell_cand_kernel"], capture_output=True, text=True, check=True).stdout
+    rows = [line for line in out.splitlines() if "cell_cand_kernel<2, true, " in line and ", 1>" in line]
+    assert len(rows) == 4, out
+    bad = [line for line in rows if " spill   0 scratch    0 " not in line or int(line.split(" vgpr ")[1].split()[0]) > 128]
+    assert not bad, f"single-product cell_cand_kernel spills registers, uses scratch or exceeds 128 VGPRs: {bad}"
+    print(f"scan_cells.hip: {len(rows)} single-product cell_cand_kernel instantiations, no register spills, no scratch")
+
+
 def build() -> None:
     subprocess.check_call(["bash", os.path.join(ROOT, "torchpq_amd", "csrc", "build.sh")])
     subprocess.check_call(["make", "-C", os.path.join(ROOT, "oracle"), "libivfpq_oracle.so"])
@@ -132,6 +144,7 @@
     check_scan_pq4_filtered_registers()
     check_scan_pq4_range_registers()
     check_scan_flat_registers()
+    check_scan_cells_registers()
     import torchpq_amd
     from torchpq_amd import _lib
     lib = _lib.load()
diff --git a/include/torchpq_amd.h b/include/torchpq_amd.h
--- a/include/torchpq_amd.h
+++ b/include/torchpq_amd.h
@@ -112,6 +112,9 @@
                                   int64_t n_slots, size_t workspace_bytes);
 int tpq_ivfpq_scan_use_cell_threshold(int on);
 int tpq_ivfpq_scan_cell_threshold_probes(void);
+#define TPQ_HAS_IVFPQ_CELL_SINGLE_PRODUCT 1
+int tpq_ivfpq_scan_use_cell_single_product(int on);
+int tpq_ivfpq_scan_last_cell_products(void);
 #define TPQ_HAS_IVFPQ_CELL_KEPT 1
 size_t tpq_ivfpq_cell_kept_bytes(int64_t n_slots, int ds);
 long long tpq_ivfpq_scan_cell_inversions(void);
diff --git a/torchpq_amd/_lib.py b/torchpq_amd/_lib.py
--- a/torchpq_amd/_lib.py
+++ b/torchpq_amd/_lib.py
@@ -54,6 +54,8 @@
     "tpq_ivfpq_scan_cell_threshold": (_i, [_i, _i, _i, _i, _i, _i, _i64, _i, _i, _i, _i, _i, _i64, _sz]),
     "tpq_ivfpq_scan_use_cell_threshold": (_i, [_i]),
     "tpq_ivfpq_scan_cell_threshold_probes": (_i, []),
+    "tpq_ivfpq_scan_use_cell_single_product": (_i, [_i]),
+    "tpq_ivfpq_scan_last_cell_products": (_i, []),
     "tpq_ivfpq_scan_topk_residual": (_i, [_vp, _vp, _vp, _vp, _vp, _vp, _vp, _vp, _vp, _vp, _vp, _vp,
                                           _vp, _vp, _i64, _i, _i, _i, _i, _vp]),
     "tpq_residual_part1": (_i, [_vp, _vp, _vp, _i, _i, _i, _vp]),
diff --git a/torchpq_amd/csrc/scan.hip b/torchpq_amd/csrc/scan.hip
--- a/torchpq_amd/csrc/scan.hip
+++ b/torchpq_amd/csrc/scan.hip
@@ -286,6 +286,11 @@
   plan_dump_dispatch(p, nq, slots > 0 ? slots : dump_slots(*packed_unit(m), p.mode), workspace_bytes);
   return p.ordered ? 1 : 0;
 }
+
+static std::atomic<int> g_cell_single_product{1};
+static std::atomic<int> g_cell_products{0};
+extern "C" int tpq_ivfpq_scan_use_cell_single_product(int on) { return g_cell_single_product.exchange(on ? 1 : 0); }
+extern "C" int tpq_ivfpq_scan_last_cell_products(void) { return g_cell_products.load(); }
 
 struct CellMajor {
   const int64_t* cells;
@@ -345,6 +350,8 @@
   c.n_slots = a.n_slots; c.nq = nq; c.max_nprobe = a.max_nprobe; c.n_cells = cm.n_cells; c.ds = a.ds;
   c.euclid = a.euclid; c.p0 = kCellP0; c.p_hi = a.max_nprobe; c.k = a.k; c.chunks = chunks; c.epoch = a.epoch;
   c.rel = cell_delta_rel(a.ds);
+  c.products = 3;
+  g_cell_products.store(3);
   c.seed_vals = a.out_vals; c.seed_addr = a.out_addr;
   c.keys = reinterpret_cast<unsigned*>(a.ws_vals); c.idx = reinterpret_cast<unsigned*>(a.ws_idx);
   c.list_evict = a.list_evict; c.flags = a.flags; c.ws_delta = a.ws_delta;
@@ -376,7 +383,9 @@
   c.cell_start = a.cell_start; c.cell_size = a.cell_size; c.n_probe_list = a.n_probe_list; c.cells = cm.cells;
   c.n_slots = a.n_slots; c.nq = nq; c.max_nprobe = a.max_nprobe; c.n_cells = cm.n_cells; c.ds = a.ds;
   c.euclid = a.euclid; c.p0 = 0; c.p_hi = a.max_nprobe; c.k = 0; c.thr_k = a.k; c.chunks = chunks; c.epoch = a.epoch;
-  c.rel = cell_delta_rel(a.ds);
+  c.products = g_cell_single_product.load() && cell_single_product_built(a.ds) ? 1 : 3;
+  c.rel = c.products == 1 ? cell_delta1_rel(a.ds) : cell_delta_rel(a.ds);
+  g_cell_products.store(c.products);
   c.keys = reinterpret_cast<unsigned*>(a.ws_vals); c.idx = reinterpret_cast<unsigned*>(a.ws_idx);
   c.list_evict = a.list_evict; c.flags = a.flags; c.ws_delta = a.ws_delta;
   char* at = reinterpret_cast<char*>(workspace) + ws_bytes_for(nq, 1, chunks);
@@ -387,7 +396,8 @@
   cell_fill_thr(t, at + head, nq, a.max_nprobe, cm.n_cells);
   int rc = launch_cell_threshold(c, t, st);
   if (rc) return rc;
-  return u.finish(a, chunks, p.Rf, 0, c.cnt, st);
+  const int Rf1 = c.products == 1 ? cell_single_finish_regs(a.k) : 0;
+  return u.finish(a, chunks, Rf1 > p.Rf ? Rf1 : p.Rf, 0, c.cnt, st);
 }
 
 extern "C" int tpq_ivfpq_scan_cell_major(int nq, int k, int n_split, int m, int ds, int max_nprobe, int64_t slots_hint,
@@ -434,6 +444,7 @@
   int rc = validate(a);
   if (rc) return rc;
   TPQ_REQUIRE(a.packed != nullptr, "ivfpq_scan_packed: null packed pointer");
+  g_cell_products.store(0);
   if (a.nq == 0) return TPQ_OK;
   hipStream_t st = reinterpret_cast<hipStream_t>(stream);
   ScanPlan p = plan_scan(a, ra != nullptr);
diff --git a/torchpq_amd/csrc/scan_cells.h b/torchpq_amd/csrc/scan_cells.h
--- a/torchpq_amd/csrc/scan_cells.h
+++ b/torchpq_amd/csrc/scan_cells.h
@@ -86,7 +86,9 @@
   float* kparams;
   unsigned* book;
   int kept_build;
+  int products;
 };
+constexpr int kCellPieceMaxAt = 64;
 inline size_t cell_book_bytes(int ds) { return (size_t)64 * 256 * 4 * ds; }
 inline size_t cell_kept_bytes(int64_t n_slots, int ds) {
   return 256 + cell_book_bytes(ds) + ((((size_t)(n_slots > 0 ? n_slots : 0) * 4) + 255) & ~(size_t)255);
@@ -157,6 +159,8 @@
 
 void cell_fill_extras(CellArgs& a, void* at, size_t room, int layout_p0 = -1);
 float cell_delta_rel(int ds);
+float cell_delta1_rel(int ds);
+inline bool cell_single_product_built(int ds) { return ds == 2; }
 int launch_cell_candidates(const CellArgs& a, hipStream_t st);
 void cell_fill_thr(CellThrArrays& t, void* at, int nq, int max_nprobe, int n_cells);
 int launch_cell_threshold(const CellArgs& a, const CellThrArrays& t, hipStream_t st);
diff --git a/torchpq_amd/csrc/scan_cells.hip b/torchpq_amd/csrc/scan_cells.hip
--- a/torchpq_amd/csrc/scan_cells.hip
+++ b/torchpq_amd/csrc/scan_cells.hip
@@ -11,6 +11,13 @@
 float cell_delta_rel(int ds) {
   const double D = 64.0 * ds, N = 3.0 * D, u = 1.0 / 16777216.0;
   const double sum = 0.5 * (3.03 * 4 * u + 1.003 * N * 2 * u) + 1.01 * std::sqrt(D) * u / 4 + (D + 1) * u + 14 * u + 4 * u +
+                     1.001 * (64 + ds + 2) * u;
+  return (float)(1.25 * sum * (1.0 + 1.0 / 1024));
+}
+
+float cell_delta1_rel(int ds) {
+  const double D = 64.0 * ds, N = D, u = 1.0 / 16777216.0;
+  const double sum = 0.5 * (2.03 * 4 * u + 1.003 * N * 2 * u) + 1.01 * std::sqrt(D) * u / 4 + (D + 1) * u + 14 * u + 4 * u +
                      1.001 * (64 + ds + 2) * u;
   return (float)(1.25 * sum * (1.0 + 1.0 / 1024));
 }
@@ -81,9 +88,45 @@
   return mb;
 }
 
+template <int DS>
+__device__ __forceinline__ void prep_piece_maxima(const float* __restrict__ codebook, float sx, int lane, int wave,
+                                                  float* xh2_s, float* xl2_s) {
+#pragma unroll
+  for (int jj = 0; jj < 4; ++jj) {
+    float hm = 0.f, lm = 0.f;
+#pragma unroll
+    for (int cc = 0; cc < 4; ++cc) {
+      float h2 = 0.f, l2 = 0.f;
+#pragma unroll
+      for (int e = 0; e < DS; ++e) {
+        const float ys = codebook[((wave + 16 * jj) * DS + e) * 256 + lane + 64 * cc] * sx;
+        const _Float16 h = (_Float16)ys;
+        const float hf = (float)h, lf = (float)(_Float16)(ys - hf);
+        h2 = fmaf(hf, hf, h2);
+        l2 = fmaf(lf, lf, l2);
+      }
+      hm = fmaxf(hm, h2);
+      lm = fmaxf(lm, l2);
+    }
+#pragma unroll
+    for (int d = 32; d > 0; d >>= 1) {
+      hm = fmaxf(hm, __shfl_xor(hm, d, 64));
+      lm = fmaxf(lm, __shfl_xor(lm, d, 64));
+    }
+    if (lane == 0) {
+      xh2_s[wave + 16 * jj] = hm;
+      xl2_s[wave + 16 * jj] = lm;
+    }
+  }
+}
+__device__ __forceinline__ unsigned short piece_max16(float sq_norm) {
+  return (unsigned short)((__float_as_uint(sqrtf(sq_norm) * 1.0001f) + 0xffffu) >> 16);
+}
+__device__ __forceinline__ float piece_max_of(unsigned short w) { return __uint_as_float((unsigned)w << 16); }
+
 __global__ __launch_bounds__(1024) void cell_prep_kernel(CellArgs a) {
   __shared__ unsigned maxbits_s;
-  __shared__ float c2max_s[64];
+  __shared__ float c2max_s[64], xh2_s[64], xl2_s[64], sx_s;
   const int tid = (int)threadIdx.x, lane = tid & 63, wave = tid >> 6;
   if (tid == 0) maxbits_s = 0u;
   __syncthreads();
@@ -102,6 +145,19 @@
     a.kparams[1] = x2;
     a.kparams[2] = ok ? 1.f : 0.f;
     a.kparams[3] = ok ? pow2i(kCellScaleExp - e) : 0.f;
+    sx_s = ok ? pow2i(kCellScaleExp - e) : 0.f;
+  }
+  __syncthreads();
+  if (a.ds == 1)
+    prep_piece_maxima<1>(a.codebook, sx_s, lane, wave, xh2_s, xl2_s);
+  else
+    prep_piece_maxima<2>(a.codebook, sx_s, lane, wave, xh2_s, xl2_s);
+  __syncthreads();
+  if (tid < 64) {
+    const float* s = tid < 32 ? xh2_s : xl2_s;
+    const int i = tid & 31;
+    unsigned short* out = reinterpret_cast<unsigned short*>(reinterpret_cast<char*>(a.kparams) + kCellPieceMaxAt);
+    out[tid] = piece_max16(fmaxf(s[2 * i], s[2 * i + 1]));
   }
 }
 
@@ -164,8 +220,29 @@
     }
     return;
   }
+  const float sq = pow2i(kCellScaleExp - eq);
+  const float y0 = x0 * sq, y1 = x1 * sq;
+  const _Float16 h0 = (_Float16)y0, h1 = (_Float16)y1;
+  const _Float16 l0 = (_Float16)(y0 - (float)h0), l1 = (_Float16)(y1 - (float)h1);
   const float B = sqrtf(q2) * 1.000001f + sqrtf(a.kparams[1]) * 1.000001f;
-  const float delta = a.rel * (B * B);
+  float delta = a.rel * (B * B);
+  if (a.products == 1) {
+    const unsigned short* pm =
+        reinterpret_cast<const unsigned short*>(reinterpret_cast<const char*>(a.kparams) + kCellPieceMaxAt);
+    auto subq_norm = [&](_Float16 v) {
+      float s = (float)v * (float)v;
+      if (a.ds == 2) s += __shfl_xor(s, 1, 64);
+      return sqrtf(s) * 1.000001f;
+    };
+    const float nh0 = subq_norm(h0), nl0 = subq_norm(l0), nh1 = subq_norm(h1), nl1 = subq_norm(l1);
+    const int i0 = lane / (2 * a.ds), i1 = a.ds == 2 ? 16 + (lane >> 2) : 0;
+    float t = fmaf(piece_max_of(pm[i0]), nl0, piece_max_of(pm[32 + i0]) * (nh0 + nl0)) +
+              fmaf(piece_max_of(pm[i1]), nl1, piece_max_of(pm[32 + i1]) * (nh1 + nl1));
+    if (a.ds == 2 && (lane & 1)) t = 0.f;
+#pragma unroll
+    for (int d = 32; d > 0; d >>= 1) t += __shfl_xor(t, d, 64);
+    delta = fmaf(1.25f * 1.0001f * t, 2.f / (sq * a.kparams[3]), delta);
+  }
   if (lane == 0) {
     if (a.thr_k == 0) a.thr[q] = a.euclid ? cell_fold_threshold(tau - delta, q2) : tau - delta;
     a.ws_delta[q] = 2.f * delta;
@@ -176,17 +253,14 @@
   }
   if (a.list_evict && lane < a.chunks) a.list_evict[(int64_t)q * a.chunks + lane] = 0;
   {
-    const float sq = pow2i(kCellScaleExp - eq);
     _Float16* qs = a.qsplit + (int64_t)q * kCellQSplit;
-    const float y0 = x0 * sq, y1 = x1 * sq;
-    const _Float16 h0 = (_Float16)y0, h1 = (_Float16)y1;
     if (lane < D) {
       qs[lane] = h0;
-      qs[128 + lane] = (_Float16)(y0 - (float)h0);
+      qs[128 + lane] = l0;
     }
     if (64 + lane < D) {
       qs[64 + lane] = h1;
-      qs[192 + lane] = (_Float16)(y1 - (float)h1);
+      qs[192 + lane] = l1;
     }
   }
   const int64_t base = (int64_t)q * a.chunks * 64;
@@ -342,15 +416,21 @@
 #define TPQ_CELL_WAVES 8
 #endif
 constexpr int kCellWaves = TPQ_CELL_WAVES;
+#ifndef TPQ_CELL_WAVES1
+#define TPQ_CELL_WAVES1 12
+#endif
+constexpr int kCellWaves1 = TPQ_CELL_WAVES1;
+constexpr int cell_waves(int products) { return products == 1 ? kCellWaves1 : kCellWaves; }
 constexpr size_t kCellLdsBytes = 160 * 1024;
-template <int DS>
+template <int DS, int PRODUCTS = 3>
 struct CellBook {
   static constexpr int KS = 4 * DS;
-  static constexpr size_t kBook = (size_t)64 * 256 * 4 * DS;
-  static constexpr int kWaves = kCellWaves;
+  static constexpr size_t kBook = (size_t)64 * 256 * (PRODUCTS == 1 ? 2 : 4) * DS;
+  static constexpr int kWaves = cell_waves(PRODUCTS);
   static constexpr int kThreads = 64 * kWaves;
   static constexpr size_t kNorms = (size_t)kWaves * 32 * 4;
-  static constexpr int kDepth = (int)((kCellLdsBytes - (size_t)64 * 256 * 8 - kNorms) / ((size_t)kWaves * 64 * 8));
+  static constexpr int kDepth = (int)((kCellLdsBytes - (PRODUCTS == 1 ? kBook : (size_t)64 * 256 * 8) - kNorms) /
+                                      ((size_t)kWaves * 64 * 8));
   static constexpr size_t kBytes = kBook + kNorms + (size_t)kWaves * 64 * kDepth * 8;
   static_assert(kDepth >= 1 && kBytes <= kCellLdsBytes, "the staging area does not fit the CU's LDS");
 };
@@ -451,10 +531,11 @@
   }
 }
 
-template <int DS, bool NORMS, bool EUCLID, bool MAXIMA = false>
-__global__ __launch_bounds__(CellBook<DS>::kThreads) void cell_cand_kernel(CellArgs a) {
+template <int DS, bool NORMS, bool EUCLID, bool MAXIMA = false, int PRODUCTS = 3>
+__global__ __launch_bounds__(64 * cell_waves(PRODUCTS)) void cell_cand_kernel(CellArgs a) {
   static_assert(!MAXIMA || NORMS, "pass A reads the slot norms");
-  using T = CellBook<DS>;
+  static_assert(PRODUCTS == 3 || (PRODUCTS == 1 && DS == 2 && NORMS), "the single-product key: ds = 2 with slot norms");
+  using T = CellBook<DS, PRODUCTS>;
   constexpr int S = cell_pieces(MAXIMA);
   constexpr int KS = T::KS;
   constexpr int kDepth = T::kDepth;
@@ -470,7 +551,20 @@
   const float inv_sx = 1.f / sx;
   const float inv_sx2 = inv_sx * inv_sx;
   const uint8_t* __restrict__ emp = a.is_empty ? a.is_empty : a.codes;
-  if (a.book) {
+  if constexpr (PRODUCTS == 1) {
+    if (a.book) {
+      const u32x4* __restrict__ img = reinterpret_cast<const u32x4*>(a.book);
+      for (int i = tid; i < 64 * 256 / 2; i += T::kThreads) {
+        const u32x4 v = img[i];
+        reinterpret_cast<uint2*>(book)[i] = make_uint2(v[0], v[2]);
+      }
+    } else {
+      for (int i = tid; i < 64 * 256; i += T::kThreads) {
+        const int j = i >> 8, c = i & 255;
+        book[i] = pack_f16x2((_Float16)(a.codebook[(j * 2) * 256 + c] * sx), (_Float16)(a.codebook[(j * 2 + 1) * 256 + c] * sx));
+      }
+    }
+  } else if (a.book) {
     const u32x4* __restrict__ img = reinterpret_cast<const u32x4*>(a.book);
     for (int i = tid; i < (int)(T::kBook / 16); i += T::kThreads) reinterpret_cast<u32x4*>(book)[i] = img[i];
   } else {
@@ -514,13 +608,14 @@
     const float q2 = qvalid ? a.qnorm[q] : 0.f;
     const float unscale = qvalid ? (1.f / sq) * inv_sx : 0.f;
     const float um = EUCLID ? 2.f * unscale : unscale;
-    f16x8 qh[KS], ql[KS];
+    f16x8 qh[KS], ql[PRODUCTS == 3 ? KS : 1];
     const _Float16* __restrict__ qs = a.qsplit + (int64_t)q * kCellQSplit + 8 * half;
 #pragma unroll
     for (int s = 0; s < KS; ++s) {
       const u32x4 z = {0u, 0u, 0u, 0u};
       qh[s] = __builtin_bit_cast(f16x8, qvalid ? *reinterpret_cast<const u32x4*>(qs + 16 * s) : z);
-      ql[s] = __builtin_bit_cast(f16x8, qvalid ? *reinterpret_cast<const u32x4*>(qs + 128 + 16 * s) : z);
+      if constexpr (PRODUCTS == 3)
+        ql[s] = __builtin_bit_cast(f16x8, qvalid ? *reinterpret_cast<const u32x4*>(qs + 128 + 16 * s) : z);
     }
     auto load_tile = [&](int r0, uint32_t (&w)[8], unsigned& aux) {
       const int row = r0 + col < sz ? r0 + col : sz - 1;
@@ -576,7 +671,13 @@
 #pragma unroll
       for (int s = 0; s < KS; ++s) {
         u32x4 vh, vl;
-        if constexpr (DS == 2) {
+        if constexpr (PRODUCTS == 1) {
+          const int j0 = 8 * s + 4 * half;
+#pragma unroll
+          for (int bb = 0; bb < 4; ++bb) vh[bb] = book[(j0 + bb) * 256 + (int)((w[s] >> (8 * bb)) & 255u)];
+          acc = __builtin_amdgcn_mfma_f32_32x32x16_f16(__builtin_bit_cast(f16x8, vh), qh[s], acc, 0, 0, 0);
+          continue;
+        } else if constexpr (DS == 2) {
           const int j0 = 8 * s + 4 * half;
           uint2 en[4];
 #pragma unroll
@@ -707,10 +808,12 @@
   }
 }
 
-template <int DS, bool NORMS, bool MAXIMA = false>
-static int launch_cand(const CellArgs& a, dim3 grid, dim3 wg, hipStream_t st) {
-  return a.euclid ? launch_with_lds(cell_cand_kernel<DS, NORMS, true, MAXIMA>, "cell_cand_kernel", grid, wg, CellBook<DS>::kBytes, st, a)
-                  : launch_with_lds(cell_cand_kernel<DS, NORMS, false, MAXIMA>, "cell_cand_kernel", grid, wg, CellBook<DS>::kBytes, st, a);
+template <int DS, bool NORMS, bool MAXIMA = false, int PRODUCTS = 3>
+static int launch_cand(const CellArgs& a, dim3 grid, hipStream_t st) {
+  using T = CellBook<DS, PRODUCTS>;
+  const dim3 wg(T::kThreads);
+  return a.euclid ? launch_with_lds(cell_cand_kernel<DS, NORMS, true, MAXIMA, PRODUCTS>, "cell_cand_kernel", grid, wg, T::kBytes, st, a)
+                  : launch_with_lds(cell_cand_kernel<DS, NORMS, false, MAXIMA, PRODUCTS>, "cell_cand_kernel", grid, wg, T::kBytes, st, a);
 }
 
 static int cell_cus() {
@@ -795,7 +898,8 @@
   int64_t blocks = (int64_t)a.n_cells + np / kCellGroup;
   if (blocks > np) blocks = np;
   if (blocks < 1) return 0;
-  blocks = (blocks * cell_pieces(maxima) + kCellWaves - 1) / kCellWaves;
+  const int waves = cell_waves(a.products);
+  blocks = (blocks * cell_pieces(maxima) + waves - 1) / waves;
   return (unsigned)(blocks > n_cus ? n_cus : blocks);
 }
 
@@ -812,13 +916,14 @@
   if (a.p_hi <= a.p0) return TPQ_OK;
   if (int rc = launch_cell_inversion(a, st)) return rc;
   const int n_cus = cell_cus();
-  const dim3 grid(cell_cand_grid(a, n_cus)), cand_wg(64 * kCellWaves);
+  TPQ_REQUIRE(a.products == 3, "ivfpq_scan (cell-major): the seeded form runs three products");
+  const dim3 grid(cell_cand_grid(a, n_cus));
   if (a.norm) {
     if (!a.book)
       if (int rc = launch_cell_norms(a, n_cus, st)) return rc;
-    return a.ds == 1 ? launch_cand<1, true>(a, grid, cand_wg, st) : launch_cand<2, true>(a, grid, cand_wg, st);
-  }
-  return a.ds == 1 ? launch_cand<1, false>(a, grid, cand_wg, st) : launch_cand<2, false>(a, grid, cand_wg, st);
+    return a.ds == 1 ? launch_cand<1, true>(a, grid, st) : launch_cand<2, true>(a, grid, st);
+  }
+  return a.ds == 1 ? launch_cand<1, false>(a, grid, st) : launch_cand<2, false>(a, grid, st);
 }
 
 void cell_fill_thr(CellThrArrays& t, void* at, int nq, int max_nprobe, int n_cells) {
@@ -868,9 +973,11 @@
     if (int rc = launch_cell_norms(b, n_cus, st)) return rc;
   if (!one_walk)
     if (int rc = launch_cell_inversion(pa, st)) return rc;
-  const dim3 cand_wg(64 * kCellWaves);
-  if (int rc = a.ds == 1 ? launch_cand<1, true, true>(pa, dim3(cell_cand_grid(pa, n_cus, true)), cand_wg, st)
-                         : launch_cand<2, true, true>(pa, dim3(cell_cand_grid(pa, n_cus, true)), cand_wg, st))
+  const bool single = a.products == 1;
+  const dim3 grid_a(cell_cand_grid(pa, n_cus, true));
+  if (int rc = a.ds == 1 ? launch_cand<1, true, true>(pa, grid_a, st)
+               : single  ? launch_cand<2, true, true, 1>(pa, grid_a, st)
+                         : launch_cand<2, true, true>(pa, grid_a, st))
     return rc;
   const dim3 per_query((unsigned)((a.nq + 3) / 4));
   if (a.chunks <= 8)
@@ -879,7 +986,9 @@
     hipLaunchKernelGGL(cell_kth_kernel<16>, per_query, dim3(256), 0, st, b);
   TPQ_LAUNCH_CHECK("cell_kth_kernel");
   const dim3 grid(cell_cand_grid(b, n_cus));
-  return a.ds == 1 ? launch_cand<1, true>(b, grid, cand_wg, st) : launch_cand<2, true>(b, grid, cand_wg, st);
+  return a.ds == 1 ? launch_cand<1, true>(b, grid, st)
+         : single  ? launch_cand<2, true, false, 1>(b, grid, st)
+                   : launch_cand<2, true>(b, grid, st);
 }
 
 }
@@ -917,6 +1026,7 @@
   a.euclid = metric == TPQ_METRIC_NEG_SQ_L2 ? 1 : 0;
   a.p0 = first_probe; a.p_hi = max_nprobe; a.k = 0; a.chunks = capacity / 64; a.epoch = 1; a.rel = cell_delta_rel(ds);
   a.thr_in = threshold;
+  a.products = 3;
   a.keys = out_keys; a.idx = out_addr; a.flags = out_flags; a.ws_delta = out_delta;
   cell_fill_extras(a, workspace, workspace_bytes);
   a.cnt = out_count;
diff --git a/torchpq_amd/csrc/scan_host.h b/torchpq_amd/csrc/scan_host.h
--- a/torchpq_amd/csrc/scan_host.h
+++ b/torchpq_amd/csrc/scan_host.h
@@ -18,6 +18,7 @@
   const int slack = (slots_hint > 0 && slots_hint <= 16384) ? kBandSlack : 16 + k / 8;
   return pow2_ceil((k + slack + 63) / 64);
 }
+static int cell_single_finish_regs(int k) { return pow2_ceil((k + 4 * (16 + k / 8) + 63) / 64); }
 #ifndef TPQ_SCAN_MIN_RL_K
 #define TPQ_SCAN_MIN_RL_K 1
 #endif
diff --git a/torchpq_amd/fn/IVFPQTopk.py b/torchpq_amd/fn/IVFPQTopk.py
--- a/torchpq_amd/fn/IVFPQTopk.py
+++ b/torchpq_amd/fn/IVFPQTopk.py
@@ -17,13 +17,14 @@
 
     def topk_fused(self, data, query, codebook, cell_start, cell_size, is_empty, n_probe_list, k=256,
                    distance="euclidean", packed=None, address2id=None, slots_hint=None, cells=None, n_cells=0,
-                   cell_threshold=True, kept=None):
+                   cell_threshold=True, kept=None, cell_single_product=True):
         assert 0 < k <= 1024
         return self._scan.topk_fused(data=data, query=query, codebook=codebook, is_empty=is_empty,
                                      cell_start=cell_start, cell_size=cell_size,
                                      n_probe_list=n_probe_list, n_candidates=k, distance=distance,
                                      packed=packed, address2id=address2id, slots_hint=slots_hint,
-                                     cells=cells, n_cells=n_cells, cell_threshold=cell_threshold, kept=kept)
+                                     cells=cells, n_cells=n_cells, cell_threshold=cell_threshold, kept=kept,
+                                     cell_single_product=cell_single_product)
 
     def topk_residual(self, data, precomputed, cell_start, cell_size, base_sims, is_empty,
                       n_probe_list, k=256, address2id=None):
diff --git a/torchpq_amd/index/IVFPQIndex.py b/torchpq_amd/index/IVFPQIndex.py
--- a/torchpq_amd/index/IVFPQIndex.py
+++ b/torchpq_amd/index/IVFPQIndex.py
@@ -16,6 +16,7 @@
     fused_lut_max_subvector = 4
     use_cell_major = True
     use_cell_threshold = True
+    use_cell_single_product = True
     use_cell_kept = True
 
     def __init__(self, d_vector, n_subvectors=8, n_cells=128, initial_size=None,
@@ -50,6 +51,7 @@
         self.use_fused_lut = True
         self.use_cell_major = True
         self.use_cell_threshold = True
+        self.use_cell_single_product = True
         self.use_cell_kept = True
         self._cell_kept = None
         self._cell_kept_built = 0
@@ -280,7 +282,7 @@
             found = self._ivfpq_topk.topk_fused(
                 packed=self._scan_layout(), query=x, codebook=self.pq_codec.codebook, k=k, distance=self.distance,
                 slots_hint=slots_hint, cells=cells if self.use_cell_major else None, n_cells=self.n_cells,
-                cell_threshold=self.use_cell_threshold,
+                cell_threshold=self.use_cell_threshold, cell_single_product=self.use_cell_single_product,
                 kept=self._cell_kept_state if self.use_cell_kept and self.use_cell_major else None, **lists)
         else:
             found = self._ivfpq_topk.topk(
diff --git a/torchpq_amd/index/graphed.py b/torchpq_amd/index/graphed.py
--- a/torchpq_amd/index/graphed.py
+++ b/torchpq_amd/index/graphed.py
@@ -6,7 +6,7 @@
 class GraphedSearch:
 
     KNOBS = ("n_probe", "use_smart_probing", "_smart_probing_temperature", "use_packed_layout",
-             "use_fused_lut", "use_cell_major", "use_cell_threshold", "use_cell_kept", "use_fused_probe", "use_cublas", "_use_precomputed", "pq_use_residual",
+             "use_fused_lut", "use_cell_major", "use_cell_threshold", "use_cell_single_product", "use_cell_kept", "use_fused_probe", "use_cublas", "_use_precomputed", "pq_use_residual",
              "distance", "max_query_batch", "_has_holes", "_codes_version")
 
     @staticmethod
diff --git a/torchpq_amd/kernels/scan.py b/torchpq_amd/kernels/scan.py
--- a/torchpq_amd/kernels/scan.py
+++ b/torchpq_amd/kernels/scan.py
@@ -55,6 +55,7 @@
         self._last_cells = None
         self._last_withheld = False
         self.last_cell_kept = None
+        self._last_products = None
 
     def _tickets(self, n_query, n_split, device):
         if n_split <= 1:
@@ -158,6 +159,9 @@
         if self._last_cells is None or self._last_withheld:
             return False
         return self.cell_threshold(self.last_workspace_bytes, *self._last_cells)
+
+    def last_cell_products(self):
+        return self._last_products
 
     def last_cell_threshold_state(self):
         assert self.last_workspace is not None and self.last_cell_threshold() is True
@@ -198,7 +202,7 @@
         return workgroups_per_query(n_query, self.n_cus, per_cu, waves, slots_hint)
 
     def _scan(self, name, inputs, data, cell_start, address2id, k, n_split, slots_hint, packed, ticketed,
-              cells=None, n_cells=0, cell_threshold=True, kept=None, **route):
+              cells=None, n_cells=0, cell_threshold=True, kept=None, cell_single_product=True, **route):
         n_data, device = data.shape[1], data.device
         n_query, n_probe = cell_start.shape
         values, address, ids = alloc_topk(n_query, k, device, address2id)
@@ -240,11 +244,14 @@
                     kept.before_use(device)
                     tail += (ptr(kept.buf), kept.buf.numel(), int(kept.valid))
             before = lib.tpq_ivfpq_scan_use_cell_threshold(1 if cell_threshold else 0)
+            before_sp = lib.tpq_ivfpq_scan_use_cell_single_product(1 if cell_single_product else 0)
             try:
                 rc = getattr(lib, name)(*inputs, ptr(values), ptr(address), ptr(address2id), ptr(ids), n_data, n_query,
                                         n_probe, self.m, k, n_split, ptr(ws), ws_bytes, *tail, stream_ptr(device))
+                self._last_products = lib.tpq_ivfpq_scan_last_cell_products()
             finally:
                 lib.tpq_ivfpq_scan_use_cell_threshold(before)
+                lib.tpq_ivfpq_scan_use_cell_single_product(before_sp)
             if rc != 0 and ticketed:
                 self._drop_tickets(device)
             check(rc, name)
@@ -289,7 +296,7 @@
 
     def topk_fused(self, data, query, codebook, is_empty, cell_start, cell_size, n_probe_list,
                    n_candidates, distance="euclidean", packed=None, address2id=None, n_split=None,
-                   slots_hint=None, cells=None, n_cells=0, cell_threshold=True, kept=None):
+                   slots_hint=None, cells=None, n_cells=0, cell_threshold=True, kept=None, cell_single_product=True):
         n_data = data.shape[1]
         n_query, n_probe = cell_start.shape
         m, ds, kk = codebook.shape
@@ -313,7 +320,7 @@
             require_gpu(cells)
             return self._scan("tpq_ivfpq_search_fused_cells", inputs, data, cell_start, address2id, n_candidates,
                               n_split, slots_hint, packed, True, cells=cells, n_cells=n_cells, cell_threshold=cell_threshold,
-                              kept=kept, ds=ds, has_lut=False)
+                              kept=kept, cell_single_product=cell_single_product, ds=ds, has_lut=False)
         return self._scan("tpq_ivfpq_search_fused_tickets", inputs, data, cell_start, address2id, n_candidates,
                           n_split, slots_hint, packed, True, ds=ds, has_lut=False)
 
```

Measured after the change: 13.83 million queries/s, median of 6. 1.08x the previous value.
